# glmanhtu/vit-ed

Hardware: AMD Instinct MI355X
Metric: patch-pairs/sec fwd+bwd, div2k_erosion7_4bin_patch8_64 ViT-ED (higher is better)
Workload: dtype bf16

## Files before the change

### include/vited.h

```cpp
#ifndef VITED_H
#define VITED_H

#include <stdint.h>

#ifdef __cplusplus
extern "C" {
#endif

#define VITED_ABI_VERSION 1

#define VITED_OK 0
#define VITED_ERR_BAD_ARG 1
#define VITED_ERR_UNSUPPORTED 2
#define VITED_ERR_LAUNCH 3
#define VITED_ERR_WORKSPACE 4

#define VITED_F32 0
#define VITED_BF16 1
#define VITED_F16 2
#define VITED_I32 3
#define VITED_I64 4

#define VITED_EPI_STORE 0
#define VITED_EPI_GELU 1
#define VITED_EPI_RESIDUAL 2
#define VITED_EPI_MUL_GELU_GRAD 3
#define VITED_EPI_STORE_F32 4
#define VITED_EPI_MUL 5
#define VITED_EPI_GELU_GRAD 6

#define VITED_B_NK 0
#define VITED_B_KN 1

int vited_abi_version(void);
const char* vited_strerror(int code);

int vited_last_gemm_path(void);
int vited_last_attention_path(void);


int vited_cast(const void* src, int src_dtype, void* dst, int dst_dtype, int64_t n, void* stream);

int vited_cast_transpose(const float* src, void* dst, int dst_dtype, int64_t rows, int64_t cols, void* stream);

int vited_cast_weights(const int64_t* desc, int count, int64_t total_tiles, void* stream);

int vited_patchify(const float* img, int64_t img_bs, const int64_t* batch_index, void* out, int out_dtype,
                   int64_t batch, int chans, int img_size, int patch, void* stream);

int vited_patchify_u8(const uint8_t* img, int64_t img_bs, const int64_t* batch_index, void* out, int out_dtype,
                      int64_t batch, int chans, int img_size, int patch, const float* mean, const float* std, void* stream);

int vited_crop_pairs_u8(const uint8_t* src, int64_t src_bs, const int* cells, const int* erode, uint8_t* out, int64_t batch,
                        int chans, int img_size, void* stream);

int vited_div2k_regions_u8(const uint8_t* store, const int64_t* img_off, const int* img_hw, int n_images, const int* image,
                           const int* flags, const double* minv, const float* rgb, const int* crop, uint8_t* out, int64_t batch,
                           int img_size, void* stream);

int vited_hisfrag_windows_u8(const uint8_t* store, const int64_t* img_off, const int* img_hw, int n_images, const int* image,
                             const int* flags, const int64_t* afix, const double* minv, const int* origin, uint8_t* out, int64_t batch,
                             int img_size, void* stream);

int vited_hisfrag_jitter_u8(const uint8_t* in, const int* flags, const int* order, const float* factors, const int* hue, int64_t* sums,
                            uint8_t* out, int64_t batch, int img_size, void* stream);

int vited_hisfrag_blur_u8(const uint8_t* in, const int* flags, const float* weights, uint8_t* out, int64_t batch, int img_size,
                          void* stream);

int vited_michigan_windows_u8(const uint8_t* store, const int64_t* img_off, const int* img_hw, int n_images, const int* image,
                              const int* flags, const int* origin, const int* x0, const int* kx, const int* y0, const int* ky,
                              const int* holes, const int* n_holes, uint8_t* out, int64_t batch, int img_size, void* stream);

int vited_michigan_blur_gray_u8(const uint8_t* in, const int* flags, const int* weights, uint8_t* out, int64_t batch, int img_size,
                                void* stream);

int vited_slice_rows_cast(const float* in, void* out, int out_dtype, int64_t batch, int64_t in_rows,
                          int64_t row_offset, int64_t rows, int64_t dim, void* stream);

int vited_write_cls_row(float* x, const float* cls, const float* pos, int64_t batch, int64_t rows_per_batch,
                        int64_t dim, void* stream);

int64_t vited_sum_rows_workspace_bytes(int64_t batch, int64_t width);
int vited_sum_rows(const void* in, int in_dtype, int64_t in_ld, float* out, int64_t batch, int64_t width,
                   float* workspace, int64_t workspace_bytes, void* stream);


int vited_layernorm_fwd(const float* x, int64_t x_ld, const float* gamma, const float* beta, void* y,
                        int y_dtype, int64_t y_ld, float* mean, float* rstd, int64_t rows, int64_t dim,
                        float eps, void* stream);

int64_t vited_layernorm_bwd_workspace_bytes(int64_t rows, int64_t dim);
int vited_layernorm_bwd(const void* dy, int dy_dtype, int64_t dy_ld, const float* x, int64_t x_ld,
                        const float* gamma, const float* mean, const float* rstd, const float* dx_in,
                        int64_t dx_in_ld, float* dx_out, int64_t dx_out_ld, void* dx_lp, int dx_lp_dtype,
                        int64_t dx_lp_ld, float* dgamma, float* dbeta, int accumulate, int64_t rows, int64_t dim,
                        float* workspace, int64_t workspace_bytes, void* stream);

int vited_layernorm_bwd_scaled(const void* dy, int dy_dtype, int64_t dy_ld, const float* x, int64_t x_ld,
                               const float* gamma, const float* mean, const float* rstd, const float* dx_in,
                               int64_t dx_in_ld, float* dx_out, int64_t dx_out_ld, void* dx_lp, int dx_lp_dtype,
                               int64_t dx_lp_ld, const float* lp_scale, float* dgamma, float* dbeta, int accumulate,
                               int64_t rows, int64_t dim, float* workspace, int64_t workspace_bytes, void* stream);

int vited_scale_rows_cast(const float* src, int64_t src_ld, const float* row_scale, void* dst, int dst_dtype, int64_t dst_ld,
                          int64_t rows, int64_t dim, void* stream);


int vited_gemm(const void* A, int64_t lda, const void* B, int64_t ldb, int b_layout, int dtype, int64_t M,
               int64_t N, int64_t K, int epilogue, const float* bias, const void* aux,
               const float* residual, void* out, void* out2, int64_t ldo, int64_t rows_per_batch,
               int64_t out_rows_per_batch, int64_t row_offset, int residual_bcast, void* stream);

int vited_gemm_scaled(const void* A, int64_t lda, const void* B, int64_t ldb, int b_layout, int dtype, int64_t M, int64_t N,
                      int64_t K, const float* bias, const float* residual, const float* row_scale, float* out, int64_t ldo,
                      void* stream);

int64_t vited_linear_bwd_weight_workspace_bytes(int64_t M, int64_t N, int64_t K);
int vited_linear_bwd_weight(const void* dY, int64_t lddy, const void* X, int64_t ldx, int dtype, int64_t M,
                            int64_t N, int64_t K, float* dW, float* dbias, int accumulate, float* workspace,
                            int64_t workspace_bytes, void* stream);

int vited_linear_bwd_weight_batched_supported(int count, const int64_t* M, const int64_t* N, const int64_t* K, int dtype);
int64_t vited_linear_bwd_weight_batched_workspace_bytes(int count, const int64_t* M, const int64_t* N, const int64_t* K);
int vited_linear_bwd_weight_batched(int count, const void* const* dY, const int64_t* lddy, const void* const* X,
                                    const int64_t* ldx, const int64_t* M, const int64_t* N, const int64_t* K, float* const* dW,
                                    float* const* dbias, int dtype, int accumulate, float* workspace, int64_t workspace_bytes,
                                    void* stream);

int vited_linear_layernorm_supported(int64_t M, int64_t N, int64_t K);

int vited_linear_residual_layernorm_fwd(const void* a, int64_t lda, const void* w, int64_t ldw, const float* bias,
                                        const float* residual, int64_t ldr, float* y, int64_t ldy, const float* gamma,
                                        const float* beta, float eps, void* h, int64_t ldh, float* mean, float* rstd,
                                        int64_t M, int64_t N, int64_t K, void* stream);

int vited_linear_residual_layernorm_fwd_scaled(const void* a, int64_t lda, const void* w, int64_t ldw, const float* bias,
                                               const float* residual, int64_t ldr, const float* row_scale, float* y, int64_t ldy,
                                               const float* gamma, const float* beta, float eps, void* h, int64_t ldh, float* mean,
                                               float* rstd, int64_t M, int64_t N, int64_t K, void* stream);

int vited_linear_layernorm_bwd_segmented(const void* dy, int64_t lddy, int64_t seg_k, int64_t seg_stride, int64_t segments,
                                         const void* wt, int64_t ldwt, const float* x, int64_t ldx, const float* gamma,
                                         const float* mean, const float* rstd, const float* dx_in, int64_t dx_in_ld,
                                         float* dx_out, int64_t dx_out_ld, void* dx_lp, int64_t dx_lp_ld, float* dgamma,
                                         float* dbeta, int accumulate, int64_t M, int64_t N, float* workspace,
                                         int64_t workspace_bytes, void* stream);
int64_t vited_linear_layernorm_bwd_partial_rows(int64_t M);
int vited_layernorm_bwd_finish_batched(int count, const float* const* partial, const int* nparts, float* const* dgamma,
                                       float* const* dbeta, const int* accumulate, int64_t dim, void* stream);
int64_t vited_linear_layernorm_bwd_workspace_bytes(int64_t M, int64_t N);
int vited_linear_layernorm_bwd(const void* dy, int64_t lddy, const void* wt, int64_t ldwt, const float* x, int64_t ldx,
                               const float* gamma, const float* mean, const float* rstd, const float* dx_in,
                               int64_t dx_in_ld, float* dx_out, int64_t dx_out_ld, void* dx_lp, int64_t dx_lp_ld,
                               float* dgamma, float* dbeta, int accumulate, int64_t M, int64_t N, int64_t K,
                               float* workspace, int64_t workspace_bytes, void* stream);

int vited_linear_layernorm_bwd_scaled(const void* dy, int64_t lddy, const void* wt, int64_t ldwt, const float* x, int64_t ldx,
                                      const float* gamma, const float* mean, const float* rstd, const float* dx_in,
                                      int64_t dx_in_ld, float* dx_out, int64_t dx_out_ld, void* dx_lp, int64_t dx_lp_ld,
                                      const float* lp_scale, float* dgamma, float* dbeta, int accumulate, int64_t M, int64_t N,
                                      int64_t K, float* workspace, int64_t workspace_bytes, void* stream);

int vited_fold_context_weights(int count, const float* const* w, const float* const* bias, const float* const* gamma,
                               const float* const* beta, int64_t N, int64_t K, void* w_out, void* wt_out, float* bias_out,
                               void* stream);
int vited_unfold_context_grads(int count, const float* dwf, const float* dbf, const float* const* w, const float* const* gamma,
                               const float* const* beta, float* const* dw, float* const* dbias, float* const* dgamma, float* const* dbeta, int64_t N,
                               int64_t K, int accumulate, void* stream);


int vited_mlp_fwd(const float* x, int64_t ldx, const float* gamma, const float* beta, const void* w1, const float* b1,
                  const void* w2, const float* b2, float* y, int64_t ldy, void* h, void* gd, void* u, float* mean,
                  float* rstd, int64_t rows, int64_t dim, int64_t hidden, float eps, void* stream);

int64_t vited_block_workspace_bytes(int64_t batch, int64_t tokens, int64_t dim, int64_t hidden, int heads);
int vited_block_fwd(const float* x, float* y, int64_t batch, int64_t tokens, int64_t dim, int heads, int64_t hidden,
                    const float* ln1_g, const float* ln1_b, const void* wqkv, const float* bqkv, const void* wproj,
                    const float* bproj, const float* ln2_g, const float* ln2_b, const void* w1, const float* b1,
                    const void* w2, const float* b2, float eps, void* workspace, int64_t workspace_bytes, void* stream);

int64_t vited_cross_block_workspace_bytes(int64_t batch, int64_t tokens, int64_t ctx_tokens, int64_t dim, int64_t hidden, int heads);
int vited_cross_block_fwd(const float* x, const float* context, float* y, int64_t batch, int64_t tokens, int64_t ctx_tokens,
                          int64_t dim, int heads, int64_t hidden, const float* ln1_g, const float* ln1_b, const void* wqkv,
                          const float* bqkv, const void* wproj, const float* bproj, const float* lnq_g, const float* lnq_b,
                          const float* lnc_g, const float* lnc_b, const void* wq, const float* bq, const void* wkv,
                          const float* bkv, const void* wcproj, const float* bcproj, const float* ln2_g, const float* ln2_b,
                          const void* w1, const float* b1, const void* w2, const float* b2, float eps, void* workspace,
                          int64_t workspace_bytes, void* stream);


int64_t vited_adamw_workspace_bytes(void);
int vited_adamw_step(const int64_t* desc, int count, int64_t total_tiles, const float* grad_flat, int64_t grad_numel,
                     float* hyper, float max_norm, int zero_grad, float* norm_out, float* workspace,
                     int64_t workspace_bytes, void* stream);

int vited_sgd_step(const int64_t* desc, int count, int64_t total_tiles, const float* grad_flat, int64_t grad_numel,
                   float* hyper, float max_norm, int zero_grad, float* norm_out, float* workspace,
                   int64_t workspace_bytes, void* stream);


int vited_attention_fwd(const void* q, int64_t q_bs, int64_t q_ts, const void* k, int64_t k_bs, int64_t k_ts,
                        const void* v, int64_t v_bs, int64_t v_ts, void* o, int64_t o_bs, int64_t o_ts,
                        float* lse, int dtype, int64_t batch, int heads, int64_t nq, int64_t nk, int head_dim,
                        float scale, void* stream);

int vited_attention_fwd_indexed(const void* q, int64_t q_bs, int64_t q_ts, const void* k, int64_t k_bs, int64_t k_ts,
                                const void* v, int64_t v_bs, int64_t v_ts, const int64_t* kv_index, void* o, int64_t o_bs,
                                int64_t o_ts, float* lse, int dtype, int64_t batch, int heads, int64_t nq, int64_t nk,
                                int head_dim, float scale, void* stream);

int vited_attention_bwd(const void* q, int64_t q_bs, int64_t q_ts, const void* k, int64_t k_bs, int64_t k_ts,
                        const void* v, int64_t v_bs, int64_t v_ts, const void* o, const void* d_o,
                        int64_t o_bs, int64_t o_ts, const float* lse, float* delta, void* dq, int64_t dq_bs,
                        int64_t dq_ts, void* dk, int64_t dk_bs, int64_t dk_ts, void* dv, int64_t dv_bs,
                        int64_t dv_ts, int dtype, int64_t batch, int heads, int64_t nq, int64_t nk,
                        int head_dim, float scale, void* stream);

int64_t vited_attention_bwd_indexed_workspace_bytes(int dtype, int64_t batch, int heads, int64_t nk, int head_dim);
int vited_attention_bwd_indexed(const void* q, int64_t q_bs, int64_t q_ts, const void* k, int64_t k_bs, int64_t k_ts,
                                const void* v, int64_t v_bs, int64_t v_ts, const int64_t* kv_index, const int64_t* seg_order,
                                const int64_t* seg_offsets, int64_t kv_items, const void* o, const void* d_o, int64_t o_bs,
                                int64_t o_ts, const float* lse, float* delta, void* dq, int64_t dq_bs, int64_t dq_ts, void* dk,
                                int64_t dk_bs, int64_t dk_ts, void* dv, int64_t dv_bs, int64_t dv_ts, int dtype, int64_t batch,
                                int heads, int64_t nq, int64_t nk, int head_dim, float scale, void* workspace,
                                int64_t workspace_bytes, void* stream);

enum { VITED_CAM_GRAD = 0, VITED_CAM_PROB = 1 };
int vited_attention_cam(const void* q, int64_t q_bs, int64_t q_ts, const void* k, int64_t k_bs, int64_t k_ts,
                        const void* v, int64_t v_bs, int64_t v_ts, const void* d_o, int64_t do_bs, int64_t do_ts,
                        const float* lse, const float* head_weight, float* cam, int64_t cam_bs, int64_t cam_ld,
                        int mode, int dtype, int64_t batch, int heads, int64_t nq, int64_t nk, int head_dim,
                        float scale, void* stream);


int vited_retrieval_metrics(const void* D, int dtype, int64_t ld, int64_t n, int64_t r0, int64_t r1, const int* labels,
                            const int* offsets, const int* members, int num_classes, int remove_self_column, int from_similarity,
                            double* rows_out, double* sums, void* stream);


int vited_group_retrieval_metrics(const void* D, int dtype, int64_t ld, int64_t n, int64_t r0, int64_t r1, const int* labels,
                                  int num_labels, const int* col_offsets, const int* col_members, const int* pos_offsets,
                                  const int* pos_labels, const int* neg_offsets, const int* neg_labels, const int* ks, int nk,
                                  double* rows_out, double* sums, void* stream);


int64_t vited_pair_scores_workspace_bytes(int64_t n, int64_t m);
int vited_pair_scores_add(const void* pairs, int pair_dtype, int64_t pair_ld, const void* scores, int score_dtype, int64_t m, int64_t n,
                          int* counts, int* rec_cells, float* rec_values, int* bad, void* stream);
int vited_pair_scores_finish(const int* rec_cells, const float* rec_values, int64_t m, int64_t n, const int* counts, float* mean,
                             float* minv, double* stdev, double* stats, int* bad, void* workspace, int64_t workspace_bytes,
                             void* stream);

int vited_puzzle_distances_from_logits(const float* logits, const int64_t* pi, const int64_t* pj, int64_t m, int64_t n, int* dq,
                                       int* bad, void* stream);
int vited_puzzle_compat_init(const int* dq, int64_t n, int64_t* min_d, int64_t* second_d, int* candidate, int* best_buddy,
                             float* compat, float* mutual, int* start_count, float* start_total, int* start_order, void* stream);
int vited_puzzle_compat_recalc(const int* dq, int64_t n, const int* placed, int64_t* min_d, int64_t* second_d, float* compat,
                               float* mutual, int* changed, void* stream);
int vited_puzzle_best_slot(const float* mutual, int64_t n, const int* placed, const int* slot_piece, const int* slot_side,
                           int64_t slots, int64_t* best, void* stream);

int vited_cls_metrics_update(const float* logits, int64_t ld_logits, const float* targets, int64_t ld_targets, int64_t batch,
                             int64_t classes, double* meters, double* last, int* bad, void* stream);

int vited_mine_pairs_max_images(void);
int vited_mine_pairs(const int64_t* targets, int n, const float* keys, double neg_per_pos, int ordered_negatives, int64_t capacity,
                     int64_t* groups, float* labels, float* weights, int64_t* seg_index, int64_t* seg_order, int64_t* seg_offsets,
                     int32_t* counts, void* stream);

#ifdef __cplusplus
}
#endif
#endif
```

### vit-ed_amd/csrc/attention.hip

```cpp
#include "attention_kernels.h"
#include "pair_segsum.h"

static thread_local int g_last_attn_path = 0;
extern "C" int vited_last_attention_path(void) { return g_last_attn_path; }
void attention_set_last_path(int path) { g_last_attn_path = path; }

static int check_common(const AttnArgs& a, int dtype) {
    if (!a.q || !a.k || !a.v || !a.o || !a.lse) return VITED_ERR_BAD_ARG;
    if (a.batch <= 0 || a.heads <= 0 || a.nq <= 0 || a.nk <= 0 || a.head_dim <= 0) return VITED_ERR_BAD_ARG;
    if (dtype != VITED_F32 && dtype != VITED_BF16) return VITED_ERR_UNSUPPORTED;
    if (a.batch > 65535 || a.heads > 65535) return VITED_ERR_UNSUPPORTED;
    return VITED_OK;
}

extern "C" int vited_attention_fwd(const void* q, int64_t q_bs, int64_t q_ts, const void* k, int64_t k_bs, int64_t k_ts,
                                   const void* v, int64_t v_bs, int64_t v_ts, void* o, int64_t o_bs, int64_t o_ts,
                                   float* lse, int dtype, int64_t batch, int heads, int64_t nq, int64_t nk, int head_dim,
                                   float scale, void* stream) {
    return vited_attention_fwd_indexed(q, q_bs, q_ts, k, k_bs, k_ts, v, v_bs, v_ts, nullptr, o, o_bs, o_ts, lse, dtype, batch, heads, nq,
                                       nk, head_dim, scale, stream);
}

extern "C" int vited_attention_fwd_indexed(const void* q, int64_t q_bs, int64_t q_ts, const void* k, int64_t k_bs, int64_t k_ts,
                                           const void* v, int64_t v_bs, int64_t v_ts, const int64_t* kv_index, void* o, int64_t o_bs,
                                           int64_t o_ts, float* lse, int dtype, int64_t batch, int heads, int64_t nq, int64_t nk,
                                           int head_dim, float scale, void* stream) {
    AttnArgs a = {};
    a.q = q; a.k = k; a.v = v;
    a.kv_index = kv_index;
    a.q_bs = q_bs; a.q_ts = q_ts; a.k_bs = k_bs; a.k_ts = k_ts; a.v_bs = v_bs; a.v_ts = v_ts;
    a.o = o; a.o_bs = o_bs; a.o_ts = o_ts;
    a.lse = lse;
    a.batch = batch; a.heads = heads; a.nq = nq; a.nk = nk; a.head_dim = head_dim; a.scale = scale;
    int rc = check_common(a, dtype);
    if (rc != VITED_OK) return rc;
    hipStream_t s = (hipStream_t)stream;
    if (dtype == VITED_BF16 && attention_mfma_supported(a, false)) {
        g_last_attn_path = 2;
        return attention_fwd_mfma(a, s);
    }
    g_last_attn_path = 1;
    return attention_fwd_portable(a, dtype, s);
}

static int bwd_dispatch(const AttnArgs& a, int dtype, hipStream_t s) {
    if (dtype == VITED_BF16 && attention_mfma_supported(a, true)) {
        g_last_attn_path = 2;
        return attention_bwd_mfma(a, s);
    }
    g_last_attn_path = 1;
    return attention_bwd_portable(a, dtype, s);
}

extern "C" int vited_attention_bwd(const void* q, int64_t q_bs, int64_t q_ts, const void* k, int64_t k_bs, int64_t k_ts,
                                   const void* v, int64_t v_bs, int64_t v_ts, const void* o, const void* d_o, int64_t o_bs,
                                   int64_t o_ts, const float* lse, float* delta, void* dq, int64_t dq_bs, int64_t dq_ts,
                                   void* dk, int64_t dk_bs, int64_t dk_ts, void* dv, int64_t dv_bs, int64_t dv_ts, int dtype,
                                   int64_t batch, int heads, int64_t nq, int64_t nk, int head_dim, float scale, void* stream) {
    AttnArgs a = {};
    a.q = q; a.k = k; a.v = v;
    a.q_bs = q_bs; a.q_ts = q_ts; a.k_bs = k_bs; a.k_ts = k_ts; a.v_bs = v_bs; a.v_ts = v_ts;
    a.o = o; a.d_o = d_o; a.o_bs = o_bs; a.o_ts = o_ts;
    a.lse = (float*)lse; a.delta = delta;
    a.dq = dq; a.dk = dk; a.dv = dv;
    a.dq_bs = dq_bs; a.dq_ts = dq_ts; a.dk_bs = dk_bs; a.dk_ts = dk_ts; a.dv_bs = dv_bs; a.dv_ts = dv_ts;
    a.batch = batch; a.heads = heads; a.nq = nq; a.nk = nk; a.head_dim = head_dim; a.scale = scale;
    int rc = check_common(a, dtype);
    if (rc != VITED_OK) return rc;
    if (!d_o || !delta || !dq || !dk || !dv) return VITED_ERR_BAD_ARG;
    return bwd_dispatch(a, dtype, (hipStream_t)stream);
}

static int64_t elem_bytes(int dtype) { return dtype == VITED_BF16 ? 2 : 4; }

extern "C" int64_t vited_attention_bwd_indexed_workspace_bytes(int dtype, int64_t batch, int heads, int64_t nk, int head_dim) {
    if ((dtype != VITED_F32 && dtype != VITED_BF16) || batch <= 0 || heads <= 0 || nk <= 0 || head_dim <= 0) return -1;
    return batch * nk * 2 * (int64_t)heads * head_dim * elem_bytes(dtype);
}

extern "C" int vited_attention_bwd_indexed(const void* q, int64_t q_bs, int64_t q_ts, const void* k, int64_t k_bs, int64_t k_ts,
                                           const void* v, int64_t v_bs, int64_t v_ts, const int64_t* kv_index,
                                           const int64_t* seg_order, const int64_t* seg_offsets, int64_t kv_items, const void* o,
                                           const void* d_o, int64_t o_bs, int64_t o_ts, const float* lse, float* delta, void* dq,
                                           int64_t dq_bs, int64_t dq_ts, void* dk, int64_t dk_bs, int64_t dk_ts, void* dv,
                                           int64_t dv_bs, int64_t dv_ts, int dtype, int64_t batch, int heads, int64_t nq, int64_t nk,
                                           int head_dim, float scale, void* workspace, int64_t workspace_bytes, void* stream) {
    AttnArgs a = {};
    a.q = q; a.k = k; a.v = v;
    a.kv_index = kv_index;
    a.q_bs = q_bs; a.q_ts = q_ts; a.k_bs = k_bs; a.k_ts = k_ts; a.v_bs = v_bs; a.v_ts = v_ts;
    a.o = o; a.d_o = d_o; a.o_bs = o_bs; a.o_ts = o_ts;
    a.lse = (float*)lse; a.delta = delta;
    a.dq = dq; a.dq_bs = dq_bs; a.dq_ts = dq_ts;
    a.batch = batch; a.heads = heads; a.nq = nq; a.nk = nk; a.head_dim = head_dim; a.scale = scale;
    int rc = check_common(a, dtype);
    if (rc != VITED_OK) return rc;
    if (!d_o || !delta || !dq || !dk || !dv || !kv_index || !seg_order || !seg_offsets || !workspace) return VITED_ERR_BAD_ARG;
    if (kv_items <= 0 || ((uintptr_t)workspace % 16) != 0) return VITED_ERR_BAD_ARG;
    if (kv_items > 65535) return VITED_ERR_UNSUPPORTED;
    if (workspace_bytes < vited_attention_bwd_indexed_workspace_bytes(dtype, batch, heads, nk, head_dim)) return VITED_ERR_WORKSPACE;
    const int64_t width = (int64_t)heads * head_dim;
    a.dk = workspace;
    a.dv = (char*)workspace + width * elem_bytes(dtype);
    a.dk_ts = a.dv_ts = 2 * width;
    a.dk_bs = a.dv_bs = nk * 2 * width;
    hipStream_t s = (hipStream_t)stream;
    rc = bwd_dispatch(a, dtype, s);
    if (rc != VITED_OK) return rc;
    SegSumArgs g = {};
    g.ws = workspace;
    g.out[0] = dk; g.out_bs[0] = dk_bs; g.out_ts[0] = dk_ts;
    g.out[1] = dv; g.out_bs[1] = dv_bs; g.out_ts[1] = dv_ts;
    g.order = seg_order; g.offsets = seg_offsets;
    g.batch = batch; g.items = kv_items; g.nk = nk; g.width = (int)width;
    return attention_segsum(g, dtype, s);
}
```

### vit-ed_amd/csrc/attention_kernels.h

```cpp
#pragma once
#include "common.h"

struct AttnArgs {
    const void *q, *k, *v;
    const int64_t* kv_index;
    int64_t q_bs, q_ts, k_bs, k_ts, v_bs, v_ts;
    const void* o;
    const void* d_o;
    int64_t o_bs, o_ts;
    float* lse;
    float* delta;
    void *dq, *dk, *dv;
    int64_t dq_bs, dq_ts, dk_bs, dk_ts, dv_bs, dv_ts;
    int64_t batch, nq, nk;
    int heads, head_dim;
    float scale;
};

int attention_fwd_portable(const AttnArgs& a, int dtype, hipStream_t s);
int attention_bwd_portable(const AttnArgs& a, int dtype, hipStream_t s);

bool attention_mfma_supported(const AttnArgs& a, bool backward);
int attention_fwd_mfma(const AttnArgs& a, hipStream_t s);
int attention_bwd_mfma(const AttnArgs& a, hipStream_t s);

int attention_fwd_flash(const AttnArgs& a, hipStream_t s);
int attention_bwd_flash(const AttnArgs& a, hipStream_t s);

struct SegSumArgs;
int attention_segsum(const SegSumArgs& a, int dtype, hipStream_t s);

void attention_set_last_path(int path);
```

### vit-ed_amd/csrc/attention_mfma.hip

```cpp
#include "attention_tiles.h"

template <int HD, int NKT>
__global__ void __launch_bounds__(256)
attn_fwd_small_kernel(AttnArgs a) {
    using C = SmallCfg<HD>;
    extern __shared__ __attribute__((aligned(16))) char smem[];
    const int lane = threadIdx.x & 63;
    const int wave = __builtin_amdgcn_readfirstlane(threadIdx.x >> 6);
    const int fr = lane & 15, g = lane >> 4, qq = fr >> 2, p = fr & 3;
    const int64_t b = blockIdx.x;
    int h = blockIdx.y * 4 + wave;
    const bool live = h < a.heads;
    h = live ? h : a.heads - 1;
    const int nq = (int)a.nq, nk = (int)a.nk;
    const bf16* qb = (const bf16*)a.q + b * a.q_bs + (int64_t)h * HD;
    const int64_t bkv = a.kv_index ? a.kv_index[b] : b;
    const bf16* kb = (const bf16*)a.k + bkv * a.k_bs + (int64_t)h * HD;
    const bf16* vb = (const bf16*)a.v + bkv * a.v_bs + (int64_t)h * HD;
    char* vs = smem + wave * C::TILE_BYTES;
    char* os = smem + 4 * C::TILE_BYTES + wave * 16 * C::ROW_BYTES;

    bf16x8 kf[NKT][C::KCH], qnext[C::KCH];
    load_row_frags<HD>(qb, a.q_ts, 0, nq, fr, g, qnext);
#pragma unroll
    for (int t = 0; t < NKT; ++t) {
        load_row_frags<HD>(kb, a.k_ts, 16 * t, nk, fr, g, kf[t]);
        bf16x8 vf[C::KCH];
        load_row_frags<HD>(vb, a.v_ts, 16 * t, nk, fr, g, vf);
        stage_tile<HD>(vs, 16 * t, nk, fr, g, vf);
    }
    if (NKT & 1) {
        const bf16x8 z[C::KCH] = {};
        stage_tile<HD>(vs, 16 * NKT, 0, fr, g, z);
    }
    asm volatile("" ::: "memory");
    const float sc = a.scale * LOG2E;
    const int nqt = (nq + 15) >> 4;
    for (int i = 0; i < nqt; ++i) {
        bf16x8 qf[C::KCH];
#pragma unroll
        for (int c = 0; c < C::KCH; ++c) qf[c] = qnext[c];
        if (i + 1 < nqt) load_row_frags<HD>(qb, a.q_ts, 16 * (i + 1), nq, fr, g, qnext);
        f32x4 st[NKT + 1];
        float m = -INFINITY;
#pragma unroll
        for (int t = 0; t < NKT; ++t) {
            f32x4 s = {0.f, 0.f, 0.f, 0.f};
#pragma unroll
            for (int c = 0; c < C::KCH; ++c) s = __builtin_amdgcn_mfma_f32_16x16x32_bf16(kf[t][c], qf[c], s, 0, 0, 0);
            if (t == NKT - 1) {
#pragma unroll
                for (int e = 0; e < 4; ++e) s[e] = (16 * t + 4 * g + e) < nk ? s[e] : -INFINITY;
            }
            m = fmaxf(fmaxf(m, fmaxf(s[0], s[1])), fmaxf(s[2], s[3]));
            st[t] = s;
        }
        st[NKT] = f32x4{0.f, 0.f, 0.f, 0.f};
        m = group_max4(m) * sc;
        float l = 0.f;
#pragma unroll
        for (int t = 0; t < NKT; ++t)
#pragma unroll
            for (int e = 0; e < 4; ++e) {
                const float pe = __builtin_amdgcn_exp2f(fmaf(st[t][e], sc, -m));
                st[t][e] = pe;
                l += pe;
            }
        l = group_sum4(l);
        const float inv = 1.f / l;
        const int q = 16 * i + fr;
#pragma unroll
        for (int dt = 0; dt < C::DT; ++dt) {
            f32x4 o = {0.f, 0.f, 0.f, 0.f};
#pragma unroll
            for (int ks = 0; ks < (NKT + 1) / 2; ++ks) {
                const bf16x8 vt = tr_frag<HD>(vs, ks, dt, g, qq, p);
                o = __builtin_amdgcn_mfma_f32_16x16x32_bf16(vt, pack_pair(st[2 * ks], st[2 * ks + 1]), o, 0, 0, 0);
            }
            const bf16x4 ov = {(bf16)(o[0] * inv), (bf16)(o[1] * inv), (bf16)(o[2] * inv), (bf16)(o[3] * inv)};
            *(bf16x4*)(os + fr * C::ROW_BYTES + (dt * 16 + 4 * g) * 2) = ov;
        }
        asm volatile("" ::: "memory");
        {
            constexpr int CPR = C::ROW_BYTES / 16;
#pragma unroll
            for (int j = 0; j < 16 * CPR / 64; ++j) {
                const int c = lane + 64 * j;
                const int row = c / CPR, ch = c % CPR;
                const bf16x8 v = *(const bf16x8*)(os + row * C::ROW_BYTES + ch * 16);
                if (live && 16 * i + row < nq)
                    *(bf16x8*)((bf16*)a.o + b * a.o_bs + (int64_t)(16 * i + row) * a.o_ts + (int64_t)h * HD + ch * 8) = v;
            }
        }
        asm volatile("" ::: "memory");
        if (live && g == 0 && q < nq) a.lse[(b * a.heads + h) * a.nq + q] = (m + log2f(l)) * LN2;
    }
}

template <int HD, int NT>
__device__ __forceinline__ void store_rows4(const char* region, bf16* dst_head0, int64_t ts, int n, int live_heads, int tid) {
    constexpr int ROW = 4 * HD * 2, CPR = ROW / 16;
#pragma unroll
    for (int j = 0; j < NT * 16 * CPR / 256; ++j) {
        const int c = tid + 256 * j;
        const int row = c / CPR, ch = c % CPR;
        const bf16x8 v = *(const bf16x8*)(region + row * ROW + ch * 16);
        if (row < n && ch / (CPR / 4) < live_heads) *(bf16x8*)(dst_head0 + (int64_t)row * ts + ch * 8) = v;
    }
}

template <int HD, int NQT, int NKT> struct BwdSmallLds {
    static constexpr int MAXT = NQT > NKT ? NQT : NKT;
    static constexpr int IMG_TILES = (MAXT + 1) & ~1;
    static constexpr int IMG_BYTES = IMG_TILES * 16 * HD * 2;
    static constexpr int STAT_FLOATS = IMG_TILES * 16;
    static constexpr int WAVE_BYTES = 2 * IMG_BYTES + 2 * STAT_FLOATS * 4;
    static constexpr int SLOT1_BASE = 4 * IMG_BYTES, STATS_BASE = 8 * IMG_BYTES;
};

template <int HD, int NQT, int NKT>
#ifndef ATTN_BWD_WAVES_PER_EU
#define ATTN_BWD_WAVES_PER_EU 3
#endif
__global__ void __launch_bounds__(256) __attribute__((amdgpu_waves_per_eu(ATTN_BWD_WAVES_PER_EU)))
attn_bwd_small_kernel(AttnArgs a) {
    using C = SmallCfg<HD>;
    extern __shared__ __attribute__((aligned(16))) char smem[];
    using L = BwdSmallLds<HD, NQT, NKT>;
    const int lane = threadIdx.x & 63;
    const int wave = __builtin_amdgcn_readfirstlane(threadIdx.x >> 6);
    const int fr = lane & 15, g = lane >> 4, qq = fr >> 2, p = fr & 3;
    const int64_t b = blockIdx.y;
    const int hg = blockIdx.x;
    int h = hg * 4 + wave;
    const bool live = h < a.heads;
    h = live ? h : a.heads - 1;
    const int nq = (int)a.nq, nk = (int)a.nk;
    const int64_t hoff = (int64_t)h * HD;
    const bf16* qb = (const bf16*)a.q + b * a.q_bs + hoff;
    const int64_t bkv = a.kv_index ? a.kv_index[b] : b;
    const bf16* kb = (const bf16*)a.k + bkv * a.k_bs + hoff;
    const bf16* vb = (const bf16*)a.v + bkv * a.v_bs + hoff;
    const bf16* dob = (const bf16*)a.d_o + b * a.o_bs + hoff;
    char* k_s = smem + wave * L::IMG_BYTES;
    char* q_s = k_s;
    char* do_s = smem + L::SLOT1_BASE + wave * L::IMG_BYTES;
    float* lse_s = (float*)(smem + L::STATS_BASE) + wave * 2 * L::STAT_FLOATS;
    float* del_s = lse_s + L::STAT_FLOATS;
    char* out0 = smem;
    char* out1 = smem + L::SLOT1_BASE;
    const int tid = threadIdx.x;
    const int live_heads = a.heads - hg * 4;
    const int64_t hoff0 = (int64_t)hg * 4 * HD;
    constexpr int OROW = 4 * HD * 2;
    const float sc = a.scale * LOG2E;

    bf16x8 kf[NKT][C::KCH], vf[NKT][C::KCH], qf[NQT][C::KCH], dof[NQT][C::KCH];
    float lse_r[NQT];
#pragma unroll
    for (int t = 0; t < NKT; ++t) {
        load_row_frags<HD>(kb, a.k_ts, 16 * t, nk, fr, g, kf[t]);
        load_row_frags<HD>(vb, a.v_ts, 16 * t, nk, fr, g, vf[t]);
    }
#pragma unroll
    for (int i = 0; i < NQT; ++i) {
        load_row_frags<HD>(qb, a.q_ts, 16 * i, nq, fr, g, qf[i]);
        load_row_frags<HD>(dob, a.o_ts, 16 * i, nq, fr, g, dof[i]);
        const int q = 16 * i + fr;
        lse_r[i] = a.lse[(b * a.heads + h) * a.nq + (q < nq ? q : nq - 1)];
    }
    asm volatile("" ::: "memory");
#pragma unroll
    for (int t = 0; t < NKT; ++t) stage_tile<HD>(k_s, 16 * t, nk, fr, g, kf[t]);
#pragma unroll
    for (int i = 0; i < NQT; ++i) {
        const int q = 16 * i + fr;
        if (g == 0) lse_s[q] = lse_r[i] * LOG2E;
    }
    {
        const bf16x8 z[C::KCH] = {};
        if (NKT & 1) stage_tile<HD>(k_s, 16 * NKT, 0, fr, g, z);
    }
    asm volatile("" ::: "memory");

#pragma unroll
    for (int i = 0; i < NQT; ++i) {
        const int q = 16 * i + fr;
        const float lse2 = lse_s[q];
        f32x4 ds[NKT + 1], dpv[NKT];
        float dl = 0.f;
#pragma unroll
        for (int t = 0; t < NKT; ++t) {
            f32x4 s = {0.f, 0.f, 0.f, 0.f}, dp = {0.f, 0.f, 0.f, 0.f};
#pragma unroll
            for (int c = 0; c < C::KCH; ++c) {
                s = __builtin_amdgcn_mfma_f32_16x16x32_bf16(kf[t][c], qf[i][c], s, 0, 0, 0);
                dp = __builtin_amdgcn_mfma_f32_16x16x32_bf16(vf[t][c], dof[i][c], dp, 0, 0, 0);
            }
#pragma unroll
            for (int e = 0; e < 4; ++e) {
                float pe = __builtin_amdgcn_exp2f(fmaf(s[e], sc, -lse2));
                if (t == NKT - 1) pe = (16 * t + 4 * g + e) < nk ? pe : 0.f;
                ds[t][e] = pe;
                dl = fmaf(pe, dp[e], dl);
            }
            dpv[t] = dp;
        }
        dl = group_sum4(dl);
        if (g == 0) del_s[q] = dl;
#pragma unroll
        for (int t = 0; t < NKT; ++t)
#pragma unroll
            for (int e = 0; e < 4; ++e) ds[t][e] *= dpv[t][e] - dl;
        ds[NKT] = f32x4{0.f, 0.f, 0.f, 0.f};
#pragma unroll
        for (int dt = 0; dt < C::DT; ++dt) {
            f32x4 acc = {0.f, 0.f, 0.f, 0.f};
#pragma unroll
            for (int ks = 0; ks < (NKT + 1) / 2; ++ks)
                acc = __builtin_amdgcn_mfma_f32_16x16x32_bf16(tr_frag<HD>(k_s, ks, dt, g, qq, p),
                                                              pack_pair(ds[2 * ks], ds[2 * ks + 1]), acc, 0, 0, 0);
            const bf16x4 ov = {(bf16)(acc[0] * a.scale), (bf16)(acc[1] * a.scale), (bf16)(acc[2] * a.scale), (bf16)(acc[3] * a.scale)};
            *(bf16x4*)(out1 + q * OROW + wave * (HD * 2) + (dt * 16 + 4 * g) * 2) = ov;
        }
    }
    __syncthreads();
    store_rows4<HD, NQT>(out1, (bf16*)a.dq + b * a.dq_bs + hoff0, a.dq_ts, nq, live_heads, tid);
    __syncthreads();

    asm volatile("" ::: "memory");
#pragma unroll
    for (int i = 0; i < NQT; ++i) {
        stage_tile<HD>(q_s, 16 * i, nq, fr, g, qf[i]);
        stage_tile<HD>(do_s, 16 * i, nq, fr, g, dof[i]);
    }
    if (NQT & 1) {
        const bf16x8 z[C::KCH] = {};
        stage_tile<HD>(q_s, 16 * NQT, 0, fr, g, z);
        stage_tile<HD>(do_s, 16 * NQT, 0, fr, g, z);
    }
    asm volatile("" ::: "memory");
    bf16x4 dvo[NKT][C::DT], dko[NKT][C::DT];
#pragma unroll
    for (int t = 0; t < NKT; ++t) {
        f32x4 pr[NQT + 1], ds[NQT + 1];
#pragma unroll
        for (int i = 0; i < NQT; ++i) {
            f32x4 s = {0.f, 0.f, 0.f, 0.f}, dp = {0.f, 0.f, 0.f, 0.f};
#pragma unroll
            for (int c = 0; c < C::KCH; ++c) {
                s = __builtin_amdgcn_mfma_f32_16x16x32_bf16(qf[i][c], kf[t][c], s, 0, 0, 0);
                dp = __builtin_amdgcn_mfma_f32_16x16x32_bf16(dof[i][c], vf[t][c], dp, 0, 0, 0);
            }
            const f32x4 l4 = *(const f32x4*)(lse_s + 16 * i + 4 * g);
            const f32x4 d4 = *(const f32x4*)(del_s + 16 * i + 4 * g);
#pragma unroll
            for (int e = 0; e < 4; ++e) {
                float pe = __builtin_amdgcn_exp2f(fmaf(s[e], sc, -l4[e]));
                if (i == NQT - 1) pe = (16 * i + 4 * g + e) < nq ? pe : 0.f;
                pr[i][e] = pe;
                ds[i][e] = pe * (dp[e] - d4[e]);
            }
        }
        pr[NQT] = f32x4{0.f, 0.f, 0.f, 0.f};
        ds[NQT] = f32x4{0.f, 0.f, 0.f, 0.f};
#pragma unroll
        for (int dt = 0; dt < C::DT; ++dt) {
            f32x4 av = {0.f, 0.f, 0.f, 0.f}, ak = {0.f, 0.f, 0.f, 0.f};
#pragma unroll
            for (int qs = 0; qs < (NQT + 1) / 2; ++qs) {
                av = __builtin_amdgcn_mfma_f32_16x16x32_bf16(tr_frag<HD>(do_s, qs, dt, g, qq, p),
                                                             pack_pair(pr[2 * qs], pr[2 * qs + 1]), av, 0, 0, 0);
                ak = __builtin_amdgcn_mfma_f32_16x16x32_bf16(tr_frag<HD>(q_s, qs, dt, g, qq, p),
                                                             pack_pair(ds[2 * qs], ds[2 * qs + 1]), ak, 0, 0, 0);
            }
            dvo[t][dt] = bf16x4{(bf16)av[0], (bf16)av[1], (bf16)av[2], (bf16)av[3]};
            dko[t][dt] = bf16x4{(bf16)(ak[0] * a.scale), (bf16)(ak[1] * a.scale), (bf16)(ak[2] * a.scale), (bf16)(ak[3] * a.scale)};
        }
        __builtin_amdgcn_sched_barrier(0);
    }
    __syncthreads();
#pragma unroll
    for (int t = 0; t < NKT; ++t)
#pragma unroll
        for (int dt = 0; dt < C::DT; ++dt) {
            *(bf16x4*)(out0 + (16 * t + fr) * OROW + wave * (HD * 2) + (dt * 16 + 4 * g) * 2) = dvo[t][dt];
            *(bf16x4*)(out1 + (16 * t + fr) * OROW + wave * (HD * 2) + (dt * 16 + 4 * g) * 2) = dko[t][dt];
        }
    __syncthreads();
    store_rows4<HD, NKT>(out0, (bf16*)a.dv + b * a.dv_bs + hoff0, a.dv_ts, nk, live_heads, tid);
    store_rows4<HD, NKT>(out1, (bf16*)a.dk + b * a.dk_bs + hoff0, a.dk_ts, nk, live_heads, tid);
}

static bool small_ok(const AttnArgs& a, bool backward) {
    if (a.nk > 16 * SM_MAX_TILES) return false;
    if (backward) return a.head_dim == 32 && a.nq <= 16 * SM_MAX_TILES;
    return true;
}

bool attention_mfma_supported(const AttnArgs& a, bool backward) {
    auto al = [](const void* p, int n) { return ((uintptr_t)p % n) == 0; };
    if (a.head_dim != 32 && a.head_dim != 64) return false;
    if (a.nq > (1 << 20) || a.nk > (1 << 20)) return false;
    if (a.q_ts % 8 || a.k_ts % 8 || a.v_ts % 8 || a.q_bs % 8 || a.k_bs % 8 || a.v_bs % 8 || a.o_ts % 8 || a.o_bs % 8) return false;
    if (!al(a.q, 16) || !al(a.k, 16) || !al(a.v, 16) || !al(a.o, 16)) return false;
    if (backward) {
        if (a.dq_ts % 8 || a.dk_ts % 8 || a.dv_ts % 8 || a.dq_bs % 8 || a.dk_bs % 8 || a.dv_bs % 8) return false;
        if (!al(a.d_o, 16) || !al(a.dq, 16) || !al(a.dk, 16) || !al(a.dv, 16)) return false;
    }
    return true;
}

template <int HD>
static int launch_fwd_small(const AttnArgs& a, hipStream_t s) {
    const int nkt = (int)((a.nk + 15) / 16);
    dim3 grid((unsigned)a.batch, (unsigned)((a.heads + 3) / 4));
    const size_t lds = 4 * SmallCfg<HD>::TILE_BYTES + 4 * 16 * SmallCfg<HD>::ROW_BYTES;
#define L(N) hipLaunchKernelGGL((attn_fwd_small_kernel<HD, N>), grid, dim3(256), lds, s, a)
    switch (nkt) {
        case 1: L(1); break;
        case 2: L(2); break;
        case 3: L(3); break;
        case 4: L(4); break;
        case 5: L(5); break;
        default: return VITED_ERR_UNSUPPORTED;
    }
#undef L
    return vited_check_launch();
}

int attention_fwd_mfma(const AttnArgs& a, hipStream_t s) {
    if (!small_ok(a, false)) return attention_fwd_flash(a, s);
    if (a.head_dim == 32) return launch_fwd_small<32>(a, s);
    if (a.head_dim == 64) return launch_fwd_small<64>(a, s);
    return VITED_ERR_UNSUPPORTED;
}

template <int NQT, int NKT>
static void launch_bwd_small_one(const AttnArgs& a, dim3 grid, hipStream_t s) {
    auto kernel = attn_bwd_small_kernel<32, NQT, NKT>;
    constexpr size_t lds = 4 * BwdSmallLds<32, NQT, NKT>::WAVE_BYTES;
    hipLaunchKernelGGL(kernel, grid, dim3(256), lds, s, a);
}

template <int NQT>
static int launch_bwd_small32(const AttnArgs& a, int nkt, hipStream_t s) {
    dim3 grid((unsigned)((a.heads + 3) / 4), (unsigned)a.batch);
#define L(N) launch_bwd_small_one<NQT, N>(a, grid, s)
    switch (nkt) {
        case 1: L(1); break;
        case 2: L(2); break;
        case 3: L(3); break;
        case 4: L(4); break;
        case 5: L(5); break;
        default: return VITED_ERR_UNSUPPORTED;
    }
#undef L
    return vited_check_launch();
}

int attention_bwd_mfma(const AttnArgs& a, hipStream_t s) {
    if (!small_ok(a, true)) return attention_bwd_flash(a, s);
    const int nqt = (int)((a.nq + 15) / 16), nkt = (int)((a.nk + 15) / 16);
    switch (nqt) {
        case 1: return launch_bwd_small32<1>(a, nkt, s);
        case 2: return launch_bwd_small32<2>(a, nkt, s);
        case 3: return launch_bwd_small32<3>(a, nkt, s);
        case 4: return launch_bwd_small32<4>(a, nkt, s);
        case 5: return launch_bwd_small32<5>(a, nkt, s);
        default: return VITED_ERR_UNSUPPORTED;
    }
}
```

### vit-ed_amd/csrc/elementwise.hip

```cpp
#include "common.h"

template <typename S, typename D>
__global__ void cast_kernel(const S* __restrict__ src, D* __restrict__ dst, int64_t n) {
    int64_t i = ((int64_t)blockIdx.x * blockDim.x + threadIdx.x) * 4;
    const int64_t stride = (int64_t)gridDim.x * blockDim.x * 4;
    for (; i + 3 < n; i += stride) {
        S a = src[i], b = src[i + 1], c = src[i + 2], d = src[i + 3];
        dst[i] = from_f32<D>(to_f32(a));
        dst[i + 1] = from_f32<D>(to_f32(b));
        dst[i + 2] = from_f32<D>(to_f32(c));
        dst[i + 3] = from_f32<D>(to_f32(d));
    }
    for (; i < n; ++i) dst[i] = from_f32<D>(to_f32(src[i]));
}

extern "C" int vited_cast(const void* src, int src_dtype, void* dst, int dst_dtype, int64_t n, void* stream) {
    if (!src || !dst || n < 0) return VITED_ERR_BAD_ARG;
    if (n == 0) return VITED_OK;
    hipStream_t s = (hipStream_t)stream;
    const int threads = 256;
    int64_t blocks = ceil_div64(n, threads * 4);
    if (blocks > 4096) blocks = 4096;
    if (src_dtype == VITED_F32 && dst_dtype == VITED_BF16)
        hipLaunchKernelGGL((cast_kernel<float, bf16>), dim3(blocks), dim3(threads), 0, s, (const float*)src, (bf16*)dst, n);
// ... 84 lines not shown
        const int mid = (lo + hi + 1) >> 1;
        if (desc[(int64_t)mid * WS_DESC_WORDS + 5] <= blk) lo = mid; else hi = mid - 1;
    }
    const int64_t* d = desc + (int64_t)lo * WS_DESC_WORDS;
    const float* __restrict__ src = (const float*)d[0];
    bf16* __restrict__ dst = (bf16*)d[1];
    bf16* __restrict__ dst_t = (bf16*)d[2];
    const int64_t rows = d[3], cols = d[4];
    const int64_t t = blk - d[5], tiles_c = (cols + 63) >> 6;
    const int64_t r0 = (t / tiles_c) << 6, c0 = (t % tiles_c) << 6;
    const int tx = threadIdx.x & 15, ty = threadIdx.x >> 4;
    const bool vec = (cols & 3) == 0;
#pragma unroll
    for (int j = 0; j < 4; ++j) {
        const int lr = ty + 16 * j;
        const int64_t r = r0 + lr, c = c0 + tx * 4;
        float v[4] = {0.f, 0.f, 0.f, 0.f};
        if (r < rows) {
            if (vec && c + 3 < cols) {
                const f32x4 q = *(const f32x4*)(src + r * cols + c);
                v[0] = q[0]; v[1] = q[1]; v[2] = q[2]; v[3] = q[3];
            } else {
#pragma unroll
                for (int e = 0; e < 4; ++e) if (c + e < cols) v[e] = src[r * cols + c + e];
            }
        }
        bf16 b[4];
#pragma unroll
        for (int e = 0; e < 4; ++e) { b[e] = (bf16)v[e]; tile[lr][tx * 4 + e] = b[e]; }
        if (dst && r < rows) {
            if (vec && c + 3 < cols) *(bf16x4*)(dst + r * cols + c) = bf16x4{b[0], b[1], b[2], b[3]};
            else {
#pragma unroll
                for (int e = 0; e < 4; ++e) if (c + e < cols) dst[r * cols + c + e] = b[e];
            }
        }
    }
    if (!dst_t) return;
    __syncthreads();
    const bool vec_t = (rows & 3) == 0;
#pragma unroll
    for (int j = 0; j < 4; ++j) {
        const int lc = ty + 16 * j;
        const int64_t c = c0 + lc, r = r0 + tx * 4;
        if (c >= cols) continue;
        bf16 b[4];
#pragma unroll
        for (int e = 0; e < 4; ++e) b[e] = tile[tx * 4 + e][lc];
        if (vec_t && r + 3 < rows) *(bf16x4*)(dst_t + c * rows + r) = bf16x4{b[0], b[1], b[2], b[3]};
        else {
#pragma unroll
            for (int e = 0; e < 4; ++e) if (r + e < rows) dst_t[c * rows + r + e] = b[e];
        }
    }
}

extern "C" int vited_cast_weights(const int64_t* desc, int count, int64_t total_tiles, void* stream) {
    if (!desc || count <= 0 || total_tiles <= 0 || total_tiles > 0x7fffffff) return VITED_ERR_BAD_ARG;
    hipLaunchKernelGGL(cast_weights_kernel, dim3((unsigned)total_tiles), dim3(256), 0, (hipStream_t)stream, desc, count);
    return vited_check_launch();
}

template <typename D>
__global__ void patchify_kernel(const float* __restrict__ img, int64_t img_bs, const int64_t* __restrict__ bidx,
                                D* __restrict__ out, int chans, int S, int p) {
    const int G = S / p;
    const int64_t b = blockIdx.y;
    const int py = blockIdx.x;
    const int64_t src_b = bidx ? bidx[b] : b;
    const float* base = img + src_b * img_bs;
    const int Kp = chans * p * p;
    const int total = chans * p * S;
    D* obase = out + (b * G * G + (int64_t)py * G) * Kp;
    for (int e = threadIdx.x; e < total; e += blockDim.x) {
        const int x = e % S;
        const int ci = e / S;
        const int i = ci % p, c = ci / p;
        const float v = base[((int64_t)c * S + (py * p + i)) * S + x];
        const int px = x / p, j = x - px * p;
        obase[(int64_t)px * Kp + (c * p + i) * p + j] = from_f32<D>(v);
    }
}

extern "C" int vited_patchify(const float* img, int64_t img_bs, const int64_t* batch_index, void* out, int out_dtype,
                              int64_t batch, int chans, int img_size, int patch, void* stream) {
    if (!img || !out || batch <= 0 || chans <= 0 || img_size <= 0 || patch <= 0 || img_size % patch) return VITED_ERR_BAD_ARG;
    dim3 grid(img_size / patch, (unsigned)batch);
    hipStream_t s = (hipStream_t)stream;
    if (out_dtype == VITED_BF16)
        hipLaunchKernelGGL((patchify_kernel<bf16>), grid, dim3(256), 0, s, img, img_bs, batch_index, (bf16*)out, chans, img_size, patch);
    else if (out_dtype == VITED_F32)
        hipLaunchKernelGGL((patchify_kernel<float>), grid, dim3(256), 0, s, img, img_bs, batch_index, (float*)out, chans, img_size, patch);
    else
        return VITED_ERR_UNSUPPORTED;
    return vited_check_launch();
}

struct U8Norm { float scale[4], shift[4]; };

template <typename D>
__global__ void patchify_u8_kernel(const uint8_t* __restrict__ img, int64_t img_bs, const int64_t* __restrict__ bidx,
                                   D* __restrict__ out, int chans, int S, int p, U8Norm nrm) {
    const int G = S / p;
    const int64_t b = blockIdx.y;
    const int py = blockIdx.x;
    const int64_t src_b = bidx ? bidx[b] : b;
    const uint8_t* base = img + src_b * img_bs;
    const int Kp = chans * p * p;
    const int total = chans * p * S;
    D* obase = out + (b * G * G + (int64_t)py * G) * Kp;
    for (int e = threadIdx.x; e < total; e += blockDim.x) {
        const int x = e % S;
        const int ci = e / S;
        const int i = ci % p, c = ci / p;
        const float v = fmaf((float)base[((int64_t)c * S + (py * p + i)) * S + x], nrm.scale[c], nrm.shift[c]);
        const int px = x / p, j = x - px * p;
        obase[(int64_t)px * Kp + (c * p + i) * p + j] = from_f32<D>(v);
    }
}

extern "C" int vited_patchify_u8(const uint8_t* img, int64_t img_bs, const int64_t* batch_index, void* out, int out_dtype,
                                 int64_t batch, int chans, int img_size, int patch, const float* mean, const float* std,
                                 void* stream) {
    if (!img || !out || !mean || !std || batch <= 0 || chans <= 0 || chans > 4 || img_size <= 0 || patch <= 0 || img_size % patch)
        return VITED_ERR_BAD_ARG;
    U8Norm nrm = {};
    for (int c = 0; c < chans; ++c) {
        if (!(std[c] > 0.f)) return VITED_ERR_BAD_ARG;
        nrm.scale[c] = 1.0f / (255.0f * std[c]);
        nrm.shift[c] = -mean[c] / std[c];
    }
    dim3 grid(img_size / patch, (unsigned)batch);
    hipStream_t s = (hipStream_t)stream;
    if (out_dtype == VITED_BF16)
        hipLaunchKernelGGL((patchify_u8_kernel<bf16>), grid, dim3(256), 0, s, img, img_bs, batch_index, (bf16*)out, chans, img_size, patch, nrm);
    else if (out_dtype == VITED_F32)
        hipLaunchKernelGGL((patchify_u8_kernel<float>), grid, dim3(256), 0, s, img, img_bs, batch_index, (float*)out, chans, img_size, patch, nrm);
    else
        return VITED_ERR_UNSUPPORTED;
    return vited_check_launch();
}

struct ResampleTaps {
    int x0, n;
    int k0, k1;
};

__device__ __forceinline__ ResampleTaps resample_taps(int xx, int in_size, int out_size) {
    constexpr int PRECISION_BITS = 32 - 8 - 2;
    const double scale = (double)in_size / (double)out_size;
    const double center = (xx + 0.5) * scale;
    int xmin = (int)(center - 1.0 + 0.5);
    xmin = xmin < 0 ? 0 : xmin;
    int xmax = (int)(center + 1.0 + 0.5);
    xmax = (xmax < in_size ? xmax : in_size) - xmin;
    double w0 = 1.0 - fabs((double)xmin - center + 0.5), w1 = xmax > 1 ? 1.0 - fabs((double)xmin + 1.0 - center + 0.5) : 0.0;
    w0 = w0 < 0.0 ? 0.0 : w0;
    w1 = w1 < 0.0 ? 0.0 : w1;
    const double ww = w0 + w1;
    ResampleTaps t;
    t.x0 = xmin;
    t.n = xmax > 1 ? 2 : 1;
    t.k0 = (int)(0.5 + (w0 / ww) * (double)(1 << PRECISION_BITS));
    t.k1 = (int)(0.5 + (w1 / ww) * (double)(1 << PRECISION_BITS));
    return t;
}

__device__ __forceinline__ int resample_px(int p0, int p1, const ResampleTaps& t) {
    constexpr int PRECISION_BITS = 32 - 8 - 2;
    int acc = (1 << (PRECISION_BITS - 1)) + p0 * t.k0 + (t.n > 1 ? p1 * t.k1 : 0);
    acc >>= PRECISION_BITS;
    return acc < 0 ? 0 : (acc > 255 ? 255 : acc);
}

__global__ void __launch_bounds__(256)
crop_pairs_u8_kernel(const uint8_t* __restrict__ src, int64_t src_bs, const int* __restrict__ cells, const int* __restrict__ erode,
                     uint8_t* __restrict__ out, int chans, int S) {
    const int64_t b = blockIdx.z;
    const int img = blockIdx.y / chans, c = blockIdx.y % chans;
    int cell = cells[b * 2 + img], e = erode[b];
    cell = cell < 0 ? 0 : (cell > 5 ? 5 : cell);
    e = e < 1 ? 1 : (e > S ? S : e);
    const int off = (int)rint((S - e) / 2.0);
    const int r0 = (cell / 3) * S + off, c0 = (cell % 3) * S + off;
    const uint8_t* base = src + b * src_bs + ((int64_t)c * 2 * S + r0) * (3 * S) + c0;
    uint8_t* o = out + (((b * 2 + img) * chans + c) * (int64_t)S) * S;
    for (int i = blockIdx.x * blockDim.x + threadIdx.x; i < S * S; i += gridDim.x * blockDim.x) {
        const int y = i / S, x = i - y * S;
        const ResampleTaps tx = resample_taps(x, e, S), ty = resample_taps(y, e, S);
        const uint8_t* ra = base + (int64_t)ty.x0 * (3 * S) + tx.x0;
        const int h0 = resample_px(ra[0], tx.n > 1 ? ra[1] : 0, tx);
        int h1 = 0;
        if (ty.n > 1) {
            const uint8_t* rb = ra + 3 * S;
            h1 = resample_px(rb[0], tx.n > 1 ? rb[1] : 0, tx);
        }
        o[i] = (uint8_t)resample_px(h0, h1, ty);
    }
}

extern "C" int vited_crop_pairs_u8(const uint8_t* src, int64_t src_bs, const int* cells, const int* erode, uint8_t* out, int64_t batch,
                                   int chans, int img_size, void* stream) {
    if (!src || !cells || !erode || !out || batch <= 0 || chans <= 0 || img_size <= 0 || batch > 65535) return VITED_ERR_BAD_ARG;
    if (src_bs < (int64_t)chans * 6 * img_size * img_size) return VITED_ERR_BAD_ARG;
    const int per = img_size * img_size;
    dim3 grid((unsigned)((per + 1023) / 1024 < 8 ? (per + 1023) / 1024 : 8), (unsigned)(2 * chans), (unsigned)batch);
    hipLaunchKernelGGL(crop_pairs_u8_kernel, grid, dim3(256), 0, (hipStream_t)stream, src, src_bs, cells, erode, out, chans, img_size);
    return vited_check_launch();
}

template <typename D>
__global__ void slice_rows_cast_kernel(const float* __restrict__ in, D* __restrict__ out, int64_t in_rows,
                                       int64_t row_offset, int64_t rows, int64_t dim, int64_t total) {
    int64_t i = (int64_t)blockIdx.x * blockDim.x + threadIdx.x;
    const int64_t stride = (int64_t)gridDim.x * blockDim.x;
    const int64_t per_b = rows * dim;
    for (; i < total; i += stride) {
        const int64_t b = i / per_b, rem = i - b * per_b;
        out[i] = from_f32<D>(in[(b * in_rows + row_offset) * dim + rem]);
    }
}
// ... 8 lines not shown
    if (out_dtype == VITED_BF16)
        hipLaunchKernelGGL((slice_rows_cast_kernel<bf16>), dim3(blocks), dim3(256), 0, s, in, (bf16*)out, in_rows, row_offset, rows, dim, total);
    else if (out_dtype == VITED_F32)
        hipLaunchKernelGGL((slice_rows_cast_kernel<float>), dim3(blocks), dim3(256), 0, s, in, (float*)out, in_rows, row_offset, rows, dim, total);
    else
        return VITED_ERR_UNSUPPORTED;
    return vited_check_launch();
}

__global__ void write_cls_row_kernel(float* __restrict__ x, const float* __restrict__ cls, const float* __restrict__ pos,
                                     int64_t batch, int64_t rows_per_batch, int64_t dim) {
    int64_t i = (int64_t)blockIdx.x * blockDim.x + threadIdx.x;
    const int64_t total = batch * dim;
    if (i >= total) return;
    const int64_t b = i / dim, d = i - b * dim;
    x[b * rows_per_batch * dim + d] = cls[d] + pos[d];
}

extern "C" int vited_write_cls_row(float* x, const float* cls, const float* pos, int64_t batch, int64_t rows_per_batch,
                                   int64_t dim, void* stream) {
    if (!x || !cls || !pos || batch <= 0 || rows_per_batch <= 0 || dim <= 0) return VITED_ERR_BAD_ARG;
    const int64_t total = batch * dim;
    hipLaunchKernelGGL(write_cls_row_kernel, dim3((unsigned)ceil_div64(total, 256)), dim3(256), 0, (hipStream_t)stream,
                       x, cls, pos, batch, rows_per_batch, dim);
    return vited_check_launch();
}

template <typename S_>
__global__ void sum_rows_kernel(const S_* __restrict__ in, int64_t in_ld, float* __restrict__ out, int64_t batch,
                                int64_t width, int64_t rows_per_split) {
    const int64_t r = (int64_t)blockIdx.x * blockDim.x + threadIdx.x;
    if (r >= width) return;
    const int64_t b0 = (int64_t)blockIdx.y * rows_per_split;
    int64_t b1 = b0 + rows_per_split;
    if (b1 > batch) b1 = batch;
    float acc0 = 0.f, acc1 = 0.f, acc2 = 0.f, acc3 = 0.f;
    int64_t b = b0;
    for (; b + 3 < b1; b += 4) {
        acc0 += to_f32(in[b * in_ld + r]);
        acc1 += to_f32(in[(b + 1) * in_ld + r]);
        acc2 += to_f32(in[(b + 2) * in_ld + r]);
        acc3 += to_f32(in[(b + 3) * in_ld + r]);
    }
    for (; b < b1; ++b) acc0 += to_f32(in[b * in_ld + r]);
    out[(int64_t)blockIdx.y * width + r] = (acc0 + acc1) + (acc2 + acc3);
}

static inline int64_t sum_rows_splits(int64_t batch, int64_t width) {
    const int64_t col_blocks = ceil_div64(width, 256);
    int64_t s = ceil_div64(1024, col_blocks);
    const int64_t max_s = ceil_div64(batch, 16);
    if (s > max_s) s = max_s;
    if (s < 1) s = 1;
    return s;
}

extern "C" int64_t vited_sum_rows_workspace_bytes(int64_t batch, int64_t width) {
    return sum_rows_splits(batch, width) * width * (int64_t)sizeof(float);
}

extern "C" int vited_sum_rows(const void* in, int in_dtype, int64_t in_ld, float* out, int64_t batch, int64_t width,
                              float* workspace, int64_t workspace_bytes, void* stream) {
    if (!in || !out || batch <= 0 || width <= 0 || in_ld < width) return VITED_ERR_BAD_ARG;
    const int64_t S = sum_rows_splits(batch, width);
    hipStream_t s = (hipStream_t)stream;
    const unsigned col_blocks = (unsigned)ceil_div64(width, 256);
    float* pass1_out = out;
    if (S > 1) {
        if (!workspace || workspace_bytes < S * width * (int64_t)sizeof(float)) return VITED_ERR_WORKSPACE;
        pass1_out = workspace;
    }
    const int64_t rps = ceil_div64(batch, S);
    if (in_dtype == VITED_F32)
        hipLaunchKernelGGL((sum_rows_kernel<float>), dim3(col_blocks, (unsigned)S), dim3(256), 0, s, (const float*)in, in_ld, pass1_out, batch, width, rps);
    else if (in_dtype == VITED_BF16)
        hipLaunchKernelGGL((sum_rows_kernel<bf16>), dim3(col_blocks, (unsigned)S), dim3(256), 0, s, (const bf16*)in, in_ld, pass1_out, batch, width, rps);
    else
        return VITED_ERR_UNSUPPORTED;
    if (S > 1)
        hipLaunchKernelGGL((sum_rows_kernel<float>), dim3(col_blocks, 1), dim3(256), 0, s, (const float*)workspace, width, out, S, width, S);
    return vited_check_launch();
}

__device__ __forceinline__ void sum_slabs_body(const float* __restrict__ in, int64_t in_ld, float* __restrict__ out, int64_t batch,
                                               int64_t width, int accumulate, int64_t r) {
    if (r >= width) return;
    if (r + 3 < width) {
        f32x4 acc = accumulate ? *(const f32x4*)(out + r) : f32x4{0.f, 0.f, 0.f, 0.f};
        int64_t b = 0;
        for (; b + 4 <= batch; b += 4) {
            const f32x4 v0 = *(const f32x4*)(in + b * in_ld + r), v1 = *(const f32x4*)(in + (b + 1) * in_ld + r);
            const f32x4 v2 = *(const f32x4*)(in + (b + 2) * in_ld + r), v3 = *(const f32x4*)(in + (b + 3) * in_ld + r);
#pragma unroll
            for (int e = 0; e < 4; ++e) acc[e] += (v0[e] + v1[e]) + (v2[e] + v3[e]);
        }
        for (; b < batch; ++b) {
            const f32x4 v = *(const f32x4*)(in + b * in_ld + r);
#pragma unroll
            for (int e = 0; e < 4; ++e) acc[e] += v[e];
        }
        *(f32x4*)(out + r) = acc;
    } else {
        for (int64_t c = r; c < width; ++c) {
            float acc = accumulate ? out[c] : 0.f;
            for (int64_t b = 0; b < batch; ++b) acc += in[b * in_ld + c];
            out[c] = acc;
        }
    }
}

__global__ void sum_slabs_kernel(const float* __restrict__ in, int64_t in_ld, float* __restrict__ out, int64_t batch, int64_t width,
                                 int accumulate) {
    sum_slabs_body(in, in_ld, out, batch, width, accumulate, ((int64_t)blockIdx.x * blockDim.x + threadIdx.x) * 4);
}

__global__ void sum_slabs_pair_kernel(const float* __restrict__ in_a, int64_t ld_a, float* __restrict__ out_a, int64_t width_a,
                                      int blocks_a, const float* __restrict__ in_b, int64_t ld_b, float* __restrict__ out_b,
                                      int64_t width_b, int64_t batch, int accumulate) {
    if ((int)blockIdx.x < blocks_a)
        sum_slabs_body(in_a, ld_a, out_a, batch, width_a, accumulate, ((int64_t)blockIdx.x * blockDim.x + threadIdx.x) * 4);
    else
        sum_slabs_body(in_b, ld_b, out_b, batch, width_b, accumulate,
                       ((int64_t)(blockIdx.x - blocks_a) * blockDim.x + threadIdx.x) * 4);
}


__global__ void sum_slabs_scalar_kernel(const float* __restrict__ in, int64_t in_ld, float* __restrict__ out, int64_t batch,
                                        int64_t width, int accumulate) {
    const int64_t c = (int64_t)blockIdx.x * blockDim.x + threadIdx.x;
    if (c >= width) return;
    float acc = accumulate ? out[c] : 0.f;
    for (int64_t b = 0; b < batch; ++b) acc += in[b * in_ld + c];
    out[c] = acc;
}

int sum_rows_f32_single_pass(const float* in, int64_t in_ld, float* out, int64_t batch, int64_t width, hipStream_t s, int accumulate) {
    const bool vec = (width % 4 == 0) && (in_ld % 4 == 0) && ((((uintptr_t)in) | ((uintptr_t)out)) & 15) == 0;
    if (vec)
        hipLaunchKernelGGL(sum_slabs_kernel, dim3((unsigned)ceil_div64(width, 1024)), dim3(256), 0, s, in, in_ld, out, batch, width, accumulate);
    else
        hipLaunchKernelGGL(sum_slabs_scalar_kernel, dim3((unsigned)ceil_div64(width, 256)), dim3(256), 0, s, in, in_ld, out, batch, width, accumulate);
    return vited_check_launch();
}

#define SB_MAX 40
struct SumBatch {
    float* out[2 * SB_MAX];
    int64_t start[2 * SB_MAX + 1];
    const float* slabs;
    const float* bias_slabs;
    int64_t slab_stride, bias_stride, splits;
    int sections, accumulate;
};

__global__ void __launch_bounds__(256) sum_slabs_batch_kernel(const SumBatch b) {
    const int64_t r = ((int64_t)blockIdx.x * blockDim.x + threadIdx.x) * 4;
    if (r >= b.start[b.sections]) return;
    int sec = 0;
    for (int i = 1; i < b.sections; ++i)
        if (b.start[i] <= r) sec = i;
    float* out = b.out[sec];
    if (!out) return;
    const bool is_bias = r >= b.slab_stride;
    const float* in = is_bias ? b.bias_slabs + (r - b.slab_stride) : b.slabs + r;
    const int64_t ld = is_bias ? b.bias_stride : b.slab_stride;
    out += r - b.start[sec];
// ... 57 lines not shown
```

### vit-ed_amd/csrc/gemm_row.hip

```cpp
#include <mutex>
#include <type_traits>

#include "gemm_kernels.h"
#include "gemm_lds.h"

#define ROW_N 384
#define ROW_LD 388

enum { ROW_MODE_FWD = 0, ROW_MODE_BWD = 1 };

struct RowArgs {
    const bf16* A; int64_t lda;
    int seg_k; int64_t seg_stride;
    const bf16* W; int64_t ldw;
    int64_t M; int K;
    const float* bias; const float* residual; int64_t ldr;
    float* y; int64_t ldy;
    const float* gamma; const float* beta; float eps;
    bf16* h; int64_t ldh; float* mean; float* rstd;
    const float* x; int64_t ldx; const float* mean_in; const float* rstd_in;
    const float* dx_in; int64_t ldxi; float* dx; int64_t lddx; bf16* dx_lp; int64_t ldlp;
    float* partial;
    const float* row_scale;
    const float* lp_scale;
};

template <int MT> struct RowCfg {
    static_assert(MT == 6 || MT == 8 || MT == 9 || MT == 10, "tile heights: 96, 128, 144 or 160 rows");
    static constexpr int BM = 16 * MT;
    static constexpr int A_BYTES = BM * 128;
    static constexpr int W_BYTES = ROW_N * 128;
    static constexpr int W_BASE = 3 * A_BYTES;
    static constexpr int LDS_BYTES = 3 * A_BYTES + 2 * W_BYTES;
    static constexpr int P0 = (MT + 1) / 2;
    static constexpr int A_PIECES = 2 * MT;
    static constexpr int A_J = (A_PIECES + 3) / 4;
    static constexpr int PASS_SUB = MT == 8 ? 4 : MT == 10 ? 5 : 3;
    static constexpr int PASS_ROWS = 16 * PASS_SUB;
    static constexpr int NPASS = MT / PASS_SUB;
    static constexpr int ROWS_PER_HALF = PASS_ROWS / 16;
    static constexpr bool EPI_ALL_ROWS = MT <= 9;
    static_assert(MT % PASS_SUB == 0, "passes cover the tile");
    static_assert(LDS_BYTES <= 160 * 1024, "LDS");
    static_assert(LDS_BYTES >= PASS_ROWS * ROW_LD * 4, "epilogue scratch must fit the staging buffers");
    static_assert(LDS_BYTES >= 16 * 2 * ROW_N * 4, "column-partial combine must fit the staging buffers");
};

__device__ __forceinline__ float row_half_sum(float v) { return half_wave_sum(v); }

#define ROW_STORE(ptr, val) __builtin_nontemporal_store(val, ptr)
#define ROW_STORE_LP(ptr, val) (*(ptr) = (val))
#define ROW_LOAD(ptr) __builtin_nontemporal_load(ptr)

template <int SC> struct RowFwdIn { f32x4 res[3]; float scale[SC]; };
template <int SC> struct RowBwdIn { f32x4 x[3], din[3]; float mu, rs; float lps[SC]; };

template <int MODE, int MT, bool SCALED>
__global__ void __launch_bounds__(512)
gemm_row_kernel(const RowArgs a) {
    extern __shared__ __attribute__((aligned(16))) char smem[];
    using R = RowCfg<MT>;
    const int lane = threadIdx.x & 63;
    const int wave = __builtin_amdgcn_readfirstlane(threadIdx.x >> 6);
    const int64_t m0 = (int64_t)blockIdx.x * R::BM;

    f32x4 acc[MT][3];
#pragma unroll
    for (int i = 0; i < MT; ++i)
#pragma unroll
        for (int j = 0; j < 3; ++j) acc[i][j] = f32x4{0.f, 0.f, 0.f, 0.f};

    const int grp = wave >> 2, u = wave & 3;
    const int nt = a.K / 64;
    const int r8 = lane >> 3, c8 = lane & 7;
    const int cs_even = (c8 ^ (r8 >> 1)) * 8, cs_odd = (c8 ^ (r8 >> 1) ^ 4) * 8;
    const int cs_u = (u & 1) ? cs_odd : cs_even;
    const int a_per = (R::A_PIECES - u + 3) / 4;
    const bf16* pa[R::A_J];
#pragma unroll
    for (int j = 0; j < R::A_J; ++j) {
        int64_t ar = m0 + 8 * (4 * j + u) + r8;
#ifdef ROW_DBG_A_RESIDENT
        ar -= m0;
#endif
        ar = ar < a.M ? ar : a.M - 1;
        pa[j] = a.A + ar * a.lda + cs_u;
    }
    const bf16* pw = a.W + (int64_t)(8 * u + r8) * a.ldw + cs_u;
    auto issue_a = [&](int t) {
#ifdef ROW_DBG_NO_DMA
        return;
#endif
        if (t >= nt) return;
        char* dst = smem + (t % 3) * R::A_BYTES;
        const int k0 = t * 64;
        const int seg = k0 / a.seg_k;
        const int64_t ka = (int64_t)seg * a.seg_stride + (k0 - seg * a.seg_k);
#pragma unroll
        for (int j = 0; j < R::A_J; ++j)
            if (4 * j + 3 < R::A_PIECES || j < a_per) glds16_asm(pa[j] + ka, dst + (4 * j + u) * 1024);
    };
    auto issue_w = [&](int t, int part) {
#ifdef ROW_DBG_NO_DMA
        return;
// ... 65 lines not shown
    };
    using I0 = std::integral_constant<int, 0>;
    using IP0 = std::integral_constant<int, R::P0>;
    using IP1 = std::integral_constant<int, MT - R::P0>;
    if (grp == 0) {
        issue_a(0);
        issue_w(0, 1);
        issue_a(1);
        certify_barrier(nt > 1);
        for (int t = 0; t < nt; ++t) {
            read_b(t);
            read_a(t, I0{}, IP0{});
            issue_w(t + 1, 1);
            landed();
            barrier();
            mfmas(I0{}, IP0{});
            barrier();
            read_a(t, IP0{}, IP1{});
            issue_a(t + 2);
            landed();
            barrier();
            mfmas(IP0{}, IP1{});
            certify_barrier(t + 2 < nt);
        }
        barrier();
    } else {
        issue_w(0, 0);
        issue_w(0, 2);
        issue_w(1, 0);
        certify_barrier(nt > 1);
        barrier();
        for (int t = 0; t < nt; ++t) {
            read_b(t);
            read_a(t, I0{}, IP0{});
            issue_w(t + 1, 2);
            landed();
            barrier();
            mfmas(I0{}, IP0{});
            barrier();
            read_a(t, IP0{}, IP1{});
            issue_w(t + 2, 0);
            landed();
            certify_barrier(t + 2 < nt);
            mfmas(IP0{}, IP1{});
            barrier();
        }
    }
#ifdef ROW_DBG_NO_EPI
#pragma unroll
    for (int i = 0; i < MT; ++i)
#pragma unroll
        for (int j = 0; j < 3; ++j) asm volatile("" ::"v"(acc[i][j]));
    return;
#endif

    float* sc = (float*)smem;
    const int hl = lane & 31;
    const int hw = wave * 2 + (lane >> 5);
    const float inv_d = 1.0f / ROW_N;
    f32x4 gm[3], bt[3], bs[3];
#pragma unroll
    for (int j = 0; j < 3; ++j) {
        const int c = (j * 32 + hl) * 4;
        gm[j] = a.gamma ? *(const f32x4*)(a.gamma + c) : f32x4{1.f, 1.f, 1.f, 1.f};
        bt[j] = (MODE == ROW_MODE_FWD && a.beta) ? *(const f32x4*)(a.beta + c) : f32x4{0.f, 0.f, 0.f, 0.f};
        bs[j] = (MODE == ROW_MODE_FWD && a.bias) ? *(const f32x4*)(a.bias + c) : f32x4{0.f, 0.f, 0.f, 0.f};
    }
    f32x4 dg[3], db[3];
#pragma unroll
    for (int j = 0; j < 3; ++j) {
        dg[j] = f32x4{0.f, 0.f, 0.f, 0.f};
        db[j] = f32x4{0.f, 0.f, 0.f, 0.f};
    }
    auto load_fwd = [&](RowFwdIn<SCALED>& in, int64_t m) {
        const bool ok = m < a.M;
        if constexpr (SCALED) in.scale[0] = ok ? a.row_scale[m] : 0.f;
#pragma unroll
        for (int j = 0; j < 3; ++j)
            in.res[j] = ok ? ROW_LOAD((const f32x4*)(a.residual + m * a.ldr + (j * 32 + hl) * 4)) : f32x4{0.f, 0.f, 0.f, 0.f};
    };
    auto load_bwd = [&](RowBwdIn<SCALED>& in, int64_t m) {
        const bool ok = m < a.M;
        if constexpr (SCALED) in.lps[0] = ok ? a.lp_scale[m] : 0.f;
#pragma unroll
        for (int j = 0; j < 3; ++j) {
            const int c = (j * 32 + hl) * 4;
            in.x[j] = ok ? ROW_LOAD((const f32x4*)(a.x + m * a.ldx + c)) : f32x4{0.f, 0.f, 0.f, 0.f};
            in.din[j] = (ok && a.dx_in) ? ROW_LOAD((const f32x4*)(a.dx_in + m * a.ldxi + c)) : f32x4{0.f, 0.f, 0.f, 0.f};
        }
        in.mu = ok ? a.mean_in[m] : 0.f;
        in.rs = ok ? a.rstd_in[m] : 0.f;
    };
    auto row_fwd = [&](const RowFwdIn<SCALED>& in, int r, int64_t m) {
        if (m >= a.M) return;
        f32x4 v[3];
        float s = 0.f;
#pragma unroll
        for (int j = 0; j < 3; ++j) {
            const int c = (j * 32 + hl) * 4;
            v[j] = *(const f32x4*)(sc + r * ROW_LD + c);
#pragma unroll
            for (int e = 0; e < 4; ++e) {
                v[j][e] += bs[j][e];
                if constexpr (SCALED) v[j][e] = in.res[j][e] + in.scale[0] * v[j][e];
                else v[j][e] += in.res[j][e];
            }
            ROW_STORE((f32x4*)(a.y + m * a.ldy + c), v[j]);
            s += (v[j][0] + v[j][1]) + (v[j][2] + v[j][3]);
        }
        if (!a.h) return;
        const float mu = row_half_sum(s) * inv_d;
        float q = 0.f;
#pragma unroll
        for (int j = 0; j < 3; ++j)
#pragma unroll
            for (int e = 0; e < 4; ++e) {
                const float d = v[j][e] - mu;
                q = fmaf(d, d, q);
            }
        const float rs = rsqrtf(row_half_sum(q) * inv_d + a.eps);
#pragma unroll
        for (int j = 0; j < 3; ++j) {
            const int c = (j * 32 + hl) * 4;
            bf16x4 o;
#pragma unroll
            for (int e = 0; e < 4; ++e) o[e] = (bf16)((v[j][e] - mu) * rs * gm[j][e] + bt[j][e]);
            ROW_STORE_LP((bf16x4*)(a.h + m * a.ldh + c), o);
        }
        if (hl == 0) {
            a.mean[m] = mu;
            a.rstd[m] = rs;
        }
    };
    auto row_bwd = [&](const RowBwdIn<SCALED>& in, int r, int64_t m) {
        if (m >= a.M) return;
        f32x4 xh[3], gg[3];
        float s1 = 0.f, s2 = 0.f;
#pragma unroll
        for (int j = 0; j < 3; ++j) {
            const int c = (j * 32 + hl) * 4;
            const f32x4 d = *(const f32x4*)(sc + r * ROW_LD + c);
#pragma unroll
            for (int e = 0; e < 4; ++e) {
                xh[j][e] = (in.x[j][e] - in.mu) * in.rs;
                gg[j][e] = d[e] * gm[j][e];
                s1 += gg[j][e];
                s2 = fmaf(gg[j][e], xh[j][e], s2);
                dg[j][e] = fmaf(d[e], xh[j][e], dg[j][e]);
                db[j][e] += d[e];
            }
        }
        const float c1 = row_half_sum(s1) * inv_d, c2 = row_half_sum(s2) * inv_d;
#pragma unroll
        for (int j = 0; j < 3; ++j) {
            const int c = (j * 32 + hl) * 4;
            f32x4 v;
#pragma unroll
            for (int e = 0; e < 4; ++e) v[e] = in.rs * (gg[j][e] - c1 - xh[j][e] * c2) + in.din[j][e];
            ROW_STORE((f32x4*)(a.dx + m * a.lddx + c), v);
            if constexpr (SCALED) {
#pragma unroll
                for (int e = 0; e < 4; ++e) v[e] *= in.lps[0];
            }
            if (a.dx_lp) ROW_STORE_LP((bf16x4*)(a.dx_lp + m * a.ldlp + c), (bf16x4{(bf16)v[0], (bf16)v[1], (bf16)v[2], (bf16)v[3]}));
        }
    };

#pragma unroll
    for (int p = 0; p < R::NPASS; ++p) {
        const int64_t mp = m0 + p * R::PASS_ROWS;
        constexpr int AHEAD = R::EPI_ALL_ROWS ? R::ROWS_PER_HALF : 1;
// ... 66 lines not shown
}

static inline int64_t row_tiles(int64_t M) { return ceil_div64(M, 16 * row_mt(M)); }

static bool row_shape_ok(int64_t M, int64_t N, int64_t K) { return N == ROW_N && K >= 64 && K % 64 == 0 && K <= (1 << 20) && M >= 1 && M < ((int64_t)1 << 31); }

extern "C" int vited_linear_layernorm_supported(int64_t M, int64_t N, int64_t K) { return row_shape_ok(M, N, K) ? 1 : 0; }

template <int MODE, int MT, bool SCALED>
static int row_launch_scaled(const RowArgs& a, unsigned tiles, hipStream_t s) {
    auto kernel = gemm_row_kernel<MODE, MT, SCALED>;
    static std::once_flag once;
    static hipError_t status = hipSuccess;
    std::call_once(once, [&] { status = hipFuncSetAttribute((const void*)kernel, hipFuncAttributeMaxDynamicSharedMemorySize, RowCfg<MT>::LDS_BYTES); });
    if (status != hipSuccess) return VITED_ERR_LAUNCH;
    hipLaunchKernelGGL(kernel, dim3(tiles), dim3(512), RowCfg<MT>::LDS_BYTES, s, a);
    return vited_check_launch();
}

template <int MODE, int MT>
static int row_launch_mt(const RowArgs& a, unsigned tiles, hipStream_t s) {
    if (MODE == ROW_MODE_FWD ? a.row_scale != nullptr : a.lp_scale != nullptr) return row_launch_scaled<MODE, MT, true>(a, tiles, s);
    return row_launch_scaled<MODE, MT, false>(a, tiles, s);
}

template <int MODE>
static int row_launch(const RowArgs& a, hipStream_t s) {
    const unsigned tiles = (unsigned)row_tiles(a.M);
    switch (row_mt(a.M)) {
        case 6: return row_launch_mt<MODE, 6>(a, tiles, s);
        case 9: return row_launch_mt<MODE, 9>(a, tiles, s);
        case 10: return row_launch_mt<MODE, 10>(a, tiles, s);
        default: return row_launch_mt<MODE, 8>(a, tiles, s);
    }
}

static inline bool al16(const void* p) { return ((uintptr_t)p & 15) == 0; }

static int linear_residual_layernorm_fwd_impl(const void* a, int64_t lda, const void* w, int64_t ldw, const float* bias,
                                             const float* residual, int64_t ldr, const float* row_scale, float* y, int64_t ldy,
                                             const float* gamma, const float* beta, float eps, void* h, int64_t ldh, float* mean,
                                             float* rstd, int64_t M, int64_t N, int64_t K, void* stream) {
    if (!a || !w || !residual || !y || M <= 0 || N <= 0 || K <= 0 || lda < K || ldw < K || ldr < N || ldy < N) return VITED_ERR_BAD_ARG;
    if (h && (!gamma || !beta || !mean || !rstd || ldh < N)) return VITED_ERR_BAD_ARG;
    if (!row_shape_ok(M, N, K)) return VITED_ERR_UNSUPPORTED;
    if ((lda & 7) || (ldw & 7) || (ldr & 3) || (ldy & 3) || (h && (ldh & 3))) return VITED_ERR_UNSUPPORTED;
    if (!al16(a) || !al16(w) || !al16(residual) || !al16(y) || !al16(bias) || !al16(gamma) || !al16(beta) || ((uintptr_t)h & 7))
        return VITED_ERR_BAD_ARG;
    RowArgs r = {};
    r.A = (const bf16*)a; r.lda = lda; r.seg_k = (int)K; r.seg_stride = 0; r.W = (const bf16*)w; r.ldw = ldw; r.M = M; r.K = (int)K;
    r.bias = bias; r.residual = residual; r.ldr = ldr; r.y = y; r.ldy = ldy;
    r.gamma = gamma; r.beta = beta; r.eps = eps; r.h = (bf16*)h; r.ldh = ldh; r.mean = mean; r.rstd = rstd;
    r.row_scale = row_scale;
    return row_launch<ROW_MODE_FWD>(r, (hipStream_t)stream);
}

extern "C" int vited_linear_residual_layernorm_fwd(const void* a, int64_t lda, const void* w, int64_t ldw, const float* bias,
                                                   const float* residual, int64_t ldr, float* y, int64_t ldy, const float* gamma,
                                                   const float* beta, float eps, void* h, int64_t ldh, float* mean, float* rstd,
                                                   int64_t M, int64_t N, int64_t K, void* stream) {
    return linear_residual_layernorm_fwd_impl(a, lda, w, ldw, bias, residual, ldr, nullptr, y, ldy, gamma, beta, eps, h, ldh, mean, rstd,
                                              M, N, K, stream);
}

extern "C" int vited_linear_residual_layernorm_fwd_scaled(const void* a, int64_t lda, const void* w, int64_t ldw, const float* bias,
                                                          const float* residual, int64_t ldr, const float* row_scale, float* y,
                                                          int64_t ldy, const float* gamma, const float* beta, float eps, void* h,
                                                          int64_t ldh, float* mean, float* rstd, int64_t M, int64_t N, int64_t K,
                                                          void* stream) {
    return linear_residual_layernorm_fwd_impl(a, lda, w, ldw, bias, residual, ldr, row_scale, y, ldy, gamma, beta, eps, h, ldh, mean,
                                              rstd, M, N, K, stream);
}

int ln_bwd_finish(const float* partial, int nparts, int dim, float* dgamma, float* dbeta, int accumulate, hipStream_t s);

extern "C" int64_t vited_linear_layernorm_bwd_partial_rows(int64_t M) { return M >= 1 ? row_tiles(M) : 0; }

extern "C" int64_t vited_linear_layernorm_bwd_workspace_bytes(int64_t M, int64_t N) {
    return N == ROW_N && M >= 1 ? row_tiles(M) * 2 * ROW_N * (int64_t)sizeof(float) : 0;
}

static int linear_layernorm_bwd_impl(const void* dy, int64_t lddy, int64_t seg_k, int64_t seg_stride, const void* wt, int64_t ldwt,
                                    const float* x, int64_t ldx, const float* gamma, const float* mean, const float* rstd,
                                    const float* dx_in, int64_t dx_in_ld, float* dx_out, int64_t dx_out_ld, void* dx_lp, int64_t dx_lp_ld,
                                    const float* lp_scale, float* dgamma, float* dbeta, int accumulate, int64_t M, int64_t N, int64_t K,
                                    float* workspace, int64_t workspace_bytes, void* stream) {
    if (lp_scale && !dx_lp) return VITED_ERR_BAD_ARG;
    if (!dy || !wt || !x || !gamma || !mean || !rstd || !dx_out || M <= 0 || N <= 0 || K <= 0) return VITED_ERR_BAD_ARG;
    if ((dgamma == nullptr) != (dbeta == nullptr)) return VITED_ERR_BAD_ARG;
    if (seg_k <= 0 || K % seg_k || lddy < seg_k || ldwt < K || ldx < N || dx_out_ld < N || (dx_in && dx_in_ld < N) || (dx_lp && dx_lp_ld < N))
        return VITED_ERR_BAD_ARG;
    if (!row_shape_ok(M, N, K) || seg_k % 64 || (seg_stride & 7)) return VITED_ERR_UNSUPPORTED;
    if ((lddy & 7) || (ldwt & 7) || (ldx & 3) || (dx_out_ld & 3) || (dx_in && (dx_in_ld & 3)) || (dx_lp && (dx_lp_ld & 3))) return VITED_ERR_UNSUPPORTED;
    if (!al16(dy) || !al16(wt) || !al16(x) || !al16(gamma) || !al16(dx_in) || !al16(dx_out) || ((uintptr_t)dx_lp & 7)) return VITED_ERR_BAD_ARG;
    if (!workspace || workspace_bytes < vited_linear_layernorm_bwd_workspace_bytes(M, N)) return VITED_ERR_WORKSPACE;
    RowArgs r = {};
    r.A = (const bf16*)dy; r.lda = lddy; r.seg_k = (int)seg_k; r.seg_stride = seg_stride; r.W = (const bf16*)wt; r.ldw = ldwt; r.M = M; r.K = (int)K;
    r.gamma = gamma; r.x = x; r.ldx = ldx; r.mean_in = mean; r.rstd_in = rstd;
    r.dx_in = dx_in; r.ldxi = dx_in_ld; r.dx = dx_out; r.lddx = dx_out_ld; r.dx_lp = (bf16*)dx_lp; r.ldlp = dx_lp_ld;
    r.partial = workspace;
    r.lp_scale = lp_scale;
    const int rc = row_launch<ROW_MODE_BWD>(r, (hipStream_t)stream);
    if (rc != VITED_OK || !dgamma) return rc;
    return ln_bwd_finish(workspace, (int)row_tiles(M), ROW_N, dgamma, dbeta, accumulate, (hipStream_t)stream);
}

extern "C" int vited_linear_layernorm_bwd(const void* dy, int64_t lddy, const void* wt, int64_t ldwt, const float* x, int64_t ldx,
                                          const float* gamma, const float* mean, const float* rstd, const float* dx_in,
                                          int64_t dx_in_ld, float* dx_out, int64_t dx_out_ld, void* dx_lp, int64_t dx_lp_ld,
                                          float* dgamma, float* dbeta, int accumulate, int64_t M, int64_t N, int64_t K,
                                          float* workspace, int64_t workspace_bytes, void* stream) {
    return linear_layernorm_bwd_impl(dy, lddy, K, 0, wt, ldwt, x, ldx, gamma, mean, rstd, dx_in, dx_in_ld, dx_out, dx_out_ld, dx_lp, dx_lp_ld,
                                     nullptr, dgamma, dbeta, accumulate, M, N, K, workspace, workspace_bytes, stream);
}

extern "C" int vited_linear_layernorm_bwd_segmented(const void* dy, int64_t lddy, int64_t seg_k, int64_t seg_stride, int64_t segments,
                                                    const void* wt, int64_t ldwt, const float* x, int64_t ldx, const float* gamma,
                                                    const float* mean, const float* rstd, const float* dx_in, int64_t dx_in_ld,
                                                    float* dx_out, int64_t dx_out_ld, void* dx_lp, int64_t dx_lp_ld, float* dgamma,
                                                    float* dbeta, int accumulate, int64_t M, int64_t N, float* workspace,
                                                    int64_t workspace_bytes, void* stream) {
    if (segments <= 0) return VITED_ERR_BAD_ARG;
    return linear_layernorm_bwd_impl(dy, lddy, seg_k, seg_stride, wt, ldwt, x, ldx, gamma, mean, rstd, dx_in, dx_in_ld, dx_out, dx_out_ld, dx_lp,
                                     dx_lp_ld, nullptr, dgamma, dbeta, accumulate, M, N, segments * seg_k, workspace, workspace_bytes, stream);
}

extern "C" int vited_linear_layernorm_bwd_scaled(const void* dy, int64_t lddy, const void* wt, int64_t ldwt, const float* x, int64_t ldx,
                                                 const float* gamma, const float* mean, const float* rstd, const float* dx_in,
                                                 int64_t dx_in_ld, float* dx_out, int64_t dx_out_ld, void* dx_lp, int64_t dx_lp_ld,
                                                 const float* lp_scale, float* dgamma, float* dbeta, int accumulate, int64_t M, int64_t N,
                                                 int64_t K, float* workspace, int64_t workspace_bytes, void* stream) {
    return linear_layernorm_bwd_impl(dy, lddy, K, 0, wt, ldwt, x, ldx, gamma, mean, rstd, dx_in, dx_in_ld, dx_out, dx_out_ld, dx_lp, dx_lp_ld,
                                     lp_scale, dgamma, dbeta, accumulate, M, N, K, workspace, workspace_bytes, stream);
}
```

### vit-ed_amd/functions.py

```python
from __future__ import annotations

import contextlib
import os
from collections import namedtuple

import torch

from . import ops
from ._lib import (B_KN, B_NK, EPI_GELU_GRAD, EPI_MUL, EPI_RESIDUAL, EPI_STORE, EPI_STORE_F32)

LN_EPS = 1e-6


def _bundle(name, table):
    fields, keys = zip(*(pair.split('=') for pair in table.split()))
    return namedtuple(name, fields), keys


_ATTN = 'g1=norm1.weight b1=norm1.bias wqkv=attn.qkv.weight bqkv=attn.qkv.bias wproj=attn.proj.weight bproj=attn.proj.bias '
_CROSS = ('gc=norm_cross.weight bc=norm_cross.bias gx=norm_context.weight bx=norm_context.bias wq=cross_attn.q.weight '
          'bq=cross_attn.q.bias wkv=cross_attn.kv.weight bkv=cross_attn.kv.bias wcp=cross_attn.proj.weight bcp=cross_attn.proj.bias ')
_MLP = 'g2=norm2.weight b2=norm2.bias w1=mlp.fc1.weight bb1=mlp.fc1.bias w2=mlp.fc2.weight bb2=mlp.fc2.bias'
_PATCH = 'pw=patch_embed.proj.weight pb=patch_embed.proj.bias pos=pos_embed '
EncBlock, ENC_BLOCK_KEYS = _bundle('EncBlock', _ATTN + _MLP)
# ... 212 lines not shown
        ops.linear_bwd_weight(dy, x_saved, want_bias=b is not None, dw_out=gw.view(gw.shape[0], -1), db_out=gb)
        return None, None
    dw, db = ops.linear_bwd_weight(dy, x_saved)
    return dw.view_as(w), (db if b is not None else None)


class _DwBatch:

    ROUND = 256

    def __init__(self, rt, kind=None):
        self.rt, self.blocks, self.kind = rt, rt.group_dw, kind

    def __enter__(self):
        self.outer = self.rt.dw_queue
        self.rt.dw_queue = [] if (self.rt.batch_dw and not self.rt.exact) else None
        self.mark = 0
        return self

    @contextlib.contextmanager
    def block(self):
        yield
        self._end_of_block()

    @staticmethod
    def _tiles(items):
        return sum(-(-dy.shape[1] // 128) * (x.shape[1] // 384) for dy, x, _dw, _db, _a in items)

    def _end_of_block(self):
        q = self.rt.dw_queue
        if q is None:
            return
        if not self.blocks:
            self.flush()
            return
        this, count = self._tiles(q[self.mark:]), len(q) - self.mark
        self.mark = len(q)
        if self._tiles(q) + this > self.ROUND or len(q) + count > ops.MAX_BATCHED_WEIGHT_GRADS:
            self.flush()

    def flush(self):
        q = self.rt.dw_queue
        if not q:
            return
        self.rt.dw_queue, self.mark = [], 0
        with _BlockSpan(self.rt, self.kind, len(q), 'dw'):
            for acc in (True, False):
                _launch_weight_grads([(dy, x, dw, db) for dy, x, dw, db, a in q if a == acc], acc)

    def __exit__(self, exc_type, *exc):
        if exc_type is None:
            self.flush()
        self.rt.dw_queue = self.outer
        return False


def _launch_weight_grads(items, accumulate):
    for i in range(0, len(items), ops.MAX_BATCHED_WEIGHT_GRADS):
        part = items[i: i + ops.MAX_BATCHED_WEIGHT_GRADS]
        if len(part) > 1 and ops.linear_bwd_weight_batched(part, accumulate):
            continue
        for dy, x, dw, db in part:
            if accumulate:
                ops.linear_bwd_weight(dy, x, want_bias=db is not None, dw_out=dw, db_out=db)
                continue
            got_w, got_b = ops.linear_bwd_weight(dy, x, want_bias=db is not None)
            dw.copy_(got_w)
            if db is not None:
                db.copy_(got_b)


def _linear_bwd(rt, dy, x_saved, w, b=None, aux=None):
    wt, layout = rt.weight_t(w)
    if aux is not None:
        dx = ops.gemm(dy, wt, b_layout=layout, epilogue=EPI_MUL, aux=aux)
    else:
        dx = ops.gemm(dy, wt, b_layout=layout)
    dw, db = _weight_grads(rt, dy, x_saved, w, b)
    return dx, dw, db


def _row_kernel_ok(rt, m, n, k, dtype, *rowwise):
    return (rt.fused_ln and not rt.exact and ops.linear_layernorm_supported(m, n, k, dtype)
            and all(t is None or (t.dim() == 2 and t.stride(1) == 1 and t.stride(0) % 4 == 0) for t in rowwise))


def _res_linear(rt, a, w, bias, residual, ln=None, scale=None):
    wsh = rt.weight(w)
    if ln is not None and _row_kernel_ok(rt, a.shape[0], wsh.shape[0], a.shape[1], a.dtype, a, residual):
        y, h, mean, rstd = ops.linear_residual_layernorm_fwd(a, wsh, bias, residual, ln[0], ln[1], LN_EPS, row_scale=scale)
        return y, (h, mean, rstd)
    y = ops.gemm(a, wsh, epilogue=EPI_RESIDUAL, bias=bias, residual=residual, row_scale=scale)
    return y, (ops.layernorm_fwd(y, ln[0], ln[1], LN_EPS, rt.act_dtype) if ln is not None else None)


def _linear_ln_bwd(rt, dy, h_saved, w, bias, x, gamma, beta, mean, rstd, dx_in=None, dx_out=None, want_lp=True, lp_scale=None):
    want_lp = want_lp and not rt.exact
    wt, layout = rt.weight_t(w)
    if layout == B_NK and _row_kernel_ok(rt, dy.shape[0], wt.shape[0], dy.shape[1], dy.dtype, dy, x, dx_in, dx_out):
        gg, gb = _gtarget(rt, gamma), _gtarget(rt, beta)
        direct = gg is not None and gb is not None
        dx, dx_lp, dg, db = ops.linear_layernorm_bwd(dy, wt, x, gamma, mean, rstd, dx_in=dx_in, dx_out=dx_out, want_lp=want_lp,
                                                     dgamma=gg if direct else None, dbeta=gb if direct else None, defer=rt.ln_queue,
                                                     lp_scale=lp_scale)
        if direct:
            dg = db = None
    else:
        dh = ops.gemm(dy, wt, b_layout=layout)
        dx, dx_lp, dg, db = _ln_bwd(rt, dh, x, gamma, beta, mean, rstd, dx_in=dx_in, dx_out=dx_out, want_lp=want_lp, lp_scale=lp_scale,
                                    lp_dtype=rt.act_dtype)
    dw, dbias = _weight_grads(rt, dy, h_saved, w, bias)
    return dx, (dx if rt.exact and lp_scale is None else dx_lp), dg, db, dw, dbias


@contextlib.contextmanager
def _ln_sums(rt):
    rt.ln_queue = [] if not rt.exact else None
    try:
        yield
        ops.layernorm_bwd_finish(rt.ln_queue)
    finally:
        rt.ln_queue = None


def _keep_attention(rt, key, q, k):
    b, nq, d = q.shape
    qh = q.float().reshape(b, nq, rt.heads, rt.head_dim).transpose(1, 2)
    kh = k.float().reshape(b, k.shape[1], rt.heads, rt.head_dim).transpose(1, 2)
    rt.attn_store.setdefault(key, {})['attn'] = torch.softmax((qh * rt.scale) @ kh.transpose(-2, -1), dim=-1)


def _keep_attention_grad(rt, key, do, v):
    b, nq, d = do.shape
    doh = do.float().reshape(b, nq, rt.heads, rt.head_dim).transpose(1, 2)
    vh = v.float().reshape(b, v.shape[1], rt.heads, rt.head_dim).transpose(1, 2)
    rt.attn_store.setdefault(key, {})['grad'] = doh @ vh.transpose(-2, -1)


def _keep_attention_cam(rt, key, q, k, v, do, lse):
    ent = rt.attn_store.setdefault(key, {})
    ent['cam'] = ops.attention_cam(q, k, v, do, lse, rt.heads, rt.scale, mode='grad')
    if key == ('cross_blocks', rt.c_depth - 1, 'cross_attn'):
        ent['cam_operands'] = (q, k, v, do, lse)


def _cam_only(rt, grads):
    return [None] * len(grads) if rt.keep_cam else grads


def _self_attn_fwd(rt, h, wqkv, bqkv, batch, n, key=None):
    d = rt.dim
    qkv = ops.gemm(h, rt.weight(wqkv), bias=bqkv)
    qkv3 = qkv.view(batch, n, 3 * d)
    o, lse = ops.attention_fwd(qkv3[:, :, 0:d], qkv3[:, :, d:2 * d], qkv3[:, :, 2 * d:3 * d], rt.heads, rt.scale)
    if rt.keep_attn and key is not None:
        _keep_attention(rt, key, qkv3[:, :, 0:d], qkv3[:, :, d:2 * d])
    return qkv, o.view(batch * n, d), lse


def _self_attn_bwd(rt, do, qkv, o, lse, batch, n, key=None):
    d = rt.dim
    qkv3 = qkv.view(batch, n, 3 * d)
    if rt.keep_attn and key is not None:
        _keep_attention_grad(rt, key, do.view(batch, n, d), qkv3[:, :, 2 * d:3 * d])
    if rt.keep_cam and key is not None:
        _keep_attention_cam(rt, key, qkv3[:, :, 0:d], qkv3[:, :, d:2 * d], qkv3[:, :, 2 * d:3 * d], do.view(batch, n, d), lse)
    dqkv = torch.empty_like(qkv)
    dqkv3 = dqkv.view(batch, n, 3 * d)
    ops.attention_bwd(qkv3[:, :, 0:d], qkv3[:, :, d:2 * d], qkv3[:, :, 2 * d:3 * d], o.view(batch, n, d),
                      do.view(batch, n, d), lse, rt.heads, rt.scale, dqkv3[:, :, 0:d], dqkv3[:, :, d:2 * d],
                      dqkv3[:, :, 2 * d:3 * d])
    return dqkv


FUSED_MLP_TILE = 128
FUSED_MLP_CUS = 256


def _fused_mlp_rows(rt, x, w1, grad):
    if grad or rt.exact or not rt.fused_mlp or x.shape[1] != 384 or tuple(w1.shape) != (1536, 384) or x.stride(0) != 384:
        return 0
    tiles = x.shape[0] // FUSED_MLP_TILE
    rem = tiles % FUSED_MLP_CUS
    if tiles >= FUSED_MLP_CUS and rem < FUSED_MLP_CUS // 4:
        tiles -= rem
    elif x.shape[0] % FUSED_MLP_TILE:
        tiles += 1
    return min(tiles * FUSED_MLP_TILE, x.shape[0])


def _hand_over_ln(rt, x, P, grad):
    return grad or not _fused_mlp_rows(rt, x, P.w1, grad)


def _mlp_fwd(rt, x, P, grad=True, ln=None, next_ln=None, scale=None):
    g, b, w1, b1, w2, b2 = P.g2, P.b2, P.w1, P.bb1, P.w2, P.bb2
    rows = _fused_mlp_rows(rt, x, w1, grad) if ln is None and scale is None else 0
    if rows:
        y = torch.empty_like(x)
        ops.mlp_fwd(x[:rows], g, b, rt.weight(w1), b1, rt.weight(w2), b2, LN_EPS, save=False, out=(y[:rows], None, None, None, None, None))
        if rows < x.shape[0]:
            xt = x[rows:]
            ht, _, _ = ops.layernorm_fwd(xt, g, b, LN_EPS, rt.act_dtype)
            _, ut = ops.gemm(ht, rt.weight(w1), epilogue=EPI_GELU_GRAD, bias=b1)
            ops.gemm(ut, rt.weight(w2), epilogue=EPI_RESIDUAL, bias=b2, residual=xt, out=y[rows:])
        nxt = ops.layernorm_fwd(y, next_ln[0], next_ln[1], LN_EPS, rt.act_dtype) if next_ln is not None else None
        return y, None, nxt
    h, mean, rstd = ln if ln is not None else ops.layernorm_fwd(x, g, b, LN_EPS, rt.act_dtype)
    gd, u = ops.gemm(h, rt.weight(w1), epilogue=EPI_GELU_GRAD, bias=b1)
    y, nxt = _res_linear(rt, u, w2, b2, x, next_ln, scale)
    return y, (mean, rstd, h, gd, u), nxt


def _mlp_bwd(rt, dy, dy_lp, x, P, saved, lp_scale=None):
    mean, rstd, h, gd, u = saved
    dz, dw2, dbb2 = _linear_bwd(rt, dy_lp, u, P.w2, P.bb2, aux=gd)
    dx, dx_lp, dg2, db2, dw1, dbb1 = _linear_ln_bwd(rt, dz, h, P.w1, P.bb1, x, P.g2, P.b2, mean, rstd, dx_in=dy, lp_scale=lp_scale)
    return dx, dx_lp, dict(g2=dg2, b2=db2, w1=dw1, bb1=dbb1, w2=dw2, bb2=dbb2)


def _attn_branch_fwd(rt, x, P, batch, n, key=None, ln=None, next_ln=None, scale=None):
    h, mean, rstd = ln if ln is not None else ops.layernorm_fwd(x, P.g1, P.b1, LN_EPS, rt.act_dtype)
    qkv, o, lse = _self_attn_fwd(rt, h, P.wqkv, P.bqkv, batch, n, key)
    y, nxt = _res_linear(rt, o, P.wproj, P.bproj, x, next_ln, scale)
    return y, (mean, rstd, h, qkv, o, lse), nxt


def _attn_branch_bwd(rt, dy, dy_lp, x, P, saved, batch, n, key=None, lp_scale=None):
    mean, rstd, h, qkv, o, lse = saved
    do, dwproj, dbproj = _linear_bwd(rt, dy_lp, o, P.wproj, P.bproj)
    dqkv = _self_attn_bwd(rt, do, qkv, o, lse, batch, n, key)
    dx, dx_lp, dg1, db1, dwqkv, dbqkv = _linear_ln_bwd(rt, dqkv, h, P.wqkv, P.bqkv, x, P.g1, P.b1, mean, rstd, dx_in=dy, lp_scale=lp_scale)
    return dx, dx_lp, dict(g1=dg1, b1=db1, wqkv=dwqkv, bqkv=dbqkv, wproj=dwproj, bproj=dbproj)


def _patch_tokens_fwd(rt, img, S, with_cls, batch_index=None):
    patches = ops.patchify(img, rt.patch_size, rt.act_dtype, batch_index, mean=rt.input_mean, std=rt.input_std)
    batch = patches.shape[0] // rt.n1
    pos2 = S.pos.view(rt.n2, rt.dim)
    rows, first = (rt.n2, 1) if with_cls else (rt.n1, 0)
    x = ops.gemm(patches, rt.weight(S.pw), epilogue=EPI_RESIDUAL, bias=S.pb, residual=pos2[1 - first:], rows_per_batch=rt.n1,
                 out_rows_per_batch=rows, row_offset=first, residual_bcast=True, out_rows=batch * rows)
    if with_cls:
        ops.write_cls_row(x.view(batch, rt.n2, rt.dim), S.cls.view(-1), pos2)
    return x, patches, batch, rows


def _patch_tokens_bwd(rt, dx, patches, S, with_cls, batch):
    rows = rt.n2 if with_cls else rt.n1
    dx3 = dx.view(batch, rows, rt.dim)
    dpos_rows = ops.sum_rows(dx3.view(batch, rows * rt.dim)).view(rows, rt.dim)
    dpos = torch.zeros_like(S.pos)
    grads = dict(pos=dpos)
    if with_cls:
        dpos[0] = dpos_rows
        grads['cls'] = dpos_rows[0].clone().view_as(S.cls)
        dtok = ops.slice_rows_cast(dx3, 1, rt.n1, rt.act_dtype)
    else:
        dpos[0, 1:] = dpos_rows
        dtok = dx if rt.exact else ops.cast(dx, rt.act_dtype)
    grads['pw'], grads['pb'] = _weight_grads(rt, dtok, patches, S.pw, S.pb)
    return grads


def _norm1_of(blocks, i):
    return (blocks[i].g1, blocks[i].b1) if i < len(blocks) else None


class EncoderFn(torch.autograd.Function):
    @staticmethod
    def forward(ctx, rt: Runtime, img, *params):
        shared, blocks = split_params(params, EncShared, EncBlock)
        grad = any(ctx.needs_input_grad)
        x, patches, batch, n = _patch_tokens_fwd(rt, img, shared, with_cls=False)
        drop = _take_drop_rows(rt, 0, len(blocks), 2, batch, n, x.device)
        tape = []
        ln1 = None
        for i, P in enumerate(blocks):
            s_attn, s_mlp = drop.block(i) if drop is not None else (None, None)
            chain = _hand_over_ln(rt, x, P, grad or s_mlp is not None)
            with _BlockSpan(rt, 'enc', i, 'fwd'):
                xa, sa, ln2 = _attn_branch_fwd(rt, x, P, batch, n, key=('blocks', i, 'attn'), ln=ln1, next_ln=(P.g2, P.b2) if chain else None,
                                               scale=s_attn)
                xb, sm, ln1 = _mlp_fwd(rt, xa, P, grad, ln=ln2, next_ln=_norm1_of(blocks, i + 1) if chain else None, scale=s_mlp)
            if grad:
                tape.append((x, sa, xa, sm))
            x = xb
            if rt.tap is not None:
                rt.tap[f'enc.x.{len(tape) - 1 if grad else 0}'] = x.clone()
        if grad:
            ctx.rt, ctx.tape, ctx.patches, ctx.batch, ctx.params = rt, tape, patches, batch, (shared, blocks)
            ctx.drop = drop
        return x.view(batch, n, rt.dim)

    @staticmethod
    def backward(ctx, dout):
        rt, batch, n = ctx.rt, ctx.batch, ctx.rt.n1
        shared, blocks = ctx.params
        dx = dout.contiguous().view(batch * n, rt.dim).float()
        drop = ctx.drop
        scale_of = (lambda i, j: drop.get(i, j)) if drop is not None else (lambda i, j: None)
        dx_lp = _lp_scaled(rt, dx, scale_of(len(blocks) - 1, 1))
        gblocks = [None] * len(blocks)
        with _ln_sums(rt), _DwBatch(rt, kind='enc') as dwg:
            for i in reversed(range(len(blocks))):
                x, sa, xa, sm = ctx.tape[i]
                ctx.tape[i] = None
                with _BlockSpan(rt, 'enc', i, 'bwd'), dwg.block():
                    dx, dx_lp, gm = _mlp_bwd(rt, dx, dx_lp, xa, blocks[i], sm, lp_scale=scale_of(i, 0))
                    dx, dx_lp, ga = _attn_branch_bwd(rt, dx, dx_lp, x, blocks[i], sa, batch, n, key=('blocks', i, 'attn'),
                                                     lp_scale=scale_of(i - 1, 1))
                if rt.tap is not None:
                    rt.tap[f'enc.dx.{i}'] = dx.clone()
                gblocks[i] = EncBlock(**ga, **gm)
        gshared = EncShared(**_patch_tokens_bwd(rt, dx, ctx.patches, shared, with_cls=False, batch=batch))
        ctx.tape = ctx.patches = ctx.drop = None
        return (None, None, *_cam_only(rt, flatten_params(gshared, gblocks)))


def _dense_rows(t):
    out = torch.empty(t.shape, dtype=t.dtype, device=t.device)
    out.copy_(t)
    return out


def _dec_self_fwd(rt, x, P, batch, n, cls_only, key=None, ln1=None, fuse_ln=True, scale=None):
    next_ln = (P.gc, P.bc) if fuse_ln else None
    if not cls_only:
        return _attn_branch_fwd(rt, x, P, batch, n, key=key, ln=ln1, next_ln=next_ln, scale=scale)
    d = rt.dim
    h1, m1, r1 = ln1 if ln1 is not None else ops.layernorm_fwd(x, P.g1, P.b1, LN_EPS, rt.act_dtype)
    qkv = ops.gemm(h1, rt.weight(P.wqkv), bias=P.bqkv)
    qkv3 = qkv.view(batch, n, 3 * d)
    o0, lse0 = ops.attention_fwd(qkv3[:, 0:1, 0:d], qkv3[:, :, d:2 * d], qkv3[:, :, 2 * d:3 * d], rt.heads, rt.scale)
    o0 = o0.view(batch, d)
    x0 = _dense_rows(x.view(batch, n, d)[:, 0, :])
    xa, lnq = _res_linear(rt, o0, P.wproj, P.bproj, x0, next_ln, scale)
    return xa, (m1, r1, h1, qkv, o0, lse0), lnq


def _dec_self_bwd(rt, dx, dx_lp, x, P, saved, batch, n, cls_only, key=None, lp_scale=None):
    if not cls_only:
        return _attn_branch_bwd(rt, dx, dx_lp, x, P, saved, batch, n, key=key, lp_scale=lp_scale)
    d = rt.dim
    m1, r1, h1, qkv, o0, lse0 = saved
    do0, dwproj, dbproj = _linear_bwd(rt, dx_lp, o0, P.wproj, P.bproj)
    qkv3 = qkv.view(batch, n, 3 * d)
    dqkv = torch.zeros_like(qkv)
    dqkv3 = dqkv.view(batch, n, 3 * d)
    ops.attention_bwd(qkv3[:, 0:1, 0:d], qkv3[:, :, d:2 * d], qkv3[:, :, 2 * d:3 * d], o0.view(batch, 1, d), do0.view(batch, 1, d),
                      lse0, rt.heads, rt.scale, dqkv3[:, 0:1, 0:d], dqkv3[:, :, d:2 * d], dqkv3[:, :, 2 * d:3 * d])
    dres = torch.zeros((batch * n, d), dtype=torch.float32, device=dx.device)
    dres.view(batch, n, d)[:, 0, :].copy_(dx)
    dx, dx_lp, dg1, db1, dwqkv, dbqkv = _linear_ln_bwd(rt, dqkv, h1, P.wqkv, P.bqkv, x, P.g1, P.b1, m1, r1, dx_in=dres, lp_scale=lp_scale)
    return dx, dx_lp, dict(g1=dg1, b1=db1, wqkv=dwqkv, bqkv=dbqkv, wproj=dwproj, bproj=dbproj)


def _cross_q(rt, xa, P, lnq=None):
    hq, mq, rq = lnq if lnq is not None else ops.layernorm_fwd(xa, P.gc, P.bc, LN_EPS, rt.act_dtype)
    return ops.gemm(hq, rt.weight(P.wq), bias=P.bq), (hq, mq, rq)


def _dec_cross_fwd(rt, xa, P, batch, lnq=None, q=None, kv3=None, ctxf=None, kv_index=None, key=None, fuse_ln=True, scale=None, items=None):
    d, nq = rt.dim, xa.shape[0] // batch
    hq = mq = rq = hc = mc = rc = None
    if q is None:
        q, (hq, mq, rq) = _cross_q(rt, xa, P, lnq)
    kv = kv3
    if kv3 is None:
        hc, mc, rc = ops.layernorm_fwd(ctxf, P.gx, P.bx, LN_EPS, rt.act_dtype)
        kv = ops.gemm(hc, rt.weight(P.wkv), bias=P.bkv)
        kv3 = kv.view(batch if items is None else items, rt.n1, 2 * d)
    oc, lse_c = ops.attention_fwd(q.view(batch, nq, d), kv3[:, :, 0:d], kv3[:, :, d:2 * d], rt.heads, rt.scale, kv_index=kv_index)
    if rt.keep_attn and key is not None:
        _keep_attention(rt, key, q.view(batch, nq, d), kv3[:, :, 0:d])
    oc = oc.view(batch * nq, d)
    xb, ln2 = _res_linear(rt, oc, P.wcp, P.bcp, xa, (P.g2, P.b2) if fuse_ln else None, scale)
    return xb, (mq, rq, hq, mc, rc, hc, q, kv, oc, lse_c), ln2


def _dec_cross_bwd(rt, dx, dx_lp, xa, P, saved, ctxf, dctx, batch, index, dkv3=None, lp_scale=None, seg=None):
    d, nq = rt.dim, xa.shape[0] // batch
    items = batch if seg is None else seg.items
    mq, rq, hq, mc, rc, hc, q, kv, oc, lse_c = saved
    doc, dwcp, dbcp = _linear_bwd(rt, dx_lp, oc, P.wcp, P.bcp)
    dq = torch.empty_like(q)
    folded = hc is None
    if folded:
        kv3, dkv = kv, dkv3
    else:
        dkv = torch.empty_like(kv)
        kv3, dkv3 = kv.view(items, rt.n1, 2 * d), dkv.view(items, rt.n1, 2 * d)
    if rt.keep_attn:
        _keep_attention_grad(rt, ('cross_blocks', index, 'cross_attn'), doc.view(batch, nq, d), kv3[:, :, d:2 * d])
    if rt.keep_cam:
        _keep_attention_cam(rt, ('cross_blocks', index, 'cross_attn'), q.view(batch, nq, d), kv3[:, :, 0:d], kv3[:, :, d:2 * d],
                            doc.view(batch, nq, d), lse_c)
    ops.attention_bwd(q.view(batch, nq, d), kv3[:, :, 0:d], kv3[:, :, d:2 * d], oc.view(batch, nq, d),
                      doc.view(batch, nq, d), lse_c, rt.heads, rt.scale, dq.view(batch, nq, d), dkv3[:, :, 0:d],
                      dkv3[:, :, d:2 * d], segments=seg)
    if rt.tap is not None:
        i = index
        rt.tap[f'dec.doc.{i}'], rt.tap[f'dec.dq.{i}'], rt.tap[f'dec.dkv.{i}'] = doc.clone(), dq.clone(), dkv.clone()
        rt.tap[f'dec.q.{i}'], rt.tap[f'dec.kv.{i}'], rt.tap[f'dec.oc.{i}'] = q.clone(), kv.clone(), oc.clone()
    dx, dx_lp, dgc, dbc, dwq, dbq = _linear_ln_bwd(rt, dq, hq, P.wq, P.bq, xa, P.gc, P.bc, mq, rq, dx_in=dx, lp_scale=lp_scale)
    dgx = dbx = dwkv = dbkv = None
    if not folded:
        dctx, _, dgx, dbx, dwkv, dbkv = _linear_ln_bwd(rt, dkv, hc, P.wkv, P.bkv, ctxf, P.gx, P.bx, mc, rc, dx_in=dctx, dx_out=dctx, want_lp=False)
    return dx, dx_lp, dctx, dict(gc=dgc, bc=dbc, gx=dgx, bx=dbx, wq=dwq, bq=dbq, wkv=dwkv, bkv=dbkv, wcp=dwcp, bcp=dbcp)


def _dec_block_fwd(rt, x, ctxf, P, batch, n, grad, cls_only, index=0, ln1=None, next_ln=None, kv3=None, scales=(None, None, None),
                   seg=None):
    xa, sa, lnq = _dec_self_fwd(rt, x, P, batch, n, cls_only, key=('cross_blocks', index, 'attn'), ln1=ln1, scale=scales[0])
    xb, sc, ln2 = _dec_cross_fwd(rt, xa, P, batch, lnq=lnq, kv3=kv3, ctxf=ctxf, key=('cross_blocks', index, 'cross_attn'),
                                 fuse_ln=_hand_over_ln(rt, xa, P, grad or scales[2] is not None), scale=scales[1],
                                 kv_index=seg.index if seg is not None else None, items=seg.items if seg is not None else None)
    xc, sm, nxt = _mlp_fwd(rt, xb, P, grad, ln=ln2, next_ln=next_ln, scale=scales[2])
    return xc, ((x, sa, xa, sc, xb, sm) if grad else None), nxt


def _dec_block_bwd(rt, dx, dx_lp, ctxf, dctx, P, entry, batch, n, cls_only, index, dkv3=None, lp_scales=(None, None, None), seg=None):
    x, sa, xa, sc, xb, sm = entry
    dx, dx_lp, gm = _mlp_bwd(rt, dx, dx_lp, xb, P, sm, lp_scale=lp_scales[0])
    dx, dx_lp, dctx, gc = _dec_cross_bwd(rt, dx, dx_lp, xa, P, sc, ctxf, dctx, batch, index, dkv3, lp_scale=lp_scales[1], seg=seg)
    dx, dx_lp, ga = _dec_self_bwd(rt, dx, dx_lp, x, P, sa, batch, n, cls_only, key=('cross_blocks', index, 'attn'), lp_scale=lp_scales[2])
    return dx, dx_lp, dctx, DecBlock(**ga, **gc, **gm)


@torch.no_grad()
def image2_tokens(rt: Runtime, img, params):
    shared, blocks = split_params(params, DecShared, DecBlock)
    x, _, batch, _ = _patch_tokens_fwd(rt, img, shared, with_cls=True)
    if not blocks or (rt.cls_tail and rt.c_depth == 1):
        return x.view(batch, rt.n2, rt.dim), None
    xa, _, lnq = _dec_self_fwd(rt, x, blocks[0], batch, rt.n2, cls_only=False)
    q, _ = _cross_q(rt, xa, blocks[0], lnq)
# ... 188 lines not shown
```

### vit-ed_amd/ops.py

```python
from __future__ import annotations

import ctypes as C
from typing import NamedTuple

import torch

from . import _lib
from ._lib import (B_KN, B_NK, BF16, EPI_GELU, EPI_GELU_GRAD, EPI_MUL, EPI_MUL_GELU_GRAD, EPI_RESIDUAL, EPI_STORE, EPI_STORE_F32, F16,
                   F32, I32, I64)

_DTYPE = {torch.float32: F32, torch.bfloat16: BF16, torch.float16: F16, torch.int32: I32, torch.int64: I64}
_FLOATS = (torch.float32, torch.bfloat16, torch.float16)


def _code(dtype: torch.dtype) -> int:
    if dtype not in (torch.float32, torch.bfloat16):
        raise TypeError(f'vited ops support float32 and bfloat16 activations, got {dtype}')
    return _DTYPE[dtype]


def _need_gpu(*tensors):
    for t in tensors:
        if t is not None and not t.is_cuda:
            raise RuntimeError('vited ops run on the MI355X HIP kernels only: got a CPU tensor '
# ... 185 lines not shown


def hisfrag_windows_u8(store: torch.Tensor, img_off: torch.Tensor, img_hw: torch.Tensor, image: torch.Tensor, flags: torch.Tensor,
                       afix: torch.Tensor, minv: torch.Tensor, origin: torch.Tensor, img_size: int,
                       out: torch.Tensor | None = None) -> torch.Tensor:
    _need_gpu(store, img_off, img_hw, image, flags, afix, minv, origin, out)
    s, n, b = int(img_size), _store_args(store, img_off, img_hw), image.numel()
    _batch_args(b, (image, torch.int32, ()), (flags, torch.int32, ()), (afix, torch.int64, (6,)), (minv, torch.float64, (6,)),
                (origin, torch.int32, (2,)))
    if out is None:
        out = torch.empty((b, 3, s, s), dtype=torch.uint8, device=store.device)
    assert out.dtype == torch.uint8 and tuple(out.shape) == (b, 3, s, s) and out.is_contiguous()
    _lib.call('vited_hisfrag_windows_u8', _ptr(store), _ptr(img_off), _ptr(img_hw), n, _ptr(image), _ptr(flags), _ptr(afix), _ptr(minv),
              _ptr(origin), _ptr(out), b, s, _stream())
    return out


def hisfrag_jitter_u8(img: torch.Tensor, flags: torch.Tensor, order: torch.Tensor, factors: torch.Tensor, hue: torch.Tensor,
                      out: torch.Tensor | None = None) -> torch.Tensor:
    _need_gpu(img, flags, order, factors, hue, out)
    b, s, out = _crop_args(img, out, in_place=True)
    _batch_args(b, (flags, torch.int32, ()), (order, torch.int32, (4,)), (factors, torch.float32, (3,)), (hue, torch.int32, ()))
    sums = torch.empty(b, dtype=torch.int64, device=img.device)
    _lib.call('vited_hisfrag_jitter_u8', _ptr(img), _ptr(flags), _ptr(order), _ptr(factors), _ptr(hue), _ptr(sums), _ptr(out), b, s, _stream())
    return out


def hisfrag_blur_u8(img: torch.Tensor, flags: torch.Tensor, weights: torch.Tensor, out: torch.Tensor | None = None) -> torch.Tensor:
    _need_gpu(img, flags, weights, out)
    b, s, out = _crop_args(img, out, in_place=False)
    _batch_args(b, (flags, torch.int32, ()), (weights, torch.float32, (2,)))
    _lib.call('vited_hisfrag_blur_u8', _ptr(img), _ptr(flags), _ptr(weights), _ptr(out), b, s, _stream())
    return out


def michigan_windows_u8(store: torch.Tensor, img_off: torch.Tensor, img_hw: torch.Tensor, image: torch.Tensor, flags: torch.Tensor,
                        origin: torch.Tensor, x0: torch.Tensor, kx: torch.Tensor, y0: torch.Tensor, ky: torch.Tensor, holes: torch.Tensor,
                        n_holes: torch.Tensor, img_size: int, out: torch.Tensor | None = None) -> torch.Tensor:
    _need_gpu(store, img_off, img_hw, image, flags, origin, x0, kx, y0, ky, holes, n_holes, out)
    s, n, b = int(img_size), _store_args(store, img_off, img_hw), image.numel()
    i32 = torch.int32
    _batch_args(b, (image, i32, ()), (flags, i32, ()), (origin, i32, (2,)), (x0, i32, (s,)), (kx, i32, (s, 3)), (y0, i32, (s,)),
                (ky, i32, (s, 3)), (holes, i32, (16, 4)), (n_holes, i32, ()))
    if out is None:
        out = torch.empty((b, 3, s, s), dtype=torch.uint8, device=store.device)
    assert out.dtype == torch.uint8 and tuple(out.shape) == (b, 3, s, s) and out.is_contiguous()
    _lib.call('vited_michigan_windows_u8', _ptr(store), _ptr(img_off), _ptr(img_hw), n, _ptr(image), _ptr(flags), _ptr(origin), _ptr(x0),
              _ptr(kx), _ptr(y0), _ptr(ky), _ptr(holes), _ptr(n_holes), _ptr(out), b, s, _stream())
    return out


def michigan_blur_gray_u8(img: torch.Tensor, flags: torch.Tensor, weights: torch.Tensor, out: torch.Tensor | None = None) -> torch.Tensor:
    _need_gpu(img, flags, weights, out)
    b, s, out = _crop_args(img, out, in_place=False)
    _batch_args(b, (flags, torch.int32, ()), (weights, torch.int32, (2,)))
    _lib.call('vited_michigan_blur_gray_u8', _ptr(img), _ptr(flags), _ptr(weights), _ptr(out), b, s, _stream())
    return out


def slice_rows_cast(x: torch.Tensor, row_offset: int, rows: int, dtype: torch.dtype) -> torch.Tensor:
    _need_gpu(x)
    assert x.dtype == torch.float32 and x.dim() == 3 and x.is_contiguous()
    b, r, d = x.shape
    out = torch.empty((b * rows, d), dtype=dtype, device=x.device)
    _lib.call('vited_slice_rows_cast', _ptr(x), _ptr(out), _code(dtype), b, r, row_offset, rows, d, _stream())
    return out


def write_cls_row(x: torch.Tensor, cls: torch.Tensor, pos: torch.Tensor):
    _need_gpu(x, cls, pos)
    assert x.dtype == torch.float32 and x.is_contiguous() and x.dim() == 3
    b, r, d = x.shape
    _lib.call('vited_write_cls_row', _ptr(x), _ptr(cls), _ptr(pos), b, r, d, _stream())


def sum_rows(x: torch.Tensor) -> torch.Tensor:
    _need_gpu(x)
    ld = _rows2d(x)
    b, w = x.shape
    out = torch.empty(w, dtype=torch.float32, device=x.device)
    ws = _scratch(_lib.load().vited_sum_rows_workspace_bytes(b, w), x.device)
    _lib.call('vited_sum_rows', _ptr(x), _code(x.dtype), ld, _ptr(out), b, w, *ws, _stream())
    return out


def layernorm_fwd(x: torch.Tensor, gamma: torch.Tensor, beta: torch.Tensor, eps: float, out_dtype: torch.dtype, out=None):
    _need_gpu(x, gamma, beta)
    assert x.dtype == torch.float32 and gamma.dtype == torch.float32 and beta.dtype == torch.float32
    ld = _rows2d(x)
    rows, dim = x.shape
    if out is not None:
        y, mean, rstd = out
        assert y.shape == (rows, dim) and y.dtype == out_dtype and _rows2d(y) == dim and mean.numel() == rows and rstd.numel() == rows
    else:
        y = torch.empty((rows, dim), dtype=out_dtype, device=x.device)
        mean = torch.empty(rows, dtype=torch.float32, device=x.device)
        rstd = torch.empty(rows, dtype=torch.float32, device=x.device)
    _lib.call('vited_layernorm_fwd', _ptr(x), ld, _ptr(gamma), _ptr(beta), _ptr(y), _code(out_dtype), dim, _ptr(mean), _ptr(rstd), rows,
              dim, float(eps), _stream())
    return y, mean, rstd


def layernorm_bwd(dy, x, gamma, mean, rstd, dx_in=None, dx_out=None, want_lp: bool = False, dx_lp=None, dgamma=None,
                  dbeta=None, lp_scale=None, lp_dtype=torch.bfloat16):
    _need_gpu(dy, x, gamma, mean, rstd, dx_in, dx_out, dx_lp, lp_scale)
    dy_ld, x_ld = _rows2d(dy), _rows2d(x)
    rows, dim = x.shape
    assert dy.shape == x.shape and x.dtype == torch.float32
    if dx_out is None:
        dx_out = torch.empty((rows, dim), dtype=torch.float32, device=x.device)
    if lp_scale is not None:
        _check_row_scale(lp_scale, rows)
        want_lp = True
    else:
        lp_dtype = torch.bfloat16
    if want_lp and dx_lp is None:
        dx_lp = torch.empty((rows, dim), dtype=lp_dtype, device=x.device)
    assert dx_lp is None or dx_lp.dtype == lp_dtype
    if dx_in is not None:
        assert dx_in.dtype == torch.float32 and dx_in.shape == x.shape
    accumulate = dgamma is not None
    if accumulate:
        assert dbeta is not None and dgamma.dtype == dbeta.dtype == torch.float32 and dgamma.is_contiguous() and dbeta.is_contiguous()
    else:
        dgamma = torch.empty(dim, dtype=torch.float32, device=x.device)
        dbeta = torch.empty(dim, dtype=torch.float32, device=x.device)
    ws = _scratch(_lib.load().vited_layernorm_bwd_workspace_bytes(rows, dim), x.device)
    head = (_ptr(dy), _code(dy.dtype), dy_ld, _ptr(x), x_ld, _ptr(gamma), _ptr(mean), _ptr(rstd),
            _ptr(dx_in), _rows2d(dx_in) if dx_in is not None else 0, _ptr(dx_out), _rows2d(dx_out),
            _ptr(dx_lp), _code(lp_dtype), _rows2d(dx_lp) if dx_lp is not None else 0)
    tail = (_ptr(dgamma), _ptr(dbeta), int(accumulate), rows, dim, *ws, _stream())
    if lp_scale is not None:
        _lib.call('vited_layernorm_bwd_scaled', *head, _ptr(lp_scale), *tail)
    else:
        _lib.call('vited_layernorm_bwd', *head, *tail)
    return dx_out, dx_lp, dgamma, dbeta


def gemm(a: torch.Tensor, b: torch.Tensor, *, b_layout: int = B_NK, epilogue: int = EPI_STORE, bias=None, aux=None,
         residual=None, out=None, out2=None, rows_per_batch: int = 0, out_rows_per_batch: int = 0, row_offset: int = 0,
         residual_bcast: bool = False, out_rows: int | None = None, row_scale=None):
    _need_gpu(a, b, bias, aux, residual, out)
    assert a.dtype == b.dtype, f'operand dtypes differ: {a.dtype} vs {b.dtype}'
    lda, ldb = _rows2d(a), _rows2d(b)
    m, k = a.shape
    n = b.shape[0] if b_layout == B_NK else b.shape[1]
    kb = b.shape[1] if b_layout == B_NK else b.shape[0]
    if kb != k:
        raise ValueError(f'contraction mismatch: A is [{m},{k}], B gives K={kb}')
    f32_out = epilogue in (EPI_RESIDUAL, EPI_STORE_F32)
    if out is None:
        rows = m if out_rows is None else out_rows
        out = torch.empty((rows, n), dtype=torch.float32 if f32_out else a.dtype, device=a.device)
    ldo = _rows2d(out)
    if epilogue in (EPI_GELU, EPI_GELU_GRAD):
        if out2 is None:
            out2 = torch.empty_like(out)
        assert out2.dtype == out.dtype and out2.shape == out.shape and _rows2d(out2) == ldo
    else:
        out2 = None
    if aux is not None:
        assert aux.dtype == a.dtype and _rows2d(aux) == ldo
    if residual is not None:
        assert residual.dtype == torch.float32 and residual.stride(-1) == 1
        assert residual.stride(-2) == ldo if residual.dim() >= 2 else True
    if bias is not None:
# ... 10 lines not shown
    _lib.call('vited_gemm', _ptr(a), lda, _ptr(b), ldb, b_layout, _code(a.dtype), m, n, k, epilogue, _ptr(bias), _ptr(aux), _ptr(residual),
              _ptr(out), _ptr(out2), ldo, rows_per_batch, out_rows_per_batch, row_offset, int(bool(residual_bcast)), _stream())
    return (out, out2) if epilogue in (EPI_GELU, EPI_GELU_GRAD) else out


def linear_bwd_weight(dy: torch.Tensor, x: torch.Tensor, want_bias: bool = True, dw_out=None, db_out=None):
    _need_gpu(dy, x)
    assert dy.dtype == x.dtype and dy.shape[0] == x.shape[0]
    lddy, ldx = _rows2d(dy), _rows2d(x)
    m, n = dy.shape
    k = x.shape[1]
    accumulate = dw_out is not None
    if accumulate:
        assert dw_out.dtype == torch.float32 and dw_out.is_contiguous() and dw_out.numel() == n * k
        dw, db = dw_out, (db_out if want_bias else None)
        assert db is None or (db.dtype == torch.float32 and db.is_contiguous() and db.numel() == n)
    else:
        dw = torch.empty((n, k), dtype=torch.float32, device=x.device)
        db = torch.empty(n, dtype=torch.float32, device=x.device) if want_bias else None
    ws = _scratch(_lib.load().vited_linear_bwd_weight_workspace_bytes(m, n, k), x.device)
    _lib.call('vited_linear_bwd_weight', _ptr(dy), lddy, _ptr(x), ldx, _code(x.dtype), m, n, k, _ptr(dw), _ptr(db), int(accumulate), *ws,
              _stream())
    return dw, db


MAX_BATCHED_WEIGHT_GRADS = 40


def linear_bwd_weight_batched(items, accumulate: bool) -> bool:
    n = len(items)
    if n < 1 or n > MAX_BATCHED_WEIGHT_GRADS:
        return False
    for dy, x, dw, db in items:
        _need_gpu(dy, x, dw, db)
        if dy.dtype != torch.bfloat16 or x.dtype != torch.bfloat16 or dy.shape[0] != x.shape[0]:
            return False
        assert dw.dtype == torch.float32 and dw.is_contiguous() and dw.numel() == dy.shape[1] * x.shape[1]
        assert db is None or (db.dtype == torch.float32 and db.is_contiguous() and db.numel() == dy.shape[1])
        if dw.data_ptr() % 16 or (db is not None and db.data_ptr() % 16) or dy.data_ptr() % 16 or x.data_ptr() % 16:
            return False
    dys, xs, dws, dbs = zip(*items)
    M = _host_array(C.c_int64, [dy.shape[0] for dy in dys])
    N = _host_array(C.c_int64, [dy.shape[1] for dy in dys])
    K = _host_array(C.c_int64, [x.shape[1] for x in xs])
    lib = _lib.load()
    if not lib.vited_linear_bwd_weight_batched_supported(n, M, N, K, BF16):
        return False
    lddy, ldx = _host_array(C.c_int64, map(_rows2d, dys)), _host_array(C.c_int64, map(_rows2d, xs))
    ws = _scratch(lib.vited_linear_bwd_weight_batched_workspace_bytes(n, M, N, K), dys[0].device)
    _lib.call('vited_linear_bwd_weight_batched', n, _host_array(C.c_void_p, dys), lddy, _host_array(C.c_void_p, xs), ldx, M, N, K,
              _host_array(C.c_void_p, dws), _host_array(C.c_void_p, dbs), BF16, int(bool(accumulate)), *ws, _stream())
    return True


def linear_layernorm_supported(m: int, n: int, k: int, dtype: torch.dtype) -> bool:
    return dtype == torch.bfloat16 and bool(_lib.load().vited_linear_layernorm_supported(int(m), int(n), int(k)))


def linear_residual_layernorm_fwd(a, w, bias, residual, gamma=None, beta=None, eps: float = 1e-6, out=None, row_scale=None):
    _need_gpu(a, w, bias, residual, gamma, beta, out, row_scale)
    assert a.dtype == w.dtype == torch.bfloat16 and residual.dtype == torch.float32
    lda, ldw, ldr = _rows2d(a), _rows2d(w), _rows2d(residual)
    m, k = a.shape
    n = w.shape[0]
    assert w.shape[1] == k and residual.shape == (m, n)
    y = out if out is not None else torch.empty((m, n), dtype=torch.float32, device=a.device)
    assert y.dtype == torch.float32 and y.shape == (m, n)
    h = mean = rstd = None
    if gamma is not None:
        h = torch.empty((m, n), dtype=torch.bfloat16, device=a.device)
        mean = torch.empty(m, dtype=torch.float32, device=a.device)
        rstd = torch.empty(m, dtype=torch.float32, device=a.device)
    tail = (_ptr(y), _rows2d(y), _ptr(gamma), _ptr(beta), float(eps), _ptr(h), n, _ptr(mean), _ptr(rstd), m, n, k, _stream())
    if row_scale is not None:
        _check_row_scale(row_scale, m)
        _lib.call('vited_linear_residual_layernorm_fwd_scaled', _ptr(a), lda, _ptr(w), ldw, _ptr(bias), _ptr(residual), ldr, _ptr(row_scale),
                  *tail)
    else:
        _lib.call('vited_linear_residual_layernorm_fwd', _ptr(a), lda, _ptr(w), ldw, _ptr(bias), _ptr(residual), ldr, *tail)
    return y, h, mean, rstd


def linear_layernorm_bwd(dy, wt, x, gamma, mean, rstd, dx_in=None, dx_out=None, want_lp: bool = False, dgamma=None, dbeta=None,
                         defer=None, lp_scale=None):
    _need_gpu(dy, wt, x, gamma, mean, rstd, dx_in, dx_out, lp_scale)
    assert dy.dtype == wt.dtype == torch.bfloat16 and x.dtype == torch.float32
    segments = 1
    if dy.dim() == 3:
        assert dy.stride(2) == 1 and dy.stride(0) % 8 == 0
        segments, m, seg_k = dy.shape
        lddy, seg_stride, k = dy.stride(1), dy.stride(0), segments * seg_k
    else:
        lddy = _rows2d(dy)
        m, k = dy.shape
    ldwt, ldx = _rows2d(wt), _rows2d(x)
    n = wt.shape[0]
    assert wt.shape[1] == k and x.shape == (m, n)
    lib = _lib.load()
    if dx_out is None:
        dx_out = torch.empty((m, n), dtype=torch.float32, device=x.device)
    if lp_scale is not None:
        _check_row_scale(lp_scale, m)
        assert segments == 1
        want_lp = True
    dx_lp = torch.empty((m, n), dtype=torch.bfloat16, device=x.device) if want_lp else None
    accumulate = dgamma is not None
    if accumulate:
        assert dbeta is not None and dgamma.dtype == dbeta.dtype == torch.float32 and dgamma.is_contiguous() and dbeta.is_contiguous()
    else:
        dgamma = torch.empty(n, dtype=torch.float32, device=x.device)
        dbeta = torch.empty(n, dtype=torch.float32, device=x.device)
    if defer is not None:
        rows = int(lib.vited_linear_layernorm_bwd_partial_rows(m))
        part = torch.empty(rows * 2 * n, dtype=torch.float32, device=x.device)
        defer.append((part, rows, dgamma, dbeta, accumulate))
        ws = (part.data_ptr(), part.numel() * 4)
    else:
        ws = _scratch(lib.vited_linear_layernorm_bwd_workspace_bytes(m, n), x.device)
    dx_args = (_ptr(x), ldx, _ptr(gamma), _ptr(mean), _ptr(rstd), _ptr(dx_in), _rows2d(dx_in) if dx_in is not None else 0, _ptr(dx_out),
               _rows2d(dx_out), _ptr(dx_lp), n)
    sum_args = (0 if defer is not None else _ptr(dgamma), 0 if defer is not None else _ptr(dbeta), int(accumulate))
    tail = dx_args + sum_args
    if lp_scale is not None:
        _lib.call('vited_linear_layernorm_bwd_scaled', _ptr(dy), lddy, _ptr(wt), ldwt, *dx_args, _ptr(lp_scale), *sum_args, m, n, k, *ws,
                  _stream())
    elif segments > 1:
        _lib.call('vited_linear_layernorm_bwd_segmented', _ptr(dy), lddy, seg_k, seg_stride, segments, _ptr(wt), ldwt, *tail, m, n, *ws,
                  _stream())
    else:
        _lib.call('vited_linear_layernorm_bwd', _ptr(dy), lddy, _ptr(wt), ldwt, *tail, m, n, k, *ws, _stream())
    return dx_out, dx_lp, dgamma, dbeta


def layernorm_bwd_finish(entries):
    if not entries:
        return
    parts, rows, dgammas, dbetas, accumulate = zip(*entries)
    _lib.call('vited_layernorm_bwd_finish_batched', len(entries), _host_array(C.c_void_p, parts), _host_array(C.c_int, rows),
              _host_array(C.c_void_p, dgammas), _host_array(C.c_void_p, dbetas), _host_array(C.c_int, map(int, accumulate)),
              dgammas[0].numel(), _stream())
    entries.clear()


MAX_FOLDED_BLOCKS = 16


def fold_context_weights(ws, biases, gammas, betas, out=None):
    n_blk = len(ws)
    _need_gpu(*ws, *gammas, *betas)
    n, k = ws[0].shape
    dev = ws[0].device
    if out is None:
        out = (torch.empty((n_blk * n, k), dtype=torch.bfloat16, device=dev), torch.empty((k, n_blk * n), dtype=torch.bfloat16, device=dev),
               torch.empty(n_blk * n, dtype=torch.float32, device=dev))
    for t in list(ws) + list(gammas) + list(betas):
        assert t.dtype == torch.float32 and t.is_contiguous()
    _lib.call('vited_fold_context_weights', n_blk, *(_host_array(C.c_void_p, ts) for ts in (ws, biases, gammas, betas)), n, k,
              _ptr(out[0]), _ptr(out[1]), _ptr(out[2]), _stream())
    return out


def unfold_context_grads(dwf, dbf, ws, gammas, betas, dws, dbiases, dgammas, dbetas, accumulate: bool):
    n_blk = len(ws)
    n, k = ws[0].shape
    assert dwf.dtype == dbf.dtype == torch.float32 and dwf.is_contiguous() and dbf.is_contiguous()
    assert dwf.shape == (n_blk * n, k) and dbf.numel() == n_blk * n
    _lib.call('vited_unfold_context_grads', n_blk, _ptr(dwf), _ptr(dbf),
              *(_host_array(C.c_void_p, ts) for ts in (ws, gammas, betas, dws, dbiases, dgammas, dbetas)), n, k, int(bool(accumulate)),
              _stream())


def mlp_fwd(x, gamma, beta, w1, b1, w2, b2, eps: float, save: bool = True, out=None):
    _need_gpu(x, gamma, beta, w1, b1, w2, b2)
    assert x.dtype == torch.float32 and w1.dtype == w2.dtype == torch.bfloat16 and w1.is_contiguous() and w2.is_contiguous()
    ldx = _rows2d(x)
    rows, dim = x.shape
    hidden = w1.shape[0]
    assert w1.shape == (hidden, dim) and w2.shape == (dim, hidden)
    dev = x.device
    if out is not None:
        y, mean, rstd, h, gd, u = out
    else:
        y = torch.empty((rows, dim), dtype=torch.float32, device=dev)
        mean = rstd = h = gd = u = None
        if save:
            mean = torch.empty(rows, dtype=torch.float32, device=dev)
            rstd = torch.empty(rows, dtype=torch.float32, device=dev)
            h = torch.empty((rows, dim), dtype=torch.bfloat16, device=dev)
            gd = torch.empty((rows, hidden), dtype=torch.bfloat16, device=dev)
            u = torch.empty((rows, hidden), dtype=torch.bfloat16, device=dev)
    if save:
        assert h.is_contiguous() and gd.is_contiguous() and u.is_contiguous() and h.shape == (rows, dim) and gd.shape == u.shape == (rows, hidden)
    _lib.call('vited_mlp_fwd', _ptr(x), ldx, _ptr(gamma), _ptr(beta), _ptr(w1), _ptr(b1), _ptr(w2), _ptr(b2), _ptr(y), _rows2d(y),
              _ptr(h) if save else 0, _ptr(gd) if save else 0, _ptr(u) if save else 0, _ptr(mean) if save else 0, _ptr(rstd) if save else 0,
              rows, dim, hidden, float(eps), _stream())
    return y, ((mean, rstd, h, gd, u) if save else None)


def block_fwd(x, heads: int, ln1_g, ln1_b, wqkv, bqkv, wproj, bproj, ln2_g, ln2_b, w1, b1, w2, b2, eps: float = 1e-6):
    _need_gpu(x, wqkv, wproj, w1, w2)
    assert x.dtype == torch.float32 and x.dim() == 3 and x.is_contiguous()
    assert all(t.dtype == torch.bfloat16 and t.is_contiguous() for t in (wqkv, wproj, w1, w2))
    b, n, d = x.shape
    hidden = w1.shape[0]
    y = torch.empty_like(x)
    ws, nbytes = _scratch(_lib.load().vited_block_workspace_bytes(b, n, d, hidden, heads) + 256, x.device)
# ... 57 lines not shown
    def items(self) -> int:
        return self.offsets.numel() - 1

    def to(self, device):
        return self if self.index.device == torch.device(device) else PairSegments(*(t.to(device) for t in self))


def pair_segments(index: torch.Tensor, items: int) -> PairSegments:
    items = int(items)
    if index.dim() != 1 or index.dtype.is_floating_point or index.dtype == torch.bool:
        raise ValueError(f'pair_segments: expected a 1-D integer index, got {index.dtype} {tuple(index.shape)}')
    if items < 0 or (items == 0 and index.numel()):
        raise ValueError(f'pair_segments: {index.numel()} pairs over {items} items')
    index = index.to(torch.int64).contiguous()
    if index.numel() and bool(((index < 0) | (index >= items)).any()):
        raise ValueError(f'pair_segments: index outside [0, {items}): min {int(index.min())}, max {int(index.max())}')
    order = torch.argsort(index, stable=True)
    offsets = torch.zeros(items + 1, dtype=torch.int64, device=index.device)
    if items:
        offsets[1:] = torch.cumsum(torch.bincount(index, minlength=items), 0)
    return PairSegments(index, order, offsets)


MINE_MAX_CAPACITY = 24576


def mine_pairs_max_images() -> int:
    return int(_lib.load().vited_mine_pairs_max_images())


def _mine_pairs_args(targets, keys, neg_per_pos, capacity):
    for name, t, dtype in (('targets', targets, torch.int64), ('keys', keys, torch.float32)):
        if not torch.is_tensor(t) or t.dtype != dtype or t.dim() != 1:
            raise ValueError(f'mine_pairs: {name} must be a 1-D {dtype} tensor, got '
                             f'{(t.dtype, tuple(t.shape)) if torch.is_tensor(t) else type(t).__name__}')
        if not t.is_contiguous():
            raise ValueError(f'mine_pairs: {name} must be contiguous, got strides {t.stride()}')
    n = targets.numel()
    if n < 1:
        raise ValueError('mine_pairs: no images')
    if keys.numel() != n * n:
        raise ValueError(f'mine_pairs: {keys.numel()} keys for {n} images, expected one per ordered cell: {n * n}')
    if keys.device != targets.device:
        raise ValueError(f'mine_pairs: keys on {keys.device}, targets on {targets.device}')
    neg_per_pos, capacity = float(neg_per_pos), int(capacity)
    if not 0.0 <= neg_per_pos < float('inf'):
        raise ValueError(f'mine_pairs: neg_per_pos must be a finite number >= 0, got {neg_per_pos}')
    if capacity < 1:
        raise ValueError(f'mine_pairs: capacity must be at least 1, got {capacity}')
    if not targets.is_cuda:
        raise ValueError('mine_pairs: the kernel takes device tensors (engine.mine_pairs_device restates the rule for CPU tensors)')
    if n > mine_pairs_max_images():
        raise ValueError(f'mine_pairs: {n} images, the kernel takes at most {mine_pairs_max_images()}')
    if capacity > MINE_MAX_CAPACITY:
        raise ValueError(f'mine_pairs: capacity {capacity} above the {MINE_MAX_CAPACITY} rows the kernel supports')
    return n, neg_per_pos, capacity


def mine_pairs_out(targets, keys, neg_per_pos, ordered_negatives, groups, labels, weights, seg_index, seg_order, seg_offsets, counts):
    n, neg_per_pos, capacity = _mine_pairs_args(targets, keys, neg_per_pos, groups.shape[0] if torch.is_tensor(groups) and groups.dim() else 0)
    for name, t, dtype, shape in (('groups', groups, torch.int64, (capacity, 2)), ('labels', labels, torch.float32, (capacity, 1)),
                                  ('weights', weights, torch.float32, (capacity, 1)), ('seg_index', seg_index, torch.int64, (capacity,)),
                                  ('seg_order', seg_order, torch.int64, (capacity,)), ('seg_offsets', seg_offsets, torch.int64, (n + 1,)),
                                  ('counts', counts, torch.int32, (5,))):
        if not torch.is_tensor(t) or t.dtype != dtype or tuple(t.shape) != shape or not t.is_contiguous() or t.device != targets.device:
            raise ValueError(f'mine_pairs: {name} must be a contiguous {dtype} tensor of shape {shape} on {targets.device}')
    _lib.call('vited_mine_pairs', _ptr(targets), n, _ptr(keys), neg_per_pos, int(bool(ordered_negatives)), capacity, _ptr(groups),
              _ptr(labels), _ptr(weights), _ptr(seg_index), _ptr(seg_order), _ptr(seg_offsets), _ptr(counts), _stream())


def mine_pairs(targets: torch.Tensor, keys: torch.Tensor, neg_per_pos: float, ordered_negatives: bool, capacity: int):
    n, neg_per_pos, capacity = _mine_pairs_args(targets, keys, neg_per_pos, capacity)
    dev = targets.device
    groups = torch.empty((capacity, 2), dtype=torch.int64, device=dev)
    labels = torch.empty((capacity, 1), dtype=torch.float32, device=dev)
    weights = torch.empty((capacity, 1), dtype=torch.float32, device=dev)
    seg_index, seg_order = (torch.empty(capacity, dtype=torch.int64, device=dev) for _ in range(2))
    seg_offsets = torch.empty(n + 1, dtype=torch.int64, device=dev)
    counts = torch.empty(5, dtype=torch.int32, device=dev)
    mine_pairs_out(targets, keys, neg_per_pos, ordered_negatives, groups, labels, weights, seg_index, seg_order, seg_offsets, counts)
    return groups, labels, weights, PairSegments(seg_index, seg_order, seg_offsets), counts


def attention_bwd(q, k, v, o, do, lse, heads: int, scale: float, dq, dk, dv, kv_index=None, segments=None):
    _need_gpu(q, k, v, o, do, lse, dq, dk, dv)
    b, nq, d = q.shape
    nk = k.shape[1]
    hd = d // heads
    assert o.is_contiguous() and do.is_contiguous() and o.dtype == do.dtype == q.dtype
    if segments is None and kv_index is not None:
        segments = pair_segments(kv_index, k.shape[0])
    if segments is not None:
        return _attention_bwd_indexed(q, k, v, o, do, lse, heads, scale, dq, dk, dv, kv_index, segments)
    q_bs, q_ts = _head_view(q, heads, hd)
    k_bs, k_ts = _head_view(k, heads, hd)
    v_bs, v_ts = _head_view(v, heads, hd)
    dq_bs, dq_ts = _head_view(dq, heads, hd)
    dk_bs, dk_ts = _head_view(dk, heads, hd)
    dv_bs, dv_ts = _head_view(dv, heads, hd)
    delta = torch.empty((b, heads, nq), dtype=torch.float32, device=q.device)
    _lib.call('vited_attention_bwd',
              _ptr(q), q_bs, q_ts, _ptr(k), k_bs, k_ts, _ptr(v), v_bs, v_ts, _ptr(o), _ptr(do), nq * d, d, _ptr(lse), _ptr(delta),
              _ptr(dq), dq_bs, dq_ts, _ptr(dk), dk_bs, dk_ts, _ptr(dv), dv_bs, dv_ts, _code(q.dtype), b, heads, nq, nk, hd,
              float(scale), _stream())
    return dq, dk, dv


def _attention_bwd_indexed(q, k, v, o, do, lse, heads, scale, dq, dk, dv, kv_index, seg):
    if not isinstance(seg, PairSegments):
        raise TypeError(f'attention_bwd: segments must be a PairSegments (ops.pair_segments), got {type(seg).__name__}')
    b, nq, d = q.shape
    items, nk = k.shape[0], k.shape[1]
    hd = d // heads
    if kv_index is not None and kv_index is not seg.index and not torch.equal(kv_index.to(seg.index.device), seg.index):
        raise ValueError('attention_bwd: kv_index and segments.index differ')
    for name, t, size in (('index', seg.index, b), ('order', seg.order, b), ('offsets', seg.offsets, items + 1)):
        if t.dtype != torch.int64 or t.dim() != 1 or t.numel() != size or not t.is_contiguous() or t.device != q.device:
            raise ValueError(f'attention_bwd: segments.{name} must be a contiguous int64 [{size}] tensor on {q.device}, got {t.dtype} '
                             f'{tuple(t.shape)} on {t.device} ({b} pairs over {items} key/value items)')
    assert q.dtype == k.dtype == v.dtype == dq.dtype == dk.dtype == dv.dtype
    assert k.shape == v.shape == dk.shape == dv.shape and k.shape[2] == d and dq.shape == q.shape
    q_bs, q_ts = _head_view(q, heads, hd)
    k_bs, k_ts = _head_view(k, heads, hd)
    v_bs, v_ts = _head_view(v, heads, hd)
    dq_bs, dq_ts = _head_view(dq, heads, hd)
    dk_bs, dk_ts = _head_view(dk, heads, hd)
    dv_bs, dv_ts = _head_view(dv, heads, hd)
    delta = torch.empty((b, heads, nq), dtype=torch.float32, device=q.device)
    nbytes = _lib.load().vited_attention_bwd_indexed_workspace_bytes(_code(q.dtype), b, heads, nk, hd)
    if nbytes < 0:
        raise ValueError(f'attention_bwd: empty operands (B {b}, heads {heads}, Nk {nk}, head_dim {hd})')
    ws, ws_bytes = _scratch(nbytes + 16, q.device)
    base = (ws + 15) // 16 * 16
    _lib.call('vited_attention_bwd_indexed',
              _ptr(q), q_bs, q_ts, _ptr(k), k_bs, k_ts, _ptr(v), v_bs, v_ts, _ptr(seg.index), _ptr(seg.order), _ptr(seg.offsets), items,
              _ptr(o), _ptr(do), nq * d, d, _ptr(lse), _ptr(delta), _ptr(dq), dq_bs, dq_ts, _ptr(dk), dk_bs, dk_ts, _ptr(dv), dv_bs, dv_ts,
              _code(q.dtype), b, heads, nq, nk, hd, float(scale), base, ws_bytes - (base - ws), _stream())
    return dq, dk, dv


CAM_GRAD, CAM_PROB = 0, 1
_CAM_MODES = {'grad': CAM_GRAD, 'prob': CAM_PROB, CAM_GRAD: CAM_GRAD, CAM_PROB: CAM_PROB}


def _cam_operand(name, t, heads, like=None):
    if t.dim() != 3 or t.stride(2) != 1 or t.shape[2] % heads:
        raise ValueError(f'attention_cam: {name} must be [B, N, heads*head_dim] with a dense last dim, got shape {tuple(t.shape)} '
                         f'stride {t.stride()} for {heads} heads')
    if like is not None and (t.dtype != like.dtype or t.device != like.device or t.shape[0] != like.shape[0] or t.shape[2] != like.shape[2]):
        raise ValueError(f'attention_cam: {name} {tuple(t.shape)} {t.dtype} does not match q {tuple(like.shape)} {like.dtype}')
    return t.stride(0), t.stride(1)


def attention_cam(q, k, v, do, lse, heads: int, scale: float, *, mode, head_weight=None, out=None):
    if mode not in _CAM_MODES:
        raise ValueError(f"attention_cam: mode must be 'grad' or 'prob', got {mode!r}")
    mode = _CAM_MODES[mode]
    if mode == CAM_GRAD and (v is None or do is None):
        raise ValueError("attention_cam: mode='grad' needs v and do")
    if mode == CAM_GRAD and head_weight is not None:
        raise ValueError("attention_cam: head_weight belongs to mode='prob'")
    if mode == CAM_PROB:
        v = do = None
    _need_gpu(q, k, v, do, lse, head_weight, out)
    if heads <= 0:
        raise ValueError(f'attention_cam: heads must be positive, got {heads}')
    q_bs, q_ts = _cam_operand('q', q, heads)
    k_bs, k_ts = _cam_operand('k', k, heads, q)
    v_bs, v_ts = _cam_operand('v', v, heads, q) if v is not None else (0, 0)
    do_bs, do_ts = _cam_operand('do', do, heads, q) if do is not None else (0, 0)
    b, nq, d = q.shape
    nk = k.shape[1]
    if v is not None and v.shape[1] != nk:
        raise ValueError(f'attention_cam: v has {v.shape[1]} tokens, k has {nk}')
    if do is not None and do.shape[1] != nq:
        raise ValueError(f'attention_cam: do has {do.shape[1]} tokens, q has {nq}')
    if b == 0 or nq == 0 or nk == 0:
        raise ValueError(f'attention_cam: empty operands (B {b}, Nq {nq}, Nk {nk})')
    if lse.dtype != torch.float32 or tuple(lse.shape) != (b, heads, nq) or not lse.is_contiguous():
        raise ValueError(f'attention_cam: lse must be contiguous float32 [{b}, {heads}, {nq}], got {tuple(lse.shape)} {lse.dtype}')
    if head_weight is not None and (head_weight.dtype != torch.float32 or tuple(head_weight.shape) != (b, heads) or not head_weight.is_contiguous()):
        raise ValueError(f'attention_cam: head_weight must be contiguous float32 [{b}, {heads}], got {tuple(head_weight.shape)} {head_weight.dtype}')
    if out is None:
        out = torch.empty((b, nq, nk), dtype=torch.float32, device=q.device)
    elif (out.dtype != torch.float32 or out.dim() != 3 or out.shape[0] != b or out.shape[1] != nq or out.shape[2] < nk or out.stride(2) != 1
          or out.stride(1) < nk or out.device != q.device):
# ... 194 lines not shown
```

Baseline: 43870.

## Fuse patch-grad prep, periodic residual LN bwd, dq zero-fill, and vectorized patchify

```diff
diff --git a/include/vited.h b/include/vited.h
--- a/include/vited.h
+++ b/include/vited.h
@@ -84,6 +84,10 @@
 int64_t vited_sum_rows_workspace_bytes(int64_t batch, int64_t width);
 int vited_sum_rows(const void* in, int in_dtype, int64_t in_ld, float* out, int64_t batch, int64_t width,
                    float* workspace, int64_t workspace_bytes, void* stream);
+
+int64_t vited_patch_grad_prep_workspace_bytes(int64_t batch, int64_t rows, int64_t dim);
+int vited_patch_grad_prep(const float* dx, int64_t batch, int64_t rows, int64_t dim, int64_t first, void* tok, int tok_dtype,
+                          float* dpos, float* dcls, int accumulate, float* workspace, int64_t workspace_bytes, void* stream);
 
 
 int vited_layernorm_fwd(const float* x, int64_t x_ld, const float* gamma, const float* beta, void* y,
@@ -162,6 +166,12 @@
                                       const float* lp_scale, float* dgamma, float* dbeta, int accumulate, int64_t M, int64_t N,
                                       int64_t K, float* workspace, int64_t workspace_bytes, void* stream);
 
+int vited_linear_layernorm_bwd_periodic(const void* dy, int64_t lddy, const void* wt, int64_t ldwt, const float* x, int64_t ldx,
+                                        const float* gamma, const float* mean, const float* rstd, const float* dx_in,
+                                        int64_t dx_in_ld, int64_t dx_in_period, float* dx_out, int64_t dx_out_ld, void* dx_lp,
+                                        int64_t dx_lp_ld, const float* lp_scale, float* dgamma, float* dbeta, int accumulate,
+                                        int64_t M, int64_t N, int64_t K, float* workspace, int64_t workspace_bytes, void* stream);
+
 int vited_fold_context_weights(int count, const float* const* w, const float* const* bias, const float* const* gamma,
                                const float* const* beta, int64_t N, int64_t K, void* w_out, void* wt_out, float* bias_out,
                                void* stream);
@@ -217,6 +227,13 @@
                         int64_t dv_ts, int dtype, int64_t batch, int heads, int64_t nq, int64_t nk,
                         int head_dim, float scale, void* stream);
 
+int vited_attention_bwd_dq_rows(const void* q, int64_t q_bs, int64_t q_ts, const void* k, int64_t k_bs, int64_t k_ts,
+                                const void* v, int64_t v_bs, int64_t v_ts, const void* o, const void* d_o, int64_t o_bs,
+                                int64_t o_ts, const float* lse, float* delta, void* dq, int64_t dq_bs, int64_t dq_ts,
+                                int64_t dq_rows, void* dk, int64_t dk_bs, int64_t dk_ts, void* dv, int64_t dv_bs,
+                                int64_t dv_ts, int dtype, int64_t batch, int heads, int64_t nq, int64_t nk, int head_dim,
+                                float scale, void* stream);
+
 int64_t vited_attention_bwd_indexed_workspace_bytes(int dtype, int64_t batch, int heads, int64_t nk, int head_dim);
 int vited_attention_bwd_indexed(const void* q, int64_t q_bs, int64_t q_ts, const void* k, int64_t k_bs, int64_t k_ts,
                                 const void* v, int64_t v_bs, int64_t v_ts, const int64_t* kv_index, const int64_t* seg_order,
diff --git a/vit-ed_amd/csrc/attention.hip b/vit-ed_amd/csrc/attention.hip
--- a/vit-ed_amd/csrc/attention.hip
+++ b/vit-ed_amd/csrc/attention.hip
@@ -48,6 +48,7 @@
         g_last_attn_path = 2;
         return attention_bwd_mfma(a, s);
     }
+    if (a.dq_rows > a.nq) return VITED_ERR_UNSUPPORTED;
     g_last_attn_path = 1;
     return attention_bwd_portable(a, dtype, s);
 }
@@ -57,6 +58,16 @@
                                    int64_t o_ts, const float* lse, float* delta, void* dq, int64_t dq_bs, int64_t dq_ts,
                                    void* dk, int64_t dk_bs, int64_t dk_ts, void* dv, int64_t dv_bs, int64_t dv_ts, int dtype,
                                    int64_t batch, int heads, int64_t nq, int64_t nk, int head_dim, float scale, void* stream) {
+    return vited_attention_bwd_dq_rows(q, q_bs, q_ts, k, k_bs, k_ts, v, v_bs, v_ts, o, d_o, o_bs, o_ts, lse, delta, dq, dq_bs, dq_ts, 0, dk,
+                                       dk_bs, dk_ts, dv, dv_bs, dv_ts, dtype, batch, heads, nq, nk, head_dim, scale, stream);
+}
+
+extern "C" int vited_attention_bwd_dq_rows(const void* q, int64_t q_bs, int64_t q_ts, const void* k, int64_t k_bs, int64_t k_ts,
+                                           const void* v, int64_t v_bs, int64_t v_ts, const void* o, const void* d_o, int64_t o_bs,
+                                           int64_t o_ts, const float* lse, float* delta, void* dq, int64_t dq_bs, int64_t dq_ts,
+                                           int64_t dq_rows, void* dk, int64_t dk_bs, int64_t dk_ts, void* dv, int64_t dv_bs,
+                                           int64_t dv_ts, int dtype, int64_t batch, int heads, int64_t nq, int64_t nk, int head_dim,
+                                           float scale, void* stream) {
     AttnArgs a = {};
     a.q = q; a.k = k; a.v = v;
     a.q_bs = q_bs; a.q_ts = q_ts; a.k_bs = k_bs; a.k_ts = k_ts; a.v_bs = v_bs; a.v_ts = v_ts;
@@ -65,9 +76,11 @@
     a.dq = dq; a.dk = dk; a.dv = dv;
     a.dq_bs = dq_bs; a.dq_ts = dq_ts; a.dk_bs = dk_bs; a.dk_ts = dk_ts; a.dv_bs = dv_bs; a.dv_ts = dv_ts;
     a.batch = batch; a.heads = heads; a.nq = nq; a.nk = nk; a.head_dim = head_dim; a.scale = scale;
+    a.dq_rows = dq_rows;
     int rc = check_common(a, dtype);
     if (rc != VITED_OK) return rc;
     if (!d_o || !delta || !dq || !dk || !dv) return VITED_ERR_BAD_ARG;
+    if (dq_rows < 0 || (dq_rows && dq_rows < nq) || dq_rows > (1 << 20)) return VITED_ERR_BAD_ARG;
     return bwd_dispatch(a, dtype, (hipStream_t)stream);
 }
 
diff --git a/vit-ed_amd/csrc/attention_kernels.h b/vit-ed_amd/csrc/attention_kernels.h
--- a/vit-ed_amd/csrc/attention_kernels.h
+++ b/vit-ed_amd/csrc/attention_kernels.h
@@ -15,6 +15,7 @@
     int64_t batch, nq, nk;
     int heads, head_dim;
     float scale;
+    int64_t dq_rows;
 };
 
 int attention_fwd_portable(const AttnArgs& a, int dtype, hipStream_t s);
diff --git a/vit-ed_amd/csrc/attention_mfma.hip b/vit-ed_amd/csrc/attention_mfma.hip
--- a/vit-ed_amd/csrc/attention_mfma.hip
+++ b/vit-ed_amd/csrc/attention_mfma.hip
@@ -106,6 +106,16 @@
         const int row = c / CPR, ch = c % CPR;
         const bf16x8 v = *(const bf16x8*)(region + row * ROW + ch * 16);
         if (row < n && ch / (CPR / 4) < live_heads) *(bf16x8*)(dst_head0 + (int64_t)row * ts + ch * 8) = v;
+    }
+}
+
+template <int HD>
+__device__ __forceinline__ void zero_rows4(bf16* dst_head0, int64_t ts, int row0, int row1, int live_heads, int tid) {
+    constexpr int CPR = 4 * HD * 2 / 16;
+    const bf16x8 z = {};
+    for (int c = tid; c < (row1 - row0) * CPR; c += 256) {
+        const int row = row0 + c / CPR, ch = c % CPR;
+        if (ch / (CPR / 4) < live_heads) *(bf16x8*)(dst_head0 + (int64_t)row * ts + ch * 8) = z;
     }
 }
 
@@ -226,6 +236,9 @@
     }
     __syncthreads();
     store_rows4<HD, NQT>(out1, (bf16*)a.dq + b * a.dq_bs + hoff0, a.dq_ts, nq, live_heads, tid);
+    if constexpr (NQT == 1) {
+        if (a.dq_rows > nq) zero_rows4<HD>((bf16*)a.dq + b * a.dq_bs + hoff0, a.dq_ts, nq, (int)a.dq_rows, live_heads, tid);
+    }
     __syncthreads();
 
     asm volatile("" ::: "memory");
@@ -360,8 +373,9 @@
 }
 
 int attention_bwd_mfma(const AttnArgs& a, hipStream_t s) {
-    if (!small_ok(a, true)) return attention_bwd_flash(a, s);
+    if (!small_ok(a, true)) return a.dq_rows > a.nq ? VITED_ERR_UNSUPPORTED : attention_bwd_flash(a, s);
     const int nqt = (int)((a.nq + 15) / 16), nkt = (int)((a.nk + 15) / 16);
+    if (a.dq_rows > a.nq && nqt != 1) return VITED_ERR_UNSUPPORTED;
     switch (nqt) {
         case 1: return launch_bwd_small32<1>(a, nkt, s);
         case 2: return launch_bwd_small32<2>(a, nkt, s);
diff --git a/vit-ed_amd/csrc/elementwise.hip b/vit-ed_amd/csrc/elementwise.hip
--- a/vit-ed_amd/csrc/elementwise.hip
+++ b/vit-ed_amd/csrc/elementwise.hip
@@ -190,21 +190,76 @@
     }
 }
 
+struct U8Norm { float scale[4], shift[4]; };
+
+template <typename S_, typename D>
+__global__ void __launch_bounds__(256)
+patchify_run8_kernel(const S_* __restrict__ img, int64_t img_bs, const int64_t* __restrict__ bidx, D* __restrict__ out, int chans,
+                     int S, int lp, U8Norm nrm) {
+    const int p = 1 << lp, G = S >> lp, W = S >> 3;
+    const int64_t b = blockIdx.y;
+    const int py = blockIdx.x;
+    const int64_t src_b = bidx ? bidx[b] : b;
+    const S_* base = img + src_b * img_bs;
+    const int Kp = (chans << lp) << lp;
+    D* obase = out + (b * G * G + (int64_t)py * G) * Kp;
+    const int x = ((int)threadIdx.x % W) << 3, row0 = (int)threadIdx.x / W, step = (int)blockDim.x / W;
+    if (row0 >= step) return;
+    const int px = x >> lp, j = x & (p - 1);
+    for (int ci = row0; ci < (chans << lp); ci += step) {
+        const int c = ci >> lp, i = ci & (p - 1);
+        const S_* src = base + ((int64_t)c * S + ((py << lp) + i)) * S + x;
+        float v[8];
+        if constexpr (sizeof(S_) == 1) {
+            const uint2 q = *(const uint2*)src;
+            const float sc = nrm.scale[c], sh = nrm.shift[c];
+#pragma unroll
+            for (int e = 0; e < 4; ++e) {
+                v[e] = fmaf((float)((q.x >> (8 * e)) & 255u), sc, sh);
+                v[4 + e] = fmaf((float)((q.y >> (8 * e)) & 255u), sc, sh);
+            }
+        } else {
+            const f32x4 a = *(const f32x4*)src, d = *(const f32x4*)(src + 4);
+#pragma unroll
+            for (int e = 0; e < 4; ++e) { v[e] = a[e]; v[4 + e] = d[e]; }
+        }
+        D* dst = obase + (int64_t)px * Kp + (ci << lp) + j;
+        if constexpr (sizeof(D) == 2) {
+            bf16x8 o;
+#pragma unroll
+            for (int e = 0; e < 8; ++e) o[e] = from_f32<bf16>(v[e]);
+            *(bf16x8*)dst = o;
+        } else {
+            *(f32x4*)dst = f32x4{v[0], v[1], v[2], v[3]};
+            *(f32x4*)(dst + 4) = f32x4{v[4], v[5], v[6], v[7]};
+        }
+    }
+}
+
+static inline int patchify_run8_log2p(int img_size, int patch) {
+    if (patch < 8 || (patch & (patch - 1)) || img_size / 8 > 256) return 0;
+    int lp = 3;
+    while ((1 << lp) < patch) ++lp;
+    return lp;
+}
+
 extern "C" int vited_patchify(const float* img, int64_t img_bs, const int64_t* batch_index, void* out, int out_dtype,
                               int64_t batch, int chans, int img_size, int patch, void* stream) {
     if (!img || !out || batch <= 0 || chans <= 0 || img_size <= 0 || patch <= 0 || img_size % patch) return VITED_ERR_BAD_ARG;
     dim3 grid(img_size / patch, (unsigned)batch);
     hipStream_t s = (hipStream_t)stream;
-    if (out_dtype == VITED_BF16)
-        hipLaunchKernelGGL((patchify_kernel<bf16>), grid, dim3(256), 0, s, img, img_bs, batch_index, (bf16*)out, chans, img_size, patch);
-    else if (out_dtype == VITED_F32)
-        hipLaunchKernelGGL((patchify_kernel<float>), grid, dim3(256), 0, s, img, img_bs, batch_index, (float*)out, chans, img_size, patch);
-    else
+    const int lp = patchify_run8_log2p(img_size, patch);
+    const bool run8 = lp > 0 && img_bs % 4 == 0 && (((uintptr_t)img | (uintptr_t)out) & 15) == 0;
+    if (out_dtype == VITED_BF16) {
+        if (run8) hipLaunchKernelGGL((patchify_run8_kernel<float, bf16>), grid, dim3(256), 0, s, img, img_bs, batch_index, (bf16*)out, chans, img_size, lp, U8Norm{});
+        else hipLaunchKernelGGL((patchify_kernel<bf16>), grid, dim3(256), 0, s, img, img_bs, batch_index, (bf16*)out, chans, img_size, patch);
+    } else if (out_dtype == VITED_F32) {
+        if (run8) hipLaunchKernelGGL((patchify_run8_kernel<float, float>), grid, dim3(256), 0, s, img, img_bs, batch_index, (float*)out, chans, img_size, lp, U8Norm{});
+        else hipLaunchKernelGGL((patchify_kernel<float>), grid, dim3(256), 0, s, img, img_bs, batch_index, (float*)out, chans, img_size, patch);
+    } else
         return VITED_ERR_UNSUPPORTED;
     return vited_check_launch();
 }
-
-struct U8Norm { float scale[4], shift[4]; };
 
 template <typename D>
 __global__ void patchify_u8_kernel(const uint8_t* __restrict__ img, int64_t img_bs, const int64_t* __restrict__ bidx,
@@ -240,11 +295,15 @@
     }
     dim3 grid(img_size / patch, (unsigned)batch);
     hipStream_t s = (hipStream_t)stream;
-    if (out_dtype == VITED_BF16)
-        hipLaunchKernelGGL((patchify_u8_kernel<bf16>), grid, dim3(256), 0, s, img, img_bs, batch_index, (bf16*)out, chans, img_size, patch, nrm);
-    else if (out_dtype == VITED_F32)
-        hipLaunchKernelGGL((patchify_u8_kernel<float>), grid, dim3(256), 0, s, img, img_bs, batch_index, (float*)out, chans, img_size, patch, nrm);
-    else
+    const int lp = patchify_run8_log2p(img_size, patch);
+    const bool run8 = lp > 0 && img_bs % 8 == 0 && ((uintptr_t)img & 7) == 0 && ((uintptr_t)out & 15) == 0;
+    if (out_dtype == VITED_BF16) {
+        if (run8) hipLaunchKernelGGL((patchify_run8_kernel<uint8_t, bf16>), grid, dim3(256), 0, s, img, img_bs, batch_index, (bf16*)out, chans, img_size, lp, nrm);
+        else hipLaunchKernelGGL((patchify_u8_kernel<bf16>), grid, dim3(256), 0, s, img, img_bs, batch_index, (bf16*)out, chans, img_size, patch, nrm);
+    } else if (out_dtype == VITED_F32) {
+        if (run8) hipLaunchKernelGGL((patchify_run8_kernel<uint8_t, float>), grid, dim3(256), 0, s, img, img_bs, batch_index, (float*)out, chans, img_size, lp, nrm);
+        else hipLaunchKernelGGL((patchify_u8_kernel<float>), grid, dim3(256), 0, s, img, img_bs, batch_index, (float*)out, chans, img_size, patch, nrm);
+    } else
         return VITED_ERR_UNSUPPORTED;
     return vited_check_launch();
 }
@@ -419,6 +478,104 @@
     return vited_check_launch();
 }
 
+template <typename D>
+__global__ void __launch_bounds__(256)
+patch_grad_partial_kernel(const float* __restrict__ dx, D* __restrict__ tok, float* __restrict__ partial, int64_t batch, int64_t width,
+                          int64_t first_col, int64_t rows_per_split) {
+    const int64_t r = ((int64_t)blockIdx.x * blockDim.x + threadIdx.x) * 4;
+    if (r >= width) return;
+    const int64_t b0 = (int64_t)blockIdx.y * rows_per_split;
+    int64_t b1 = b0 + rows_per_split;
+    if (b1 > batch) b1 = batch;
+    const int64_t tok_ld = width - first_col;
+    D* __restrict__ t = (tok && r >= first_col) ? tok + (r - first_col) : nullptr;
+    auto put = [&](int64_t b, const f32x4& v) {
+        if (!t) return;
+        if constexpr (sizeof(D) == 2)
+            *(bf16x4*)(t + b * tok_ld) = bf16x4{from_f32<bf16>(v[0]), from_f32<bf16>(v[1]), from_f32<bf16>(v[2]), from_f32<bf16>(v[3])};
+        else
+            *(f32x4*)(t + b * tok_ld) = v;
+    };
+    f32x4 acc0 = {0.f, 0.f, 0.f, 0.f}, acc1 = acc0, acc2 = acc0, acc3 = acc0;
+    const float* __restrict__ in = dx + r;
+    int64_t b = b0;
+    for (; b + 7 < b1; b += 8) {
+        f32x4 v[8];
+#pragma unroll
+        for (int k = 0; k < 8; ++k) v[k] = *(const f32x4*)(in + (b + k) * width);
+        acc0 += v[0]; acc1 += v[1]; acc2 += v[2]; acc3 += v[3];
+        acc0 += v[4]; acc1 += v[5]; acc2 += v[6]; acc3 += v[7];
+#pragma unroll
+        for (int k = 0; k < 8; ++k) put(b + k, v[k]);
+    }
+    for (; b + 3 < b1; b += 4) {
+        f32x4 v[4];
+#pragma unroll
+        for (int k = 0; k < 4; ++k) v[k] = *(const f32x4*)(in + (b + k) * width);
+        acc0 += v[0]; acc1 += v[1]; acc2 += v[2]; acc3 += v[3];
+#pragma unroll
+        for (int k = 0; k < 4; ++k) put(b + k, v[k]);
+    }
+    for (; b < b1; ++b) {
+        const f32x4 v = *(const f32x4*)(in + b * width);
+        acc0 += v;
+        put(b, v);
+    }
+    *(f32x4*)(partial + (int64_t)blockIdx.y * width + r) = (acc0 + acc1) + (acc2 + acc3);
+}
+
+__global__ void __launch_bounds__(256)
+patch_grad_finish_kernel(const float* __restrict__ partial, int64_t splits, int64_t width, float* __restrict__ dpos, int64_t pos_off_col,
+                         float* __restrict__ dcls, int64_t dim, int accumulate) {
+    const int64_t q = ((int64_t)blockIdx.x * blockDim.x + threadIdx.x) * 4;
+    if (q >= width + pos_off_col) return;
+    const int64_t r = q - pos_off_col;
+    f32x4 sum = {0.f, 0.f, 0.f, 0.f};
+    if (r >= 0) {
+        f32x4 acc0 = sum, acc1 = sum, acc2 = sum, acc3 = sum;
+        const float* __restrict__ in = partial + r;
+        int64_t k = 0;
+        for (; k + 3 < splits; k += 4) {
+            acc0 += *(const f32x4*)(in + k * width);
+            acc1 += *(const f32x4*)(in + (k + 1) * width);
+            acc2 += *(const f32x4*)(in + (k + 2) * width);
+            acc3 += *(const f32x4*)(in + (k + 3) * width);
+        }
+        for (; k < splits; ++k) acc0 += *(const f32x4*)(in + k * width);
+        sum = (acc0 + acc1) + (acc2 + acc3);
+    }
+    *(f32x4*)(dpos + q) = accumulate ? *(const f32x4*)(dpos + q) + sum : sum;
+    if (dcls && r >= 0 && r < dim) *(f32x4*)(dcls + r) = accumulate ? *(const f32x4*)(dcls + r) + sum : sum;
+}
+
+extern "C" int64_t vited_patch_grad_prep_workspace_bytes(int64_t batch, int64_t rows, int64_t dim) {
+    if (batch <= 0 || rows <= 0 || dim <= 0) return 0;
+    return sum_rows_splits(batch, rows * dim) * rows * dim * (int64_t)sizeof(float);
+}
+
+extern "C" int vited_patch_grad_prep(const float* dx, int64_t batch, int64_t rows, int64_t dim, int64_t first, void* tok, int tok_dtype,
+                                     float* dpos, float* dcls, int accumulate, float* workspace, int64_t workspace_bytes, void* stream) {
+    if (!dx || !dpos || batch <= 0 || rows <= 0 || dim <= 0 || first < 0 || first > 1 || first >= rows) return VITED_ERR_BAD_ARG;
+    if (dcls && !first) return VITED_ERR_BAD_ARG;
+    if (dim % 4) return VITED_ERR_UNSUPPORTED;
+    if (((uintptr_t)dx | (uintptr_t)dpos | (uintptr_t)dcls | (uintptr_t)workspace) & 15) return VITED_ERR_BAD_ARG;
+    if (tok && ((uintptr_t)tok & (tok_dtype == VITED_F32 ? 15 : 7))) return VITED_ERR_BAD_ARG;
+    const int64_t width = rows * dim, S = sum_rows_splits(batch, width);
+    if (!workspace || workspace_bytes < S * width * (int64_t)sizeof(float)) return VITED_ERR_WORKSPACE;
+    const int64_t rps = ceil_div64(batch, S), first_col = first * dim, pos_off_col = (1 - first) * dim;
+    hipStream_t s = (hipStream_t)stream;
+    const dim3 grid((unsigned)ceil_div64(width, 1024), (unsigned)S);
+    if (!tok || tok_dtype == VITED_BF16)
+        hipLaunchKernelGGL((patch_grad_partial_kernel<bf16>), grid, dim3(256), 0, s, dx, (bf16*)tok, workspace, batch, width, first_col, rps);
+    else if (tok_dtype == VITED_F32)
+        hipLaunchKernelGGL((patch_grad_partial_kernel<float>), grid, dim3(256), 0, s, dx, (float*)tok, workspace, batch, width, first_col, rps);
+    else
+        return VITED_ERR_UNSUPPORTED;
+    hipLaunchKernelGGL(patch_grad_finish_kernel, dim3((unsigned)ceil_div64(width + pos_off_col, 1024)), dim3(256), 0, s,
+                       (const float*)workspace, S, width, dpos, pos_off_col, dcls, dim, accumulate);
+    return vited_check_launch();
+}
+
 __device__ __forceinline__ void sum_slabs_body(const float* __restrict__ in, int64_t in_ld, float* __restrict__ out, int64_t batch,
                                                int64_t width, int accumulate, int64_t r) {
     if (r >= width) return;
diff --git a/vit-ed_amd/csrc/gemm_row.hip b/vit-ed_amd/csrc/gemm_row.hip
--- a/vit-ed_amd/csrc/gemm_row.hip
+++ b/vit-ed_amd/csrc/gemm_row.hip
@@ -20,6 +20,7 @@
     bf16* h; int64_t ldh; float* mean; float* rstd;
     const float* x; int64_t ldx; const float* mean_in; const float* rstd_in;
     const float* dx_in; int64_t ldxi; float* dx; int64_t lddx; bf16* dx_lp; int64_t ldlp;
+    int dx_in_period;
     float* partial;
     const float* row_scale;
     const float* lp_scale;
@@ -251,11 +252,16 @@
     auto load_bwd = [&](RowBwdIn<SCALED>& in, int64_t m) {
         const bool ok = m < a.M;
         if constexpr (SCALED) in.lps[0] = ok ? a.lp_scale[m] : 0.f;
+        const float* din = (ok && a.dx_in) ? a.dx_in + m * a.ldxi : nullptr;
+        if (a.dx_in_period && din) {
+            const uint32_t item = (uint32_t)m / (uint32_t)a.dx_in_period;
+            din = (uint32_t)m == item * (uint32_t)a.dx_in_period ? a.dx_in + (int64_t)item * a.ldxi : nullptr;
+        }
 #pragma unroll
         for (int j = 0; j < 3; ++j) {
             const int c = (j * 32 + hl) * 4;
             in.x[j] = ok ? ROW_LOAD((const f32x4*)(a.x + m * a.ldx + c)) : f32x4{0.f, 0.f, 0.f, 0.f};
-            in.din[j] = (ok && a.dx_in) ? ROW_LOAD((const f32x4*)(a.dx_in + m * a.ldxi + c)) : f32x4{0.f, 0.f, 0.f, 0.f};
+            in.din[j] = din ? ROW_LOAD((const f32x4*)(din + c)) : f32x4{0.f, 0.f, 0.f, 0.f};
         }
         in.mu = ok ? a.mean_in[m] : 0.f;
         in.rs = ok ? a.rstd_in[m] : 0.f;
@@ -488,10 +494,11 @@
 
 static int linear_layernorm_bwd_impl(const void* dy, int64_t lddy, int64_t seg_k, int64_t seg_stride, const void* wt, int64_t ldwt,
                                     const float* x, int64_t ldx, const float* gamma, const float* mean, const float* rstd,
-                                    const float* dx_in, int64_t dx_in_ld, float* dx_out, int64_t dx_out_ld, void* dx_lp, int64_t dx_lp_ld,
-                                    const float* lp_scale, float* dgamma, float* dbeta, int accumulate, int64_t M, int64_t N, int64_t K,
+                                    const float* dx_in, int64_t dx_in_ld, int64_t dx_in_period, float* dx_out, int64_t dx_out_ld, void* dx_lp,
+                                    int64_t dx_lp_ld, const float* lp_scale, float* dgamma, float* dbeta, int accumulate, int64_t M, int64_t N, int64_t K,
                                     float* workspace, int64_t workspace_bytes, void* stream) {
     if (lp_scale && !dx_lp) return VITED_ERR_BAD_ARG;
+    if (dx_in_period < 0 || dx_in_period > 0x7fffffff || (dx_in_period && (!dx_in || M % dx_in_period))) return VITED_ERR_BAD_ARG;
     if (!dy || !wt || !x || !gamma || !mean || !rstd || !dx_out || M <= 0 || N <= 0 || K <= 0) return VITED_ERR_BAD_ARG;
     if ((dgamma == nullptr) != (dbeta == nullptr)) return VITED_ERR_BAD_ARG;
     if (seg_k <= 0 || K % seg_k || lddy < seg_k || ldwt < K || ldx < N || dx_out_ld < N || (dx_in && dx_in_ld < N) || (dx_lp && dx_lp_ld < N))
@@ -503,7 +510,7 @@
     RowArgs r = {};
     r.A = (const bf16*)dy; r.lda = lddy; r.seg_k = (int)seg_k; r.seg_stride = seg_stride; r.W = (const bf16*)wt; r.ldw = ldwt; r.M = M; r.K = (int)K;
     r.gamma = gamma; r.x = x; r.ldx = ldx; r.mean_in = mean; r.rstd_in = rstd;
-    r.dx_in = dx_in; r.ldxi = dx_in_ld; r.dx = dx_out; r.lddx = dx_out_ld; r.dx_lp = (bf16*)dx_lp; r.ldlp = dx_lp_ld;
+    r.dx_in = dx_in; r.ldxi = dx_in_ld; r.dx_in_period = (int)dx_in_period; r.dx = dx_out; r.lddx = dx_out_ld; r.dx_lp = (bf16*)dx_lp; r.ldlp = dx_lp_ld;
     r.partial = workspace;
     r.lp_scale = lp_scale;
     const int rc = row_launch<ROW_MODE_BWD>(r, (hipStream_t)stream);
@@ -516,7 +523,7 @@
                                           int64_t dx_in_ld, float* dx_out, int64_t dx_out_ld, void* dx_lp, int64_t dx_lp_ld,
                                           float* dgamma, float* dbeta, int accumulate, int64_t M, int64_t N, int64_t K,
                                           float* workspace, int64_t workspace_bytes, void* stream) {
-    return linear_layernorm_bwd_impl(dy, lddy, K, 0, wt, ldwt, x, ldx, gamma, mean, rstd, dx_in, dx_in_ld, dx_out, dx_out_ld, dx_lp, dx_lp_ld,
+    return linear_layernorm_bwd_impl(dy, lddy, K, 0, wt, ldwt, x, ldx, gamma, mean, rstd, dx_in, dx_in_ld, 0, dx_out, dx_out_ld, dx_lp, dx_lp_ld,
                                      nullptr, dgamma, dbeta, accumulate, M, N, K, workspace, workspace_bytes, stream);
 }
 
@@ -527,7 +534,7 @@
                                                     float* dbeta, int accumulate, int64_t M, int64_t N, float* workspace,
                                                     int64_t workspace_bytes, void* stream) {
     if (segments <= 0) return VITED_ERR_BAD_ARG;
-    return linear_layernorm_bwd_impl(dy, lddy, seg_k, seg_stride, wt, ldwt, x, ldx, gamma, mean, rstd, dx_in, dx_in_ld, dx_out, dx_out_ld, dx_lp,
+    return linear_layernorm_bwd_impl(dy, lddy, seg_k, seg_stride, wt, ldwt, x, ldx, gamma, mean, rstd, dx_in, dx_in_ld, 0, dx_out, dx_out_ld, dx_lp,
                                      dx_lp_ld, nullptr, dgamma, dbeta, accumulate, M, N, segments * seg_k, workspace, workspace_bytes, stream);
 }
 
@@ -536,6 +543,16 @@
                                                  int64_t dx_in_ld, float* dx_out, int64_t dx_out_ld, void* dx_lp, int64_t dx_lp_ld,
                                                  const float* lp_scale, float* dgamma, float* dbeta, int accumulate, int64_t M, int64_t N,
                                                  int64_t K, float* workspace, int64_t workspace_bytes, void* stream) {
-    return linear_layernorm_bwd_impl(dy, lddy, K, 0, wt, ldwt, x, ldx, gamma, mean, rstd, dx_in, dx_in_ld, dx_out, dx_out_ld, dx_lp, dx_lp_ld,
+    return linear_layernorm_bwd_impl(dy, lddy, K, 0, wt, ldwt, x, ldx, gamma, mean, rstd, dx_in, dx_in_ld, 0, dx_out, dx_out_ld, dx_lp, dx_lp_ld,
                                      lp_scale, dgamma, dbeta, accumulate, M, N, K, workspace, workspace_bytes, stream);
 }
+
+extern "C" int vited_linear_layernorm_bwd_periodic(const void* dy, int64_t lddy, const void* wt, int64_t ldwt, const float* x, int64_t ldx,
+                                                   const float* gamma, const float* mean, const float* rstd, const float* dx_in,
+                                                   int64_t dx_in_ld, int64_t dx_in_period, float* dx_out, int64_t dx_out_ld, void* dx_lp,
+                                                   int64_t dx_lp_ld, const float* lp_scale, float* dgamma, float* dbeta, int accumulate,
+                                                   int64_t M, int64_t N, int64_t K, float* workspace, int64_t workspace_bytes, void* stream) {
+    if (dx_in_period <= 0) return VITED_ERR_BAD_ARG;
+    return linear_layernorm_bwd_impl(dy, lddy, K, 0, wt, ldwt, x, ldx, gamma, mean, rstd, dx_in, dx_in_ld, dx_in_period, dx_out, dx_out_ld, dx_lp,
+                                     dx_lp_ld, lp_scale, dgamma, dbeta, accumulate, M, N, K, workspace, workspace_bytes, stream);
+}
diff --git a/vit-ed_amd/functions.py b/vit-ed_amd/functions.py
--- a/vit-ed_amd/functions.py
+++ b/vit-ed_amd/functions.py
@@ -318,7 +318,12 @@
 
 def _row_kernel_ok(rt, m, n, k, dtype, *rowwise):
     return (rt.fused_ln and not rt.exact and ops.linear_layernorm_supported(m, n, k, dtype)
-            and all(t is None or (t.dim() == 2 and t.stride(1) == 1 and t.stride(0) % 4 == 0) for t in rowwise))
+            and all(t is None or _row_operand_ok(t) for t in rowwise))
+
+
+def _row_operand_ok(t):
+    step = 8 if t.element_size() == 2 else 4
+    return t.dim() == 2 and t.stride(1) == 1 and t.stride(0) % step == 0 and t.data_ptr() % 16 == 0
 
 
 def _res_linear(rt, a, w, bias, residual, ln=None, scale=None):
@@ -326,19 +331,22 @@
     if ln is not None and _row_kernel_ok(rt, a.shape[0], wsh.shape[0], a.shape[1], a.dtype, a, residual):
         y, h, mean, rstd = ops.linear_residual_layernorm_fwd(a, wsh, bias, residual, ln[0], ln[1], LN_EPS, row_scale=scale)
         return y, (h, mean, rstd)
+    if residual.stride(0) != residual.shape[1]:
+        residual = _dense_rows(residual)
     y = ops.gemm(a, wsh, epilogue=EPI_RESIDUAL, bias=bias, residual=residual, row_scale=scale)
     return y, (ops.layernorm_fwd(y, ln[0], ln[1], LN_EPS, rt.act_dtype) if ln is not None else None)
 
 
-def _linear_ln_bwd(rt, dy, h_saved, w, bias, x, gamma, beta, mean, rstd, dx_in=None, dx_out=None, want_lp=True, lp_scale=None):
+def _linear_ln_bwd(rt, dy, h_saved, w, bias, x, gamma, beta, mean, rstd, dx_in=None, dx_out=None, want_lp=True, lp_scale=None,
+                   dx_in_period=0):
     want_lp = want_lp and not rt.exact
     wt, layout = rt.weight_t(w)
-    if layout == B_NK and _row_kernel_ok(rt, dy.shape[0], wt.shape[0], dy.shape[1], dy.dtype, dy, x, dx_in, dx_out):
+    if dx_in_period or (layout == B_NK and _row_kernel_ok(rt, dy.shape[0], wt.shape[0], dy.shape[1], dy.dtype, dy, x, dx_in, dx_out)):
         gg, gb = _gtarget(rt, gamma), _gtarget(rt, beta)
         direct = gg is not None and gb is not None
         dx, dx_lp, dg, db = ops.linear_layernorm_bwd(dy, wt, x, gamma, mean, rstd, dx_in=dx_in, dx_out=dx_out, want_lp=want_lp,
                                                      dgamma=gg if direct else None, dbeta=gb if direct else None, defer=rt.ln_queue,
-                                                     lp_scale=lp_scale)
+                                                     lp_scale=lp_scale, dx_in_period=dx_in_period)
         if direct:
             dg = db = None
     else:
@@ -483,19 +491,14 @@
 
 
 def _patch_tokens_bwd(rt, dx, patches, S, with_cls, batch):
-    rows = rt.n2 if with_cls else rt.n1
-    dx3 = dx.view(batch, rows, rt.dim)
-    dpos_rows = ops.sum_rows(dx3.view(batch, rows * rt.dim)).view(rows, rt.dim)
-    dpos = torch.zeros_like(S.pos)
+    rows, first = (rt.n2, 1) if with_cls else (rt.n1, 0)
+    want_tok = with_cls or not rt.exact
+    dtok, dpos, dcls = ops.patch_grad_prep(dx.view(batch, rows, rt.dim), first, rt.act_dtype if want_tok else None,
+                                           dpos=torch.empty_like(S.pos), dcls=torch.empty_like(S.cls) if with_cls else None)
     grads = dict(pos=dpos)
     if with_cls:
-        dpos[0] = dpos_rows
-        grads['cls'] = dpos_rows[0].clone().view_as(S.cls)
-        dtok = ops.slice_rows_cast(dx3, 1, rt.n1, rt.act_dtype)
-    else:
-        dpos[0, 1:] = dpos_rows
-        dtok = dx if rt.exact else ops.cast(dx, rt.act_dtype)
-    grads['pw'], grads['pb'] = _weight_grads(rt, dtok, patches, S.pw, S.pb)
+        grads['cls'] = dcls
+    grads['pw'], grads['pb'] = _weight_grads(rt, dtok if want_tok else dx, patches, S.pw, S.pb)
     return grads
 
 
@@ -570,7 +573,7 @@
     qkv3 = qkv.view(batch, n, 3 * d)
     o0, lse0 = ops.attention_fwd(qkv3[:, 0:1, 0:d], qkv3[:, :, d:2 * d], qkv3[:, :, 2 * d:3 * d], rt.heads, rt.scale)
     o0 = o0.view(batch, d)
-    x0 = _dense_rows(x.view(batch, n, d)[:, 0, :])
+    x0 = x.view(batch, n, d)[:, 0, :]
     xa, lnq = _res_linear(rt, o0, P.wproj, P.bproj, x0, next_ln, scale)
     return xa, (m1, r1, h1, qkv, o0, lse0), lnq
 
@@ -582,13 +585,20 @@
     m1, r1, h1, qkv, o0, lse0 = saved
     do0, dwproj, dbproj = _linear_bwd(rt, dx_lp, o0, P.wproj, P.bproj)
     qkv3 = qkv.view(batch, n, 3 * d)
-    dqkv = torch.zeros_like(qkv)
+    fill_dq = not rt.exact and ops.attention_bwd_fills_dq(qkv.dtype, 1, n, rt.head_dim)
+    dqkv = torch.empty_like(qkv) if fill_dq else torch.zeros_like(qkv)
     dqkv3 = dqkv.view(batch, n, 3 * d)
     ops.attention_bwd(qkv3[:, 0:1, 0:d], qkv3[:, :, d:2 * d], qkv3[:, :, 2 * d:3 * d], o0.view(batch, 1, d), do0.view(batch, 1, d),
-                      lse0, rt.heads, rt.scale, dqkv3[:, 0:1, 0:d], dqkv3[:, :, d:2 * d], dqkv3[:, :, 2 * d:3 * d])
-    dres = torch.zeros((batch * n, d), dtype=torch.float32, device=dx.device)
-    dres.view(batch, n, d)[:, 0, :].copy_(dx)
-    dx, dx_lp, dg1, db1, dwqkv, dbqkv = _linear_ln_bwd(rt, dqkv, h1, P.wqkv, P.bqkv, x, P.g1, P.b1, m1, r1, dx_in=dres, lp_scale=lp_scale)
+                      lse0, rt.heads, rt.scale, dqkv3[:, :, 0:d] if fill_dq else dqkv3[:, 0:1, 0:d], dqkv3[:, :, d:2 * d],
+                      dqkv3[:, :, 2 * d:3 * d])
+    wt, layout = rt.weight_t(P.wqkv)
+    if layout == B_NK and _row_kernel_ok(rt, batch * n, wt.shape[0], 3 * d, dqkv.dtype, dqkv, x, dx):
+        period, dres = n, dx
+    else:
+        period, dres = 0, torch.zeros((batch * n, d), dtype=torch.float32, device=dx.device)
+        dres.view(batch, n, d)[:, 0, :].copy_(dx)
+    dx, dx_lp, dg1, db1, dwqkv, dbqkv = _linear_ln_bwd(rt, dqkv, h1, P.wqkv, P.bqkv, x, P.g1, P.b1, m1, r1, dx_in=dres, lp_scale=lp_scale,
+                                                       dx_in_period=period)
     return dx, dx_lp, dict(g1=dg1, b1=db1, wqkv=dwqkv, bqkv=dbqkv, wproj=dwproj, bproj=dbproj)
 
 
diff --git a/vit-ed_amd/ops.py b/vit-ed_amd/ops.py
--- a/vit-ed_amd/ops.py
+++ b/vit-ed_amd/ops.py
@@ -291,6 +291,26 @@
     ws = _scratch(_lib.load().vited_sum_rows_workspace_bytes(b, w), x.device)
     _lib.call('vited_sum_rows', _ptr(x), _code(x.dtype), ld, _ptr(out), b, w, *ws, _stream())
     return out
+
+
+def patch_grad_prep(dx: torch.Tensor, first: int, tok_dtype: torch.dtype | None, dpos: torch.Tensor | None = None,
+                    dcls: torch.Tensor | None = None, accumulate: bool = False):
+    _need_gpu(dx, dpos, dcls)
+    assert dx.dtype == torch.float32 and dx.dim() == 3 and dx.is_contiguous() and first in (0, 1)
+    b, r, d = dx.shape
+    if accumulate and (dpos is None or (first and dcls is None)):
+        raise ValueError('patch_grad_prep: accumulate needs the gradients to add to')
+    if dpos is None:
+        dpos = torch.empty((r + 1 - first, d), dtype=torch.float32, device=dx.device)
+    if dcls is None and first:
+        dcls = torch.empty(d, dtype=torch.float32, device=dx.device)
+    assert dpos.dtype == torch.float32 and dpos.numel() == (r + 1 - first) * d and dpos.is_contiguous()
+    assert dcls is None or (first and dcls.dtype == torch.float32 and dcls.numel() == d and dcls.is_contiguous())
+    tok = None if tok_dtype is None else torch.empty((b * (r - first), d), dtype=tok_dtype, device=dx.device)
+    ws = _scratch(_lib.load().vited_patch_grad_prep_workspace_bytes(b, r, d), dx.device)
+    _lib.call('vited_patch_grad_prep', _ptr(dx), b, r, d, first, _ptr(tok), _code(tok_dtype or torch.bfloat16), _ptr(dpos), _ptr(dcls),
+              int(accumulate), *ws, _stream())
+    return tok, dpos, dcls
 
 
 def layernorm_fwd(x: torch.Tensor, gamma: torch.Tensor, beta: torch.Tensor, eps: float, out_dtype: torch.dtype, out=None):
@@ -467,7 +487,7 @@
 
 
 def linear_layernorm_bwd(dy, wt, x, gamma, mean, rstd, dx_in=None, dx_out=None, want_lp: bool = False, dgamma=None, dbeta=None,
-                         defer=None, lp_scale=None):
+                         defer=None, lp_scale=None, dx_in_period: int = 0):
     _need_gpu(dy, wt, x, gamma, mean, rstd, dx_in, dx_out, lp_scale)
     assert dy.dtype == wt.dtype == torch.bfloat16 and x.dtype == torch.float32
     segments = 1
@@ -506,7 +526,11 @@
                _rows2d(dx_out), _ptr(dx_lp), n)
     sum_args = (0 if defer is not None else _ptr(dgamma), 0 if defer is not None else _ptr(dbeta), int(accumulate))
     tail = dx_args + sum_args
-    if lp_scale is not None:
+    if dx_in_period:
+        assert segments == 1 and dx_in is not None and m % dx_in_period == 0 and dx_in.shape == (m // dx_in_period, n)
+        _lib.call('vited_linear_layernorm_bwd_periodic', _ptr(dy), lddy, _ptr(wt), ldwt, *dx_args[:7], int(dx_in_period), *dx_args[7:],
+                  _ptr(lp_scale), *sum_args, m, n, k, *ws, _stream())
+    elif lp_scale is not None:
         _lib.call('vited_linear_layernorm_bwd_scaled', _ptr(dy), lddy, _ptr(wt), ldwt, *dx_args, _ptr(lp_scale), *sum_args, m, n, k, *ws,
                   _stream())
     elif segments > 1:
@@ -730,6 +754,10 @@
     return groups, labels, weights, PairSegments(seg_index, seg_order, seg_offsets), counts
 
 
+def attention_bwd_fills_dq(dtype: torch.dtype, nq: int, nk: int, head_dim: int) -> bool:
+    return dtype == torch.bfloat16 and head_dim == 32 and nq <= 16 and nk <= 80
+
+
 def attention_bwd(q, k, v, o, do, lse, heads: int, scale: float, dq, dk, dv, kv_index=None, segments=None):
     _need_gpu(q, k, v, o, do, lse, dq, dk, dv)
     b, nq, d = q.shape
@@ -738,6 +766,11 @@
     assert o.is_contiguous() and do.is_contiguous() and o.dtype == do.dtype == q.dtype
     if segments is None and kv_index is not None:
         segments = pair_segments(kv_index, k.shape[0])
+    dq_rows = 0
+    if dq.shape[1] != nq:
+        dq_rows = dq.shape[1]
+        if dq_rows < nq or segments is not None or dq.shape[0] != b:
+            raise ValueError(f'attention_bwd: dq of {dq_rows} rows for {nq} query rows (more rows only, and without segments)')
     if segments is not None:
         return _attention_bwd_indexed(q, k, v, o, do, lse, heads, scale, dq, dk, dv, kv_index, segments)
     q_bs, q_ts = _head_view(q, heads, hd)
@@ -747,9 +780,9 @@
     dk_bs, dk_ts = _head_view(dk, heads, hd)
     dv_bs, dv_ts = _head_view(dv, heads, hd)
     delta = torch.empty((b, heads, nq), dtype=torch.float32, device=q.device)
-    _lib.call('vited_attention_bwd',
+    _lib.call('vited_attention_bwd_dq_rows',
               _ptr(q), q_bs, q_ts, _ptr(k), k_bs, k_ts, _ptr(v), v_bs, v_ts, _ptr(o), _ptr(do), nq * d, d, _ptr(lse), _ptr(delta),
-              _ptr(dq), dq_bs, dq_ts, _ptr(dk), dk_bs, dk_ts, _ptr(dv), dv_bs, dv_ts, _code(q.dtype), b, heads, nq, nk, hd,
+              _ptr(dq), dq_bs, dq_ts, dq_rows, _ptr(dk), dk_bs, dk_ts, _ptr(dv), dv_bs, dv_ts, _code(q.dtype), b, heads, nq, nk, hd,
               float(scale), _stream())
     return dq, dk, dv
 
```

Measured after the change: 44070, median of 6. No clear change (+0.5%).
